# kubeflow/mpi-operator

Hardware: AMD Instinct MI355X
Metric: images/sec (higher is better)
Workload: dtype bf16; 1 GPU; model=resnet101, global_batch=64, image=224, parallelism=dp1, impl=hip, graph=True

## Files before the change

### mpi_operator_amd/ops/csrc/batchnorm.hip

```cpp
#include "common.h"

template <int WHAT>
__global__ void bn_partials_k(const ushort8 *__restrict__ x,
                              const ushort8 *__restrict__ dy,
                              const ushort8 *__restrict__ y,
                              const uint8_t *__restrict__ mask,
                              const float *__restrict__ mean,
                              const float *__restrict__ invstd,
                              float *__restrict__ partial,
                              long M, int C8, int relu) {
  int C = C8 * 8;
  int cb = threadIdx.x % C8;
  int row_lane = threadIdx.x / C8;
  int rows_per_block = blockDim.x / C8;
  float a0[8] = {0}, a1[8] = {0};
  float mn[8], is[8];
  if (WHAT == 1 && row_lane < rows_per_block) {
#pragma unroll
    for (int j = 0; j < 8; ++j) {
      mn[j] = mean[cb * 8 + j];
      is[j] = invstd[cb * 8 + j];
    }
  }
  if (row_lane < rows_per_block) {
    long stride = (long)gridDim.x * rows_per_block;
    for (long row = (long)blockIdx.x * rows_per_block + row_lane; row < M;
         row += 2 * stride) {
      long r2 = row + stride;
      bool has2 = r2 < M;
      long off = row * C8 + cb, off2 = r2 * C8 + cb;
      float fx[8], fx2[8];
      ushort8 vx = x[off];
      ushort8 vx2 = has2 ? x[off2] : ushort8{0, 0, 0, 0, 0, 0, 0, 0};
      bf8_to_f8(vx, fx);
      bf8_to_f8(vx2, fx2);
      if (WHAT == 0) {
#pragma unroll
        for (int j = 0; j < 8; ++j) {
          a0[j] += fx[j] + fx2[j];
          a1[j] += fx[j] * fx[j] + fx2[j] * fx2[j];
        }
      } else {
        ushort8 vdy = dy[off];
        ushort8 vdy2 = has2 ? dy[off2] : ushort8{0, 0, 0, 0, 0, 0, 0, 0};
        float fdy[8], fdy2[8];
        bf8_to_f8(vdy, fdy);
        bf8_to_f8(vdy2, fdy2);
        if (relu) {
          if (mask) {
            int m1 = mask[off], m2 = has2 ? mask[off2] : 0;
#pragma unroll
            for (int j = 0; j < 8; ++j) {
              if (!(m1 & (1 << j))) fdy[j] = 0.f;
              if (!(m2 & (1 << j))) fdy2[j] = 0.f;
            }
          } else {
            ushort8 vy = y[off];
            ushort8 vy2 = has2 ? y[off2] : ushort8{0, 0, 0, 0, 0, 0, 0, 0};
#pragma unroll
            for (int j = 0; j < 8; ++j) {
              if (!(bf2f(vy[j]) > 0.f)) fdy[j] = 0.f;
              if (!(bf2f(vy2[j]) > 0.f)) fdy2[j] = 0.f;
            }
          }
        }
#pragma unroll
        for (int j = 0; j < 8; ++j) {
          a0[j] += fdy[j] + fdy2[j];
          a1[j] += fdy[j] * ((fx[j] - mn[j]) * is[j]) +
                   fdy2[j] * ((fx2[j] - mn[j]) * is[j]);
        }
      }
    }
  }
  __shared__ float lds[2][256 * 8];
#pragma unroll
  for (int j = 0; j < 8; ++j) {
    lds[0][threadIdx.x * 8 + j] = a0[j];
    lds[1][threadIdx.x * 8 + j] = a1[j];
  }
  __syncthreads();
  if (row_lane == 0) {
    for (int rl = 1; rl < rows_per_block; ++rl) {
#pragma unroll
      for (int j = 0; j < 8; ++j) {
        a0[j] += lds[0][(rl * C8 + cb) * 8 + j];
        a1[j] += lds[1][(rl * C8 + cb) * 8 + j];
      }
    }
    float *p0 = partial + (long)blockIdx.x * 2 * C + cb * 8;
    float *p1 = p0 + C;
#pragma unroll
    for (int j = 0; j < 8; ++j) {
      p0[j] = a0[j];
      p1[j] = a1[j];
    }
  }
}

DEV_INLINE void lane8_sums(const float *__restrict__ partial, int grid, int C,
                           int c, int lane8, float &s0, float &s1) {
  s0 = 0.f;
  s1 = 0.f;
  for (int g = lane8; g < grid; g += 32) {
    s0 += partial[(long)g * 2 * C + c];
    s1 += partial[(long)g * 2 * C + C + c];
  }
#pragma unroll
  for (int off = 16; off > 0; off >>= 1) {
    s0 += __shfl_down(s0, off, 32);
    s1 += __shfl_down(s1, off, 32);
  }
}

__global__ void bn_finalize_fwd_k(const float *__restrict__ partial, int grid,
                                  int C, const float *__restrict__ gamma,
                                  const float *__restrict__ beta, float inv_m,
                                  float eps, float *__restrict__ mean,
                                  float *__restrict__ invstd,
                                  float *__restrict__ scale,
                                  float *__restrict__ shift,
                                  float *__restrict__ running_mean,
                                  float *__restrict__ running_var,
                                  float momentum, float unbias) {
  int t = blockIdx.x * blockDim.x + threadIdx.x;
  int c = t / 32, lane8 = t % 32;
  if (c >= C) return;
  float s, sq;
  lane8_sums(partial, grid, C, c, lane8, s, sq);
  if (lane8 != 0) return;
  float mu = s * inv_m;
  float var = fmaxf(sq * inv_m - mu * mu, 0.f);
  float is = rsqrtf(var + eps);
  mean[c] = mu;
  invstd[c] = is;
  float sc = gamma[c] * is;
  scale[c] = sc;
  shift[c] = beta[c] - mu * sc;
  if (running_mean) {
    running_mean[c] = running_mean[c] * (1.f - momentum) + mu * momentum;
    running_var[c] = running_var[c] * (1.f - momentum) + var * unbias * momentum;
  }
}

__global__ void bn_finalize_bwd_k(const float *__restrict__ partial, int grid,
                                  int C, const float *__restrict__ gamma,
                                  const float *__restrict__ invstd, float inv_m,
                                  float *__restrict__ dbeta,
                                  float *__restrict__ dgamma,
                                  float *__restrict__ k1,
                                  float *__restrict__ k2,
                                  float *__restrict__ k3) {
  int t = blockIdx.x * blockDim.x + threadIdx.x;
  int c = t / 32, lane8 = t % 32;
  if (c >= C) return;
  float s0, s1;
  lane8_sums(partial, grid, C, c, lane8, s0, s1);
  if (lane8 != 0) return;
  dbeta[c] = s0;
  dgamma[c] = s1;
  float g_is = gamma[c] * invstd[c];
  k1[c] = g_is;
  k2[c] = g_is * s0 * inv_m;
  k3[c] = g_is * s1 * inv_m;
}

__global__ void bn_finalize_fwd_bands_k(
    const float *__restrict__ partial, int grid, int C,
    const float *__restrict__ gamma, const float *__restrict__ beta,
    float inv_m, float eps, float *__restrict__ mean,
    float *__restrict__ invstd, float *__restrict__ scale,
    float *__restrict__ shift, float *__restrict__ running_mean,
    float *__restrict__ running_var, float momentum,
    float unbias);

__global__ void bn_finalize_bwd_bands_k(
    const float *__restrict__ partial, int grid, int C,
    const float *__restrict__ gamma, const float *__restrict__ invstd,
    float inv_m, float *__restrict__ dbeta, float *__restrict__ dgamma,
    float *__restrict__ k1, float *__restrict__ k2, float *__restrict__ k3) {
  int c = blockIdx.x;
  if (c >= C) return;
  float s0 = 0.f, s1 = 0.f;
  for (int g = threadIdx.x; g < grid; g += 256) {
    s0 += partial[(long)g * 2 * C + c];
    s1 += partial[(long)g * 2 * C + C + c];
  }
  __shared__ float red[2][256 / WAVE];
  s0 = wave_sum(s0);
  s1 = wave_sum(s1);
  if ((threadIdx.x & (WAVE - 1)) == 0) {
    red[0][threadIdx.x / WAVE] = s0;
    red[1][threadIdx.x / WAVE] = s1;
  }
  __syncthreads();
  if (threadIdx.x != 0) return;
  s0 = red[0][0] + red[0][1] + red[0][2] + red[0][3];
  s1 = red[1][0] + red[1][1] + red[1][2] + red[1][3];
  dbeta[c] = s0;
  dgamma[c] = s1;
  float g_is = gamma[c] * invstd[c];
  k1[c] = g_is;
  k2[c] = g_is * s0 * inv_m;
  k3[c] = g_is * s1 * inv_m;
}

__global__ void bn_apply_k(const ushort8 *__restrict__ x,
                           const ushort8 *__restrict__ res,
                           const float *__restrict__ scale,
                           const float *__restrict__ shift,
                           ushort8 *__restrict__ y,
                           uint8_t *__restrict__ mask,
                           long M, int C8, int relu) {
  int cb = threadIdx.x % C8;
  int row_lane = threadIdx.x / C8;
  int rows_per_block = blockDim.x / C8;
  if (row_lane >= rows_per_block) return;
  float sc[8], sh[8];
#pragma unroll
  for (int j = 0; j < 8; ++j) {
    sc[j] = scale[cb * 8 + j];
    sh[j] = shift[cb * 8 + j];
  }
  long stride = (long)gridDim.x * rows_per_block;
  for (long row = (long)blockIdx.x * rows_per_block + row_lane; row < M;
       row += 2 * stride) {
    long r2 = row + stride;
    long off = row * C8 + cb, off2 = r2 * C8 + cb;
    ushort8 v = x[off];
    ushort8 v2 = r2 < M ? x[off2] : ushort8{0, 0, 0, 0, 0, 0, 0, 0};
    float f[8], f2[8], g[8] = {0}, g2[8] = {0};
    bf8_to_f8(v, f);
    bf8_to_f8(v2, f2);
    if (res) {
      ushort8 w = res[off];
      ushort8 w2 = r2 < M ? res[off2] : ushort8{0, 0, 0, 0, 0, 0, 0, 0};
      bf8_to_f8(w, g);
      bf8_to_f8(w2, g2);
    }
    int m1 = 0, m2 = 0;
#pragma unroll
    for (int j = 0; j < 8; ++j) {
      f[j] = f[j] * sc[j] + sh[j] + g[j];
      f2[j] = f2[j] * sc[j] + sh[j] + g2[j];
      if (relu) {
        if (f[j] > 0.f) m1 |= 1 << j;
        if (f2[j] > 0.f) m2 |= 1 << j;
        f[j] = fmaxf(f[j], 0.f);
        f2[j] = fmaxf(f2[j], 0.f);
      }
    }
    y[off] = f8_to_bf8(f);
    if (r2 < M) y[off2] = f8_to_bf8(f2);
    if (relu && mask) {
      mask[off] = (uint8_t)m1;
      if (r2 < M) mask[off2] = (uint8_t)m2;
    }
  }
}

__global__ void bn_bwd_apply_k(const ushort8 *__restrict__ dy,
                               const ushort8 *__restrict__ x,
                               const ushort8 *__restrict__ y,
                               const uint8_t *__restrict__ mask,
                               const float *__restrict__ mean,
                               const float *__restrict__ invstd,
                               const float *__restrict__ k1,
                               const float *__restrict__ k2,
                               const float *__restrict__ k3,
                               ushort8 *__restrict__ dx, long M, int C8,
                               int relu) {
  int cb = threadIdx.x % C8;
  int row_lane = threadIdx.x / C8;
  int rows_per_block = blockDim.x / C8;
  if (row_lane >= rows_per_block) return;
  float mn[8], is[8], a[8], b[8], c3[8];
#pragma unroll
  for (int j = 0; j < 8; ++j) {
    int c = cb * 8 + j;
    mn[j] = mean[c];
    is[j] = invstd[c];
    a[j] = k1[c];
    b[j] = k2[c];
    c3[j] = k3[c];
  }
  long stride = (long)gridDim.x * rows_per_block;
  for (long row = (long)blockIdx.x * rows_per_block + row_lane; row < M;
       row += 2 * stride) {
    long r2 = row + stride;
    long off = row * C8 + cb, off2 = r2 * C8 + cb;
    ushort8 vdy = dy[off], vx = x[off];
    ushort8 vdy2 = r2 < M ? dy[off2] : ushort8{0, 0, 0, 0, 0, 0, 0, 0};
    ushort8 vx2 = r2 < M ? x[off2] : ushort8{0, 0, 0, 0, 0, 0, 0, 0};
    float fdy[8], fx[8], fdy2[8], fx2[8];
    bf8_to_f8(vdy, fdy);
    bf8_to_f8(vx, fx);
    bf8_to_f8(vdy2, fdy2);
    bf8_to_f8(vx2, fx2);
    if (relu) {
      if (mask) {
        int m1 = mask[off], m2 = r2 < M ? mask[off2] : 0;
#pragma unroll
        for (int j = 0; j < 8; ++j) {
          if (!(m1 & (1 << j))) fdy[j] = 0.f;
          if (!(m2 & (1 << j))) fdy2[j] = 0.f;
        }
      } else {
        ushort8 vy = y[off];
        ushort8 vy2 = r2 < M ? y[off2] : ushort8{0, 0, 0, 0, 0, 0, 0, 0};
#pragma unroll
        for (int j = 0; j < 8; ++j) {
          if (!(bf2f(vy[j]) > 0.f)) fdy[j] = 0.f;
          if (!(bf2f(vy2[j]) > 0.f)) fdy2[j] = 0.f;
        }
      }
    }
#pragma unroll
    for (int j = 0; j < 8; ++j) {
      fdy[j] = a[j] * fdy[j] - b[j] - c3[j] * ((fx[j] - mn[j]) * is[j]);
      fdy2[j] = a[j] * fdy2[j] - b[j] - c3[j] * ((fx2[j] - mn[j]) * is[j]);
    }
    dx[off] = f8_to_bf8(fdy);
    if (r2 < M) dx[off2] = f8_to_bf8(fdy2);
  }
}

extern "C" int bn_grid_cap(int C8) {
  static const long ovr = [] {
    const char *e = getenv("MPIAMD_BN_GRID");
    long v = e ? atol(e) : 0;
    return (v >= 1 && v <= 8192) ? v : 0;
  }();
  (void)C8;
  return ovr ? (int)ovr : 512;
}

static void bn_geom(long M, int C8, int &grid, int &rows_per_block) {
  rows_per_block = 256 / C8;
  long g = (M + rows_per_block - 1) / rows_per_block;
  long cap = bn_grid_cap(C8);
  grid = (int)(g > cap ? cap : (g < 1 ? 1 : g));
}

static int bn_apply_grid(long M, int C8) {
  static const long cap = [] {
    const char *e = getenv("MPIAMD_BN_APPLY_GRID");
    long v = e ? atol(e) : 0;
    return (v >= 64 && v <= 16384) ? v : 2048L;
  }();
  int rpb = 256 / C8;
  long g = (M + rpb - 1) / rpb;
  return (int)(g > cap ? cap : (g < 1 ? 1 : g));
}

extern "C" hipError_t bn_fwd_train_launch(
    const void *x, const void *res, const float *gamma, const float *beta,
    float eps, int relu, void *y, uint8_t *relu_mask, float *mean,
    float *invstd, float *scale, float *shift, float *partial,
    float *running_mean, float *running_var, float momentum, long M, int C,
    hipStream_t s) {
  int C8 = C / 8;
  if (C8 < 1 || C8 > 256) return hipErrorInvalidValue;
  int grid, rpb;
  bn_geom(M, C8, grid, rpb);
  bn_partials_k<0><<<grid, 256, 0, s>>>((const ushort8 *)x, nullptr, nullptr,
                                        nullptr, nullptr, nullptr, partial, M,
                                        C8, 0);
  HIP_KERNEL_CHECK();
  float unbias = M > 1 ? (float)M / (float)(M - 1) : 1.f;
  bn_finalize_fwd_bands_k<<<C, 256, 0, s>>>(
      partial, grid, C, gamma, beta, 1.f / (float)M, eps, mean, invstd, scale,
      shift, running_mean, running_var, momentum, unbias);
  HIP_KERNEL_CHECK();
  bn_apply_k<<<bn_apply_grid(M, C8), 256, 0, s>>>(
      (const ushort8 *)x, (const ushort8 *)res, scale, shift, (ushort8 *)y,
      relu_mask, M, C8, relu);
  HIP_KERNEL_CHECK();
  return hipSuccess;
}

__global__ void bn_finalize_fwd_bands_k(
    const float *__restrict__ partial, int grid, int C,
    const float *__restrict__ gamma, const float *__restrict__ beta,
    float inv_m, float eps, float *__restrict__ mean,
    float *__restrict__ invstd, float *__restrict__ scale,
    float *__restrict__ shift, float *__restrict__ running_mean,
    float *__restrict__ running_var, float momentum, float unbias) {
  int c = blockIdx.x;
  if (c >= C) return;
  float s = 0.f, sq = 0.f;
  for (int g = threadIdx.x; g < grid; g += 256) {
    s += partial[(long)g * 2 * C + c];
    sq += partial[(long)g * 2 * C + C + c];
  }
  __shared__ float red[2][256 / WAVE];
  s = wave_sum(s);
  sq = wave_sum(sq);
  if ((threadIdx.x & (WAVE - 1)) == 0) {
    red[0][threadIdx.x / WAVE] = s;
    red[1][threadIdx.x / WAVE] = sq;
  }
  __syncthreads();
  if (threadIdx.x != 0) return;
  s = red[0][0] + red[0][1] + red[0][2] + red[0][3];
  sq = red[1][0] + red[1][1] + red[1][2] + red[1][3];
  float mu = s * inv_m;
  float var = fmaxf(sq * inv_m - mu * mu, 0.f);
  float is = rsqrtf(var + eps);
  mean[c] = mu;
  invstd[c] = is;
  float sc = gamma[c] * is;
  scale[c] = sc;
  shift[c] = beta[c] - mu * sc;
  if (running_mean) {
    running_mean[c] = running_mean[c] * (1.f - momentum) + mu * momentum;
    running_var[c] = running_var[c] * (1.f - momentum) + var * unbias * momentum;
  }
}

extern "C" hipError_t bn_fwd_train_pre_launch(
    const float *pre_partial, int pre_grid, const void *x, const void *res,
    const float *gamma, const float *beta, float eps, int relu, void *y,
    uint8_t *relu_mask, float *mean, float *invstd, float *scale,
    float *shift, float *running_mean, float *running_var, float momentum,
    long M, int C, hipStream_t s) {
  int C8 = C / 8;
  if (C8 < 1 || C8 > 256) return hipErrorInvalidValue;
  float unbias = M > 1 ? (float)M / (float)(M - 1) : 1.f;
  bn_finalize_fwd_bands_k<<<C, 256, 0, s>>>(
      pre_partial, pre_grid, C, gamma, beta, 1.f / (float)M, eps, mean,
      invstd, scale, shift, running_mean, running_var, momentum, unbias);
  HIP_KERNEL_CHECK();
  bn_apply_k<<<bn_apply_grid(M, C8), 256, 0, s>>>(
      (const ushort8 *)x, (const ushort8 *)res, scale, shift, (ushort8 *)y,
      relu_mask, M, C8, relu);
  HIP_KERNEL_CHECK();
  return hipSuccess;
}

extern "C" hipError_t bn_fwd_eval_launch(const void *x, const float *scale,
                                         const float *shift, int relu, void *y,
                                         long M, int C, hipStream_t s) {
  int C8 = C / 8;
  if (C8 < 1 || C8 > 256) return hipErrorInvalidValue;
  int grid, rpb;
  bn_geom(M, C8, grid, rpb);
  bn_apply_k<<<bn_apply_grid(M, C8), 256, 0, s>>>(
      (const ushort8 *)x, nullptr, scale, shift, (ushort8 *)y, nullptr, M, C8,
      relu);
  HIP_KERNEL_CHECK();
  return hipSuccess;
}

extern "C" hipError_t bn_bwd_launch(const void *dy, const void *x,
                                    const void *y, const uint8_t *relu_mask,
                                    const float *gamma, const float *mean,
                                    const float *invstd, int relu, void *dx,
                                    float *dgamma, float *dbeta, float *k1,
                                    float *k2, float *k3, float *partial,
                                    long M, int C, hipStream_t s) {
  int C8 = C / 8;
  if (C8 < 1 || C8 > 256) return hipErrorInvalidValue;
  int grid, rpb;
  bn_geom(M, C8, grid, rpb);
  bn_partials_k<1><<<grid, 256, 0, s>>>((const ushort8 *)x, (const ushort8 *)dy,
                                        (const ushort8 *)y, relu_mask, mean,
                                        invstd, partial, M, C8, relu);
  HIP_KERNEL_CHECK();
  bn_finalize_bwd_bands_k<<<C, 256, 0, s>>>(
      partial, grid, C, gamma, invstd, 1.f / (float)M, dbeta, dgamma, k1, k2, k3);
  HIP_KERNEL_CHECK();
  bn_bwd_apply_k<<<bn_apply_grid(M, C8), 256, 0, s>>>(
      (const ushort8 *)dy, (const ushort8 *)x, (const ushort8 *)y, relu_mask,
      mean, invstd, k1, k2, k3, (ushort8 *)dx, M, C8, relu);
  HIP_KERNEL_CHECK();
  return hipSuccess;
}
```

### mpi_operator_amd/ops/csrc/bindings.cpp

```cpp
#include <torch/extension.h>

#include <ATen/hip/impl/HIPGuardImplMasqueradingAsCUDA.h>
#include <ATen/hip/impl/HIPStreamMasqueradingAsCUDA.h>
#include <hip/hip_runtime.h>

#include <vector>

namespace {

using at::Tensor;

int conv_splits(long M, int Ncols, int K) {
  static const int force = [] {
    const char *e = getenv("MPIAMD_CONV_SPLITS");
    return e ? atoi(e) : -1;
  }();
  if (force >= 1) return force;
  long tiles = ((M + 127) / 128) * ((Ncols + 127) / 128);
  int nk = (K + 63) / 64;
  if (tiles >= 256 || nk < 16) return 1;
  long s = 512 / tiles;
  if (s > nk / 8) s = nk / 8;
  if (s > 16) s = 16;
  return s < 1 ? 1 : (int)s;
}

#define CHK(call)                                                              \
  do {                                                                         \
    hipError_t e_ = (call);                                                    \
    TORCH_CHECK(e_ == hipSuccess, "HIP kernel failure: ", hipGetErrorString(e_)); \
  } while (0)

hipStream_t cur_stream() {
  return c10::hip::getCurrentHIPStreamMasqueradingAsCUDA().stream();
}
using HIPDeviceGuard = c10::hip::HIPGuardMasqueradingAsCUDA;

void check_cl_bf16(const Tensor &t, const char *name) {
  TORCH_CHECK(t.is_cuda(), name, " must be on GPU");
  TORCH_CHECK(t.scalar_type() == at::kBFloat16, name, " must be bf16");
  TORCH_CHECK(t.dim() == 4 && t.is_contiguous(at::MemoryFormat::ChannelsLast),
              name, " must be 4-D channels_last");
}

Tensor empty_cl_bf16(int64_t n, int64_t c, int64_t h, int64_t w, const Tensor &like) {
  return at::empty({n, c, h, w}, like.options().dtype(at::kBFloat16),
                   at::MemoryFormat::ChannelsLast);
}

}

extern "C" {
hipError_t add_relu_fwd(const void *, const void *, void *, long, hipStream_t);
hipError_t add_bf16(const void *, const void *, void *, long, hipStream_t);
hipError_t add_relu_bwd(const void *, const void *, void *, long, hipStream_t);
hipError_t add_relu_bwd_add(const void *, const void *, const void *, void *,
                            long, hipStream_t);
hipError_t add_relu_bwd_add_mask(const void *, const void *, const void *,
                                 void *, long, hipStream_t);
hipError_t gap_fwd(const void *, void *, int, int, int, hipStream_t);
hipError_t gap_bwd(const void *, void *, int, int, int, hipStream_t);
hipError_t bias_add(void *, const float *, long, int, hipStream_t);
hipError_t colsum_bf16(const void *, float *, float *, long, int, long, hipStream_t);
int colsum_chunks(long, int);
struct SgdDesc {
  const void *grad;
  float *master;
  float *mom;
  uint16_t *out;
  long numel;
};
hipError_t sgd_step_launch(const SgdDesc *, int, int, float, float, float, int,
                           hipStream_t);
int bn_grid_cap(int);
hipError_t bn_fwd_train_launch(const void *, const void *, const float *,
                               const float *, float, int, void *, uint8_t *,
                               float *, float *, float *, float *, float *,
                               float *, float *, float, long, int,
                               hipStream_t);
hipError_t bn_fwd_eval_launch(const void *, const float *, const float *, int,
                              void *, long, int, hipStream_t);
hipError_t bn_bwd_launch(const void *, const void *, const void *,
                         const uint8_t *, const float *, const float *,
                         const float *, int, void *, float *, float *,
                         float *, float *, float *, float *, long, int,
                         hipStream_t);
hipError_t maxpool_fwd_launch(const void *, void *, uint8_t *, int, int, int,
                              int, int, int, int, int, int, hipStream_t);
hipError_t maxpool_bwd_launch(const void *, const uint8_t *, void *, int, int,
                              int, int, int, int, int, int, int, hipStream_t);
hipError_t softmax_xent_fwd_launch(const void *, const long *, float *, float *,
                                   int, int, hipStream_t);
hipError_t masked_xent_fwd_launch(const void *, const long *, float *, float *,
                                  int, int, long, long, hipStream_t);
hipError_t masked_xent_bwd_launch(const void *, const long *, const float *,
                                  const float *, const float *, void *, int,
                                  int, long, long, hipStream_t);
hipError_t attn_fwd_launch(const void *, void *, void *, const float *, int,
                           int, int, float, hipStream_t);
hipError_t attn_bwd_launch(const void *, const void *, const void *, void *,
                           int, int, int, float, hipStream_t);
hipError_t softmax_xent_bwd_launch(const float *, const long *, void *, int,
                                   int, const float *, hipStream_t);
hipError_t gemm_nt(const void *, const void *, void *, int, int, int, long,
                   long, long, int, hipStream_t);
hipError_t gemm_nt_bias(const void *, const void *, const float *, void *,
                        int, int, int, long, long, long, hipStream_t);
hipError_t gemm_nt_bias_sk(const void *, const void *, const float *, float *,
                           void *, int, int, int, long, long, long, int,
                           hipStream_t);
int gemm_fwd_splits(int, int, int);
hipError_t gemm_nt_tn(const void *, const void *, void *, int, int, int, long,
                      long, long, int, hipStream_t);
hipError_t gemm_nt_tn_acc(const void *, const void *, void *, int, int, int,
                          long, long, long, hipStream_t);
hipError_t gemm_nt_gelu_bias(const void *, const void *, const float *,
                             void *, void *, int, int, int, long, long, long,
                             hipStream_t);
hipError_t gemm_nt_tn_gelubwd(const void *, const void *, const void *,
                              void *, int, int, int, long, long, long,
                              void *, hipStream_t);
int gemm_gelubwd_wants_wt(int, int, int);
hipError_t gemm_tn_tn(const void *, const void *, void *, int, int, int, long,
                      long, long, int, hipStream_t);
int gemm_tn_tn_splits(int, int, int);
hipError_t gemm_tn_tn_sk(const void *, const void *, float *, void *, int,
                         int, int, long, long, long, int, int, hipStream_t);
hipError_t gemm_nt_tn_sk(const void *, const void *, float *, void *, int,
                         int, int, long, long, long, int, hipStream_t);
int gemm_nt_tn_splits(int, int, int);
hipError_t conv_fwd(const void *, const void *, void *, int, int, int, int,
                    int, int, int, int, int, int, int, int, float *,
                    hipStream_t);
hipError_t conv_dgrad(const void *, const void *, void *, int, int, int, int,
                      int, int, int, int, int, int, int, int, float *,
                      hipStream_t);
hipError_t conv_fwd_bn(const void *, const void *, void *, int, int, int,
                       int, int, int, int, int, int, int, int, float *,
                       hipStream_t);
hipError_t bn_fwd_train_pre_launch(const float *, int, const void *,
                                   const void *, const float *, const float *,
                                   float, int, void *, uint8_t *, float *,
                                   float *, float *, float *, float *,
                                   float *, float, long, int, hipStream_t);
hipError_t conv_dgrad_1x1_acc(const void *, const void *, void *, long, int,
                              int, hipStream_t);
hipError_t conv_wgrad_implicit(const void *, const void *, float *, void *,
                               int, int, int, int, int, int, int, int, int,
                               int, int, int, int, hipStream_t);
hipError_t mfma_probe(const void *, const void *, float *, hipStream_t);
hipError_t ln_fwd(const void *, const float *, const float *, void *, float *,
                  float *, long, int, float, hipStream_t);
hipError_t ln_fwd_add(const void *, const void *, const float *,
                      const float *, void *, void *, float *, float *, long,
                      int, float, hipStream_t);
hipError_t ln_bwd(const void *, const void *, const float *, const float *,
                  const float *, void *, float *, float *, long, int, int *,
                  hipStream_t);
}

static Tensor conv2d_fwd(const Tensor &x, const Tensor &w, int64_t stride,
                         int64_t pad) {
  check_cl_bf16(x, "x");
  check_cl_bf16(w, "w");
  const HIPDeviceGuard guard(x.device());
  int N = x.size(0), C = x.size(1), H = x.size(2), W = x.size(3);
  int Kout = w.size(0), R = w.size(2), S = w.size(3);
  TORCH_CHECK(w.size(1) == C, "conv channel mismatch");
  TORCH_CHECK(C % 8 == 0, "conv requires C%8==0 (pad the stem input)");
  int HO = (H + 2 * (int)pad - R) / (int)stride + 1;
  int WO = (W + 2 * (int)pad - S) / (int)stride + 1;
  Tensor y = empty_cl_bf16(N, Kout, HO, WO, x);
  long M = (long)N * HO * WO;
  int splits = conv_splits(M, Kout, R * S * C);
  Tensor partial;
  float *pp = nullptr;
  if (splits > 1) {
    partial = at::empty({(long)splits, M, (long)Kout},
                        x.options().dtype(at::kFloat));
    pp = partial.data_ptr<float>();
  }
  CHK(conv_fwd(x.data_ptr(), w.data_ptr(), y.data_ptr(), N, H, W, C, Kout, R,
               S, (int)stride, (int)pad, HO, WO, splits, pp, cur_stream()));
  return y;
}

static Tensor conv2d_dgrad(const Tensor &dy, const Tensor &w, int64_t H,
                           int64_t W, int64_t stride, int64_t pad) {
  check_cl_bf16(dy, "dy");
  check_cl_bf16(w, "w");
  const HIPDeviceGuard guard(dy.device());
  int N = dy.size(0), Kout = dy.size(1), HO = dy.size(2), WO = dy.size(3);
  int C = w.size(1), R = w.size(2), S = w.size(3);
  TORCH_CHECK(Kout % 8 == 0, "dgrad requires out-channels %8==0");
  TORCH_CHECK(stride == 1 || stride == 2,
              "conv2d_dgrad supports stride 1 or 2 only, got ", stride);
  Tensor dx = empty_cl_bf16(N, C, H, W, dy);
  long M = (long)N * H * W;
  int splits = stride == 1 ? conv_splits(M, C, R * S * Kout) : 1;
  Tensor partial;
  float *pp = nullptr;
  if (splits > 1) {
    partial = at::empty({(long)splits, M, (long)C},
                        dy.options().dtype(at::kFloat));
    pp = partial.data_ptr<float>();
  }
  CHK(conv_dgrad(dy.data_ptr(), w.data_ptr(), dx.data_ptr(), N, (int)H,
                 (int)W, C, Kout, R, S, (int)stride, (int)pad, HO, WO, splits,
                 pp, cur_stream()));
  return dx;
}

static Tensor conv2d_wgrad(const Tensor &x, const Tensor &dy, int64_t R,
                           int64_t S, int64_t stride, int64_t pad) {
  check_cl_bf16(x, "x");
  check_cl_bf16(dy, "dy");
  const HIPDeviceGuard guard(x.device());
  int N = x.size(0), C = x.size(1), H = x.size(2), W = x.size(3);
  int Kout = dy.size(1), HO = dy.size(2), WO = dy.size(3);
  int RSC = (int)R * S * C;
  int tiles = ((Kout + 127) / 128) * ((RSC + 127) / 128);
  long M = (long)N * HO * WO;
  int nk = (int)((M + 63) / 64);
  static const int budget = [] {
    const char *e = getenv("MPIAMD_WGRAD_BUDGET");
    int v = e ? atoi(e) : 0;
    return (v >= 64 && v <= 2048) ? v : 512;
  }();
  int splits = std::max(budget / tiles, 1);
  splits = std::min(splits, std::max(nk / 8, 1));
  splits = std::min(splits, 256);
  if (splits >= 8) splits &= ~7;
  Tensor partial = at::empty({(long)splits, (long)Kout, (long)RSC},
                             x.options().dtype(at::kFloat));
  Tensor dw = at::empty({(int64_t)Kout, (int64_t)C, R, S},
                        x.options().dtype(at::kBFloat16),
                        at::MemoryFormat::ChannelsLast);
  CHK(conv_wgrad_implicit(dy.data_ptr(), x.data_ptr(),
                          partial.data_ptr<float>(), dw.data_ptr(), N, H, W, C,
                          Kout, (int)R, (int)S, (int)stride, (int)pad, HO, WO,
                          splits, 1, cur_stream()));
  return dw;
}

static Tensor add_bf16_b(const Tensor &a, const Tensor &b) {
  const HIPDeviceGuard guard(a.device());
  TORCH_CHECK(a.numel() == b.numel() && a.numel() % 8 == 0);
  Tensor c = at::empty_like(a);
  CHK(add_bf16(a.data_ptr(), b.data_ptr(), c.data_ptr(), a.numel(), cur_stream()));
  return c;
}

static void conv2d_dgrad_acc(const Tensor &dy, const Tensor &w, Tensor &dx_acc) {
  check_cl_bf16(dy, "dy");
  check_cl_bf16(w, "w");
  check_cl_bf16(dx_acc, "dx_acc");
  const HIPDeviceGuard guard(dy.device());
  TORCH_CHECK(w.size(2) == 1 && w.size(3) == 1, "acc dgrad is 1x1-only");
  long M = (long)dy.size(0) * dy.size(2) * dy.size(3);
  CHK(conv_dgrad_1x1_acc(dy.data_ptr(), w.data_ptr(), dx_acc.data_ptr(), M,
                         (int)w.size(1), (int)dy.size(1), cur_stream()));
}

static std::vector<Tensor> conv2d_fwd_bn(const Tensor &x, const Tensor &w,
                                         int64_t stride, int64_t pad) {
  check_cl_bf16(x, "x");
  check_cl_bf16(w, "w");
  const HIPDeviceGuard guard(x.device());
  int N = x.size(0), C = x.size(1), H = x.size(2), W = x.size(3);
  int Kout = w.size(0), R = w.size(2), S = w.size(3);
  int HO = (H + 2 * (int)pad - R) / (int)stride + 1;
  int WO = (W + 2 * (int)pad - S) / (int)stride + 1;
  long M = (long)N * HO * WO;
  int splits = conv_splits(M, Kout, R * S * C);
  auto f32 = x.options().dtype(at::kFloat);
  if (splits > 1 || Kout % 8 != 0) {
    Tensor y = conv2d_fwd(x, w, stride, pad);
    return {y, at::empty({0}, f32)};
  }
  Tensor y = empty_cl_bf16(N, Kout, HO, WO, x);
  long bands = (M + 63) / 64;
  Tensor slab = at::empty({bands, 2, (long)Kout}, f32);
  CHK(conv_fwd_bn(x.data_ptr(), w.data_ptr(), y.data_ptr(), N, H, W, C, Kout,
                  R, S, (int)stride, (int)pad, HO, WO,
                  slab.data_ptr<float>(), cur_stream()));
  return {y, slab};
}

static std::vector<Tensor> bn_fwd_train_pre(
    const Tensor &x, const Tensor &slab, const Tensor &gamma,
    const Tensor &beta, double eps, bool relu, const Tensor &running_mean,
    const Tensor &running_var, double momentum, const Tensor &res) {
  check_cl_bf16(x, "x");
  const HIPDeviceGuard guard(x.device());
  int N = x.size(0), C = x.size(1), H = x.size(2), W = x.size(3);
  long M = (long)N * H * W;
  TORCH_CHECK(slab.numel() == ((M + 63) / 64) * 2 * (long)C, "slab shape");
  auto f32 = x.options().dtype(at::kFloat);
  Tensor y = empty_cl_bf16(N, C, H, W, x);
  Tensor mean = at::empty({C}, f32), invstd = at::empty({C}, f32);
  Tensor scale = at::empty({C}, f32), shift = at::empty({C}, f32);
  float *rm = running_mean.defined() && running_mean.numel() == C
                  ? running_mean.data_ptr<float>() : nullptr;
  float *rv = rm ? running_var.data_ptr<float>() : nullptr;
  const void *resp = nullptr;
  if (res.defined() && res.numel() > 0) {
    check_cl_bf16(res, "res");
    resp = res.data_ptr();
  }
  Tensor mask;
  uint8_t *mp = nullptr;
  if (relu) {
    mask = at::empty({M, (long)C / 8}, x.options().dtype(at::kByte));
    mp = mask.data_ptr<uint8_t>();
  } else {
    mask = at::empty({0}, x.options().dtype(at::kByte));
  }
  CHK(bn_fwd_train_pre_launch(
      slab.data_ptr<float>(), (int)((M + 63) / 64), x.data_ptr(), resp,
      gamma.data_ptr<float>(), beta.data_ptr<float>(), (float)eps,
      relu ? 1 : 0, y.data_ptr(), mp, mean.data_ptr<float>(),
      invstd.data_ptr<float>(), scale.data_ptr<float>(),
      shift.data_ptr<float>(), rm, rv, (float)momentum, M, C, cur_stream()));
  return {y, mean, invstd, mask};
}

static std::vector<Tensor> bn_fwd_train(const Tensor &x, const Tensor &gamma,
                                        const Tensor &beta, double eps,
                                        bool relu, const Tensor &running_mean,
                                        const Tensor &running_var,
                                        double momentum, const Tensor &res) {
  check_cl_bf16(x, "x");
  const HIPDeviceGuard guard(x.device());
  int N = x.size(0), C = x.size(1), H = x.size(2), W = x.size(3);
  long M = (long)N * H * W;
  auto f32 = x.options().dtype(at::kFloat);
  Tensor y = empty_cl_bf16(N, C, H, W, x);
  Tensor mean = at::empty({C}, f32), invstd = at::empty({C}, f32);
  Tensor scale = at::empty({C}, f32), shift = at::empty({C}, f32);
  Tensor partial = at::empty({(long)bn_grid_cap(C / 8) * 2 * C}, f32);
  float *rm = running_mean.defined() && running_mean.numel() == C
                  ? running_mean.data_ptr<float>() : nullptr;
  float *rv = rm ? running_var.data_ptr<float>() : nullptr;
  const void *resp = nullptr;
  if (res.defined() && res.numel() > 0) {
    check_cl_bf16(res, "res");
    resp = res.data_ptr();
  }
  Tensor mask;
  uint8_t *mp = nullptr;
  if (relu) {
    mask = at::empty({M, (long)C / 8}, x.options().dtype(at::kByte));
    mp = mask.data_ptr<uint8_t>();
  } else {
    mask = at::empty({0}, x.options().dtype(at::kByte));
  }
  CHK(bn_fwd_train_launch(x.data_ptr(), resp, gamma.data_ptr<float>(),
                          beta.data_ptr<float>(), (float)eps, relu ? 1 : 0,
                          y.data_ptr(), mp, mean.data_ptr<float>(),
                          invstd.data_ptr<float>(), scale.data_ptr<float>(),
                          shift.data_ptr<float>(), partial.data_ptr<float>(),
                          rm, rv, (float)momentum, M, C, cur_stream()));
  return {y, mean, invstd, mask};
}

static Tensor bn_fwd_eval(const Tensor &x, const Tensor &scale,
                          const Tensor &shift, bool relu) {
  check_cl_bf16(x, "x");
  const HIPDeviceGuard guard(x.device());
  int N = x.size(0), C = x.size(1), H = x.size(2), W = x.size(3);
  Tensor y = empty_cl_bf16(N, C, H, W, x);
  CHK(bn_fwd_eval_launch(x.data_ptr(), scale.contiguous().data_ptr<float>(),
                         shift.contiguous().data_ptr<float>(), relu ? 1 : 0,
                         y.data_ptr(), (long)N * H * W, C, cur_stream()));
  return y;
}

static std::vector<Tensor> bn_bwd(const Tensor &dy, const Tensor &x,
                                  const Tensor &y, const Tensor &gamma,
                                  const Tensor &mean, const Tensor &invstd,
                                  bool relu, const Tensor &mask) {
  check_cl_bf16(dy, "dy");
  check_cl_bf16(x, "x");
  const HIPDeviceGuard guard(x.device());
  int N = x.size(0), C = x.size(1), H = x.size(2), W = x.size(3);
  long M = (long)N * H * W;
  auto f32 = x.options().dtype(at::kFloat);
  Tensor dx = empty_cl_bf16(N, C, H, W, x);
  Tensor dgamma = at::empty({C}, f32), dbeta = at::empty({C}, f32);
  Tensor k1 = at::empty({C}, f32), k2 = at::empty({C}, f32), k3 = at::empty({C}, f32);
  Tensor partial = at::empty({(long)bn_grid_cap(C / 8) * 2 * C}, f32);
  const uint8_t *mp =
      mask.defined() && mask.numel() > 0 ? mask.data_ptr<uint8_t>() : nullptr;
  CHK(bn_bwd_launch(dy.data_ptr(), x.data_ptr(), y.data_ptr(), mp,
                    gamma.data_ptr<float>(), mean.data_ptr<float>(),
                    invstd.data_ptr<float>(), relu ? 1 : 0, dx.data_ptr(),
                    dgamma.data_ptr<float>(), dbeta.data_ptr<float>(),
                    k1.data_ptr<float>(), k2.data_ptr<float>(),
                    k3.data_ptr<float>(), partial.data_ptr<float>(), M, C,
                    cur_stream()));
  return {dx, dgamma, dbeta};
}

static std::vector<Tensor> maxpool_fwd(const Tensor &x, int64_t K,
                                       int64_t stride, int64_t pad) {
  check_cl_bf16(x, "x");
  const HIPDeviceGuard guard(x.device());
  int N = x.size(0), C = x.size(1), H = x.size(2), W = x.size(3);
  int HO = (H + 2 * (int)pad - (int)K) / (int)stride + 1;
  int WO = (W + 2 * (int)pad - (int)K) / (int)stride + 1;
  Tensor y = empty_cl_bf16(N, C, HO, WO, x);
  Tensor idx = at::empty({N, HO, WO, C}, x.options().dtype(at::kByte));
  CHK(maxpool_fwd_launch(x.data_ptr(), y.data_ptr(), idx.data_ptr<uint8_t>(),
                         N, H, W, HO, WO, C, (int)K, (int)stride, (int)pad,
                         cur_stream()));
  return {y, idx};
}

static Tensor maxpool_bwd(const Tensor &dy, const Tensor &idx, int64_t H,
                          int64_t W, int64_t K, int64_t stride, int64_t pad) {
  check_cl_bf16(dy, "dy");
  const HIPDeviceGuard guard(dy.device());
  int N = dy.size(0), C = dy.size(1), HO = dy.size(2), WO = dy.size(3);
  Tensor dx = empty_cl_bf16(N, C, H, W, dy);
  CHK(maxpool_bwd_launch(dy.data_ptr(), idx.data_ptr<uint8_t>(), dx.data_ptr(),
                         N, (int)H, (int)W, HO, WO, C, (int)K, (int)stride,
                         (int)pad, cur_stream()));
  return dx;
}

static Tensor gap_fwd_b(const Tensor &x) {
  check_cl_bf16(x, "x");
  const HIPDeviceGuard guard(x.device());
  int N = x.size(0), C = x.size(1), HW = x.size(2) * x.size(3);
  Tensor y = at::empty({N, C}, x.options());
  CHK(gap_fwd(x.data_ptr(), y.data_ptr(), N, HW, C, cur_stream()));
  return y;
}

static Tensor gap_bwd_b(const Tensor &dy, int64_t H, int64_t W) {
  TORCH_CHECK(dy.is_cuda() && dy.scalar_type() == at::kBFloat16);
  const HIPDeviceGuard guard(dy.device());
  Tensor dyc = dy.contiguous();
  int N = dy.size(0), C = dy.size(1);
  Tensor dx = empty_cl_bf16(N, C, H, W, dy);
  CHK(gap_bwd(dyc.data_ptr(), dx.data_ptr(), N, (int)(H * W), C, cur_stream()));
  return dx;
}

static std::vector<Tensor> layernorm_fwd(const Tensor &x, const Tensor &gamma,
                                         const Tensor &beta, double eps) {
  TORCH_CHECK(x.is_cuda() && x.scalar_type() == at::kBFloat16);
  const HIPDeviceGuard guard(x.device());
  Tensor xc = x.contiguous();
  long M = xc.numel() / xc.size(-1);
  int N = xc.size(-1);
  auto f32 = x.options().dtype(at::kFloat);
  Tensor y = at::empty_like(xc);
  Tensor mean = at::empty({M}, f32), rstd = at::empty({M}, f32);
  CHK(ln_fwd(xc.data_ptr(), gamma.data_ptr<float>(), beta.data_ptr<float>(),
             y.data_ptr(), mean.data_ptr<float>(), rstd.data_ptr<float>(), M,
             N, (float)eps, cur_stream()));
  return {y, mean, rstd};
}

static std::vector<Tensor> layernorm_add_fwd(const Tensor &a, const Tensor &b,
                                             const Tensor &gamma,
                                             const Tensor &beta, double eps) {
  const HIPDeviceGuard guard(a.device());
  Tensor ac = a.contiguous(), bc = b.contiguous();
  TORCH_CHECK(ac.sizes() == bc.sizes());
  long M = ac.numel() / ac.size(-1);
  int N = ac.size(-1);
  auto f32 = a.options().dtype(at::kFloat);
  Tensor sum = at::empty_like(ac);
  Tensor y = at::empty_like(ac);
  Tensor mean = at::empty({M}, f32), rstd = at::empty({M}, f32);
  CHK(ln_fwd_add(ac.data_ptr(), bc.data_ptr(), gamma.data_ptr<float>(),
                 beta.data_ptr<float>(), sum.data_ptr(), y.data_ptr(),
                 mean.data_ptr<float>(), rstd.data_ptr<float>(), M, N,
                 (float)eps, cur_stream()));
  return {y, sum, mean, rstd};
}

static std::vector<Tensor> layernorm_bwd(const Tensor &dy, const Tensor &x,
                                         const Tensor &gamma,
                                         const Tensor &mean,
                                         const Tensor &rstd) {
  const HIPDeviceGuard guard(x.device());
  Tensor dyc = dy.contiguous(), xc = x.contiguous();
  long M = xc.numel() / xc.size(-1);
  int N = xc.size(-1);
  auto f32 = x.options().dtype(at::kFloat);
  Tensor partial = at::empty({512, 2L * N}, f32);
  Tensor dgb = at::empty({2L * N}, f32);
  Tensor dx = at::empty_like(xc);
  CHK(ln_bwd(dyc.data_ptr(), xc.data_ptr(), gamma.data_ptr<float>(),
             mean.data_ptr<float>(), rstd.data_ptr<float>(), dx.data_ptr(),
             partial.data_ptr<float>(), dgb.data_ptr<float>(), M, N, nullptr,
             cur_stream()));
  return {dx, dgb.narrow(0, 0, N), dgb.narrow(0, N, N)};
}

static Tensor linear_fwd(const Tensor &x, const Tensor &w, const Tensor &b) {
  TORCH_CHECK(x.is_cuda() && x.scalar_type() == at::kBFloat16);
  const HIPDeviceGuard guard(x.device());
  Tensor xc = x.contiguous(), wc = w.contiguous();
  int M = xc.size(0), K = xc.size(1), N = wc.size(0);
  TORCH_CHECK(K % 8 == 0, "linear requires in_features %8==0");
  Tensor y = at::empty({M, N}, xc.options());
  Tensor bf = b.scalar_type() == at::kFloat ? b.contiguous()
                                            : b.to(at::kFloat).contiguous();
  int fsp = gemm_fwd_splits(M, N, K);
  Tensor part;
  float *pp = nullptr;
  if (fsp > 1) {
    part = at::empty({fsp, (long)M * N}, x.options().dtype(at::kFloat));
    pp = part.data_ptr<float>();
  }
  CHK(gemm_nt_bias_sk(xc.data_ptr(), wc.data_ptr(), bf.data_ptr<float>(), pp,
                      y.data_ptr(), M, N, K, K, K, N, fsp, cur_stream()));
  return y;
}

static std::vector<Tensor> linear_bwd(const Tensor &dy, const Tensor &x,
                                      const Tensor &w) {
  const HIPDeviceGuard guard(x.device());
  Tensor dyc = dy.contiguous(), xc = x.contiguous(), wc = w.contiguous();
  int M = xc.size(0), K = xc.size(1), N = wc.size(0);
  auto f32 = x.options().dtype(at::kFloat);
  long Np = (N + 7) / 8 * 8;
  Tensor dyp = dyc;
  if (Np != N) {
    dyp = at::zeros({M, Np}, dyc.options());
    dyp.narrow(1, 0, N).copy_(dyc);
  }
  Tensor dx = at::empty({M, K}, xc.options());
  int dx_splits = gemm_nt_tn_splits(M, K, N);
  Tensor dxp = dx_splits > 1 ? at::empty({dx_splits, (long)M * K}, f32) : dx;
  CHK(gemm_nt_tn_sk(dyp.data_ptr(), wc.data_ptr(),
                    dx_splits > 1 ? dxp.data_ptr<float>() : nullptr,
                    dx.data_ptr(), M, K, N, Np, K, K, dx_splits,
                    cur_stream()));
  bool wbf = wc.scalar_type() == at::kBFloat16;
  Tensor dw = at::empty({N, K}, wbf ? wc.options() : f32);
  int dw_splits = gemm_tn_tn_splits(N, K, M);
  Tensor dwp = dw_splits > 1
                   ? at::empty({dw_splits, (long)N * K}, f32)
                   : dw;
  CHK(gemm_tn_tn_sk(dyp.data_ptr(),
                    xc.data_ptr(),
                    dw_splits > 1 ? dwp.data_ptr<float>() : nullptr,
                    dw.data_ptr(), N, K, M, Np, K, K, dw_splits, wbf ? 1 : 0,
                    cur_stream()));
  Tensor db = at::empty({N}, f32);
  int chunks = colsum_chunks(M, N);
  Tensor dbp = chunks > 0 ? at::empty({chunks, (long)N}, f32) : db;
  CHK(colsum_bf16(dyc.data_ptr(), dbp.data_ptr<float>(),
                  db.data_ptr<float>(), M, N, N, cur_stream()));
  return {dx, dw, db};
}

static Tensor linear_dgrad(const Tensor &dy, const Tensor &w) {
  const HIPDeviceGuard guard(dy.device());
  Tensor dyc = dy.contiguous(), wc = w.contiguous();
  int M = dyc.size(0), N = wc.size(0), K = wc.size(1);
  auto f32 = dy.options().dtype(at::kFloat);
  long Np = (N + 7) / 8 * 8;
  Tensor dyp = dyc;
  if (Np != N) {
    dyp = at::zeros({M, Np}, dyc.options());
    dyp.narrow(1, 0, N).copy_(dyc);
  }
  Tensor dx = at::empty({M, K}, dyc.options());
  int dx_splits = gemm_nt_tn_splits(M, K, N);
  Tensor dxp = dx_splits > 1 ? at::empty({dx_splits, (long)M * K}, f32) : dx;
  CHK(gemm_nt_tn_sk(dyp.data_ptr(), wc.data_ptr(),
                    dx_splits > 1 ? dxp.data_ptr<float>() : nullptr,
                    dx.data_ptr(), M, K, N, Np, K, K, dx_splits,
                    cur_stream()));
  return dx;
}

static Tensor linear_dgrad_acc(const Tensor &dy, const Tensor &w,
                               Tensor acc) {
  const HIPDeviceGuard guard(dy.device());
  Tensor dyc = dy.contiguous(), wc = w.contiguous();
  int M = dyc.size(0), N = wc.size(0), K = wc.size(1);
  TORCH_CHECK(N % 8 == 0, "linear_dgrad_acc requires out_features %8");
  TORCH_CHECK(acc.is_contiguous() && acc.size(0) == M && acc.size(1) == K);
  CHK(gemm_nt_tn_acc(dyc.data_ptr(), wc.data_ptr(), acc.data_ptr(), M, K, N,
                     N, K, K, cur_stream()));
  return acc;
}

static std::vector<Tensor> linear_wgrad_only(const Tensor &dy,
                                             const Tensor &x) {
  const HIPDeviceGuard guard(x.device());
  Tensor dyc = dy.contiguous(), xc = x.contiguous();
  int M = xc.size(0), K = xc.size(1), N = dyc.size(1);
  auto f32 = x.options().dtype(at::kFloat);
  bool wbf = xc.scalar_type() == at::kBFloat16;
  Tensor dw = at::empty({N, K}, wbf ? xc.options() : f32);
  int dw_splits = gemm_tn_tn_splits(N, K, M);
  Tensor dwp =
      dw_splits > 1 ? at::empty({dw_splits, (long)N * K}, f32) : dw;
  CHK(gemm_tn_tn_sk(dyc.data_ptr(), xc.data_ptr(),
                    dw_splits > 1 ? dwp.data_ptr<float>() : nullptr,
                    dw.data_ptr(), N, K, M, N, K, K, dw_splits, wbf ? 1 : 0,
                    cur_stream()));
  Tensor db = at::empty({N}, f32);
  int chunks = colsum_chunks(M, N);
  Tensor dbp = chunks > 0 ? at::empty({chunks, (long)N}, f32) : db;
  CHK(colsum_bf16(dyc.data_ptr(), dbp.data_ptr<float>(),
                  db.data_ptr<float>(), M, N, N, cur_stream()));
  return {dw, db};
}

static std::vector<Tensor> attn_fwd(const Tensor &qkv, int64_t heads,
                                    double scale,
                                    const c10::optional<Tensor> &mask,
                                    bool want_probs) {
  TORCH_CHECK(qkv.is_cuda() && qkv.scalar_type() == at::kBFloat16);
  TORCH_CHECK(qkv.dim() == 5 && qkv.size(2) == 3 && qkv.size(4) == 64,
              "qkv must be [B,S,3,H,64]");
  TORCH_CHECK(qkv.is_contiguous());
  const HIPDeviceGuard guard(qkv.device());
  int B = qkv.size(0), S = qkv.size(1), H = qkv.size(3);
  TORCH_CHECK(H == heads);
  TORCH_CHECK(S <= 256, "fused attention supports seq <= 256");
  Tensor ctx = at::empty({B, S, (long)H * 64}, qkv.options());
  Tensor probs;
  const float *mp = nullptr;
  Tensor maskc;
  if (mask.has_value()) {
    maskc = mask->to(at::kFloat).contiguous();
    TORCH_CHECK(maskc.numel() == (long)B * S, "mask must be [B,S] additive");
    mp = maskc.data_ptr<float>();
  }
  void *pp = nullptr;
  if (want_probs) {
    probs = at::empty({B, (long)H, S, S}, qkv.options());
    pp = probs.data_ptr();
  }
  CHK(attn_fwd_launch(qkv.data_ptr(), ctx.data_ptr(), pp, mp, B, S, H,
                      (float)scale, cur_stream()));
  if (!want_probs) probs = at::empty({0}, qkv.options());
  return {ctx, probs};
}

static Tensor attn_bwd(const Tensor &qkv, const Tensor &dctx,
                       const Tensor &probs, double scale) {
  TORCH_CHECK(qkv.is_cuda() && qkv.scalar_type() == at::kBFloat16);
  const HIPDeviceGuard guard(qkv.device());
  int B = qkv.size(0), S = qkv.size(1), H = qkv.size(3);
  TORCH_CHECK(S == 128 && qkv.size(4) == 64, "fused attn bwd: S=128, D=64");
  TORCH_CHECK(qkv.is_contiguous() && probs.is_contiguous());
  Tensor dc = dctx.contiguous();
  Tensor dqkv = at::empty_like(qkv);
  CHK(attn_bwd_launch(qkv.data_ptr(), dc.data_ptr(), probs.data_ptr(),
                      dqkv.data_ptr(), B, S, H, (float)scale, cur_stream()));
  return dqkv;
}

static std::vector<Tensor> linear_gelu_fwd(const Tensor &x, const Tensor &w,
                                           const Tensor &b) {
  TORCH_CHECK(x.is_cuda() && x.scalar_type() == at::kBFloat16 && x.dim() == 2);
  TORCH_CHECK(x.is_contiguous() && w.is_contiguous());
  const HIPDeviceGuard guard(x.device());
  int M = x.size(0), K = x.size(1), N = w.size(0);
  TORCH_CHECK(w.size(1) == K);
  Tensor bias = b.to(at::kFloat).contiguous();
  Tensor g = at::empty({M, N}, x.options());
  Tensor deriv = at::empty({M, N}, x.options());
  CHK(gemm_nt_gelu_bias(x.data_ptr(), w.data_ptr(), bias.data_ptr<float>(),
                        deriv.data_ptr(), g.data_ptr(), M, N, K, K, K, N,
                        cur_stream()));
  return {g, deriv};
}

static Tensor linear_gelu_dgrad(const Tensor &dy, const Tensor &w,
                                const Tensor &pre) {
  TORCH_CHECK(dy.is_cuda() && dy.scalar_type() == at::kBFloat16);
  TORCH_CHECK(dy.is_contiguous() && w.is_contiguous() && pre.is_contiguous());
  const HIPDeviceGuard guard(dy.device());
  int M = dy.size(0), K = dy.size(1), N = w.size(1);
  TORCH_CHECK(pre.size(0) == M && pre.size(1) == N);
  Tensor dh = at::empty({M, N}, dy.options());
  Tensor wt;
  void *wtp = nullptr;
  if (gemm_gelubwd_wants_wt(M, N, K)) {
    wt = at::empty({N, K}, dy.options());
    wtp = wt.data_ptr();
  }
  CHK(gemm_nt_tn_gelubwd(dy.data_ptr(), w.data_ptr(), pre.data_ptr(),
                         dh.data_ptr(), M, N, K, K, N, N, wtp, cur_stream()));
  return dh;
}

static std::vector<Tensor> softmax_xent_fwd(const Tensor &logits,
                                            const Tensor &target) {
  TORCH_CHECK(logits.is_cuda() && logits.scalar_type() == at::kBFloat16);
  const HIPDeviceGuard guard(logits.device());
  int B = logits.size(0), V = logits.size(1);
  auto f32 = logits.options().dtype(at::kFloat);
  Tensor probs = at::empty({B, V}, f32);
  Tensor loss = at::empty({}, f32);
  CHK(softmax_xent_fwd_launch(logits.data_ptr(), target.data_ptr<long>(),
                              probs.data_ptr<float>(), loss.data_ptr<float>(),
                              B, V, cur_stream()));
  return {loss, probs};
}

static Tensor softmax_xent_bwd(const Tensor &probs, const Tensor &target,
                               const Tensor &dloss) {
  const HIPDeviceGuard guard(probs.device());
  int B = probs.size(0), V = probs.size(1);
  TORCH_CHECK(dloss.is_cuda() && dloss.scalar_type() == at::kFloat &&
              dloss.numel() == 1, "dloss must be a device fp32 scalar");
  Tensor d = at::empty({B, V}, probs.options().dtype(at::kBFloat16));
  CHK(softmax_xent_bwd_launch(probs.data_ptr<float>(), target.data_ptr<long>(),
                              d.data_ptr(), B, V, dloss.data_ptr<float>(),
                              cur_stream()));
  return d;
}

static std::vector<Tensor> masked_xent_fwd(const Tensor &logits,
                                           const Tensor &target,
                                           int64_t ignore_index) {
  TORCH_CHECK(logits.is_cuda() && logits.scalar_type() == at::kBFloat16);
  TORCH_CHECK(logits.is_contiguous());
  const HIPDeviceGuard guard(logits.device());
  int B = logits.size(0), V = logits.size(1);
  auto f32 = logits.options().dtype(at::kFloat);
  Tensor stats = at::empty({B, 2}, f32);
  Tensor out = at::empty({2}, f32);
  CHK(masked_xent_fwd_launch(logits.data_ptr(), target.data_ptr<long>(),
                             stats.data_ptr<float>(), out.data_ptr<float>(),
                             B, V, V, ignore_index, cur_stream()));
  return {out, stats};
}

static Tensor masked_xent_bwd(const Tensor &logits, const Tensor &target,
                              const Tensor &stats, const Tensor &out,
                              const Tensor &dloss, int64_t ignore_index) {
  const HIPDeviceGuard guard(logits.device());
  int B = logits.size(0), V = logits.size(1);
  TORCH_CHECK(dloss.is_cuda() && dloss.scalar_type() == at::kFloat &&
              dloss.numel() == 1, "dloss must be a device fp32 scalar");
  Tensor d = at::empty({B, V}, logits.options());
  CHK(masked_xent_bwd_launch(logits.data_ptr(), target.data_ptr<long>(),
                             stats.data_ptr<float>(), out.data_ptr<float>(),
                             dloss.data_ptr<float>(), d.data_ptr(), B, V, V,
                             ignore_index, cur_stream()));
  return d;
}

static std::vector<Tensor> mlm_head_fwd(const Tensor &h, const Tensor &w,
                                        const Tensor &b, const Tensor &target,
                                        int64_t ignore_index) {
  TORCH_CHECK(h.is_cuda() && h.scalar_type() == at::kBFloat16 && h.dim() == 2);
  TORCH_CHECK(h.is_contiguous() && w.is_contiguous());
  TORCH_CHECK(b.scalar_type() == at::kFloat, "mlm bias must be fp32");
  const HIPDeviceGuard guard(h.device());
  int M = h.size(0), K = h.size(1), V = w.size(0);
  TORCH_CHECK(w.size(1) == K && target.numel() == M);
  long Vp = ((long)V + 7) / 8 * 8;
  auto f32 = h.options().dtype(at::kFloat);
  Tensor logits = at::empty({M, Vp}, h.options());
  Tensor bc = b.contiguous();
  CHK(gemm_nt_bias(h.data_ptr(), w.data_ptr(), bc.data_ptr<float>(),
                   logits.data_ptr(), M, V, K, K, K, Vp, cur_stream()));
  Tensor stats = at::empty({M, 2}, f32);
  Tensor out = at::empty({2}, f32);
  CHK(masked_xent_fwd_launch(logits.data_ptr(), target.data_ptr<long>(),
                             stats.data_ptr<float>(), out.data_ptr<float>(),
                             M, V, Vp, ignore_index, cur_stream()));
  return {out, logits, stats};
}

static std::vector<Tensor> mlm_head_bwd(const Tensor &logits, int64_t V64,
                                        const Tensor &target,
                                        const Tensor &stats, const Tensor &out,
                                        const Tensor &dloss, const Tensor &h,
                                        const Tensor &w, int64_t ignore_index) {
  const HIPDeviceGuard guard(h.device());
  int M = logits.size(0), V = (int)V64, K = h.size(1);
  long Vp = logits.size(1);
  TORCH_CHECK(dloss.is_cuda() && dloss.scalar_type() == at::kFloat &&
              dloss.numel() == 1, "dloss must be a device fp32 scalar");
  auto f32 = h.options().dtype(at::kFloat);
  Tensor dlog = at::empty_like(logits);
  CHK(masked_xent_bwd_launch(logits.data_ptr(), target.data_ptr<long>(),
                             stats.data_ptr<float>(), out.data_ptr<float>(),
                             dloss.data_ptr<float>(), dlog.data_ptr(), M, V,
                             Vp, ignore_index, cur_stream()));
  Tensor dh = at::empty({M, K}, h.options());
  int dx_splits = gemm_nt_tn_splits(M, K, V);
  Tensor dhp = dx_splits > 1 ? at::empty({dx_splits, (long)M * K}, f32) : dh;
  CHK(gemm_nt_tn_sk(dlog.data_ptr(), w.data_ptr(),
                    dx_splits > 1 ? dhp.data_ptr<float>() : nullptr,
                    dh.data_ptr(), M, K, V, Vp, K, K, dx_splits,
                    cur_stream()));
  bool wbf = w.scalar_type() == at::kBFloat16;
  Tensor dw = at::empty({(long)V, K}, wbf ? w.options() : f32);
  int dw_splits = gemm_tn_tn_splits(V, K, M);
  Tensor dwp = dw_splits > 1 ? at::empty({dw_splits, (long)V * K}, f32) : dw;
  CHK(gemm_tn_tn_sk(dlog.data_ptr(), h.data_ptr(),
                    dw_splits > 1 ? dwp.data_ptr<float>() : nullptr,
                    dw.data_ptr(), V, K, M, Vp, K, K, dw_splits, wbf ? 1 : 0,
                    cur_stream()));
  Tensor db_pad = at::empty({Vp}, f32);
  int chunks = colsum_chunks(M, (int)Vp);
  Tensor dbp = chunks > 0 ? at::empty({chunks, Vp}, f32) : db_pad;
  CHK(colsum_bf16(dlog.data_ptr(), dbp.data_ptr<float>(),
                  db_pad.data_ptr<float>(), M, (int)Vp, Vp, cur_stream()));
  return {dh, dw, db_pad.narrow(0, 0, V)};
}

static Tensor add_relu_fwd_b(const Tensor &a, const Tensor &b) {
  check_cl_bf16(a, "a");
  const HIPDeviceGuard guard(a.device());
  Tensor y = at::empty_like(a);
  CHK(add_relu_fwd(a.data_ptr(), b.data_ptr(), y.data_ptr(), a.numel(), cur_stream()));
  return y;
}

static Tensor add_relu_bwd_b(const Tensor &dy, const Tensor &y) {
  const HIPDeviceGuard guard(dy.device());
  Tensor dx = at::empty_like(dy);
  CHK(add_relu_bwd(dy.data_ptr(), y.data_ptr(), dx.data_ptr(), dy.numel(), cur_stream()));
  return dx;
}

static Tensor add_relu_bwd_add_b(const Tensor &dy, const Tensor &y,
                                 const Tensor &dx0) {
  const HIPDeviceGuard guard(dy.device());
  TORCH_CHECK(dy.numel() == y.numel() && dy.numel() == dx0.numel() &&
              dy.numel() % 8 == 0);
  Tensor out = at::empty_like(dx0);
  CHK(add_relu_bwd_add(dy.data_ptr(), y.data_ptr(), dx0.data_ptr(),
                       out.data_ptr(), dy.numel(), cur_stream()));
  return out;
}

static Tensor add_relu_bwd_add_mask_b(const Tensor &dy, const Tensor &mask,
                                      const Tensor &dx0) {
  const HIPDeviceGuard guard(dy.device());
  TORCH_CHECK(dy.numel() == dx0.numel() && dy.numel() % 8 == 0 &&
              mask.numel() == dy.numel() / 8 &&
              mask.scalar_type() == at::kByte);
  Tensor out = at::empty_like(dx0);
  CHK(add_relu_bwd_add_mask(dy.data_ptr(), mask.data_ptr(), dx0.data_ptr(),
                            out.data_ptr(), dy.numel(), cur_stream()));
  return out;
}

static void sgd_step(std::vector<Tensor> masters, std::vector<Tensor> grads,
                     std::vector<Tensor> momenta, std::vector<Tensor> outs,
                     double lr, double mu, double wd, bool nesterov) {
  TORCH_CHECK(!masters.empty());
  const HIPDeviceGuard guard(masters[0].device());
  std::vector<SgdDesc> by_dtype[2];
  for (size_t i = 0; i < masters.size(); ++i) {
    SgdDesc d;
    d.grad = grads[i].data_ptr();
    d.master = masters[i].data_ptr<float>();
    d.mom = momenta[i].data_ptr<float>();
    d.out = outs[i].numel() > 0 ? (uint16_t *)outs[i].data_ptr() : nullptr;
    d.numel = masters[i].numel();
    by_dtype[grads[i].scalar_type() == at::kBFloat16 ? 1 : 0].push_back(d);
  }
  for (int t = 0; t < 2; ++t)
    if (!by_dtype[t].empty())
      CHK(sgd_step_launch(by_dtype[t].data(), (int)by_dtype[t].size(), t,
                          (float)lr, (float)mu, (float)wd, nesterov ? 1 : 0,
                          cur_stream()));
}

static Tensor gemm_nt_b(const Tensor &a, const Tensor &b, bool c_f32) {
  const HIPDeviceGuard guard(a.device());
  Tensor ac = a.contiguous(), bc = b.contiguous();
  int M = ac.size(0), K = ac.size(1), N = bc.size(0);
  TORCH_CHECK(bc.size(1) == K);
  TORCH_CHECK(K % 8 == 0, "gemm_nt requires K%8==0");
  Tensor c = at::empty({M, N}, ac.options().dtype(c_f32 ? at::kFloat : at::kBFloat16));
  CHK(gemm_nt(ac.data_ptr(), bc.data_ptr(), c.data_ptr(), M, N, K, K, K, N,
              c_f32 ? 1 : 0, cur_stream()));
  return c;
}

PYBIND11_MODULE(TORCH_EXTENSION_NAME, m) {
  m.def("conv2d_fwd", &conv2d_fwd);
  m.def("conv2d_dgrad", &conv2d_dgrad);
  m.def("conv2d_fwd_bn", &conv2d_fwd_bn);
  m.def("bn_fwd_train_pre", &bn_fwd_train_pre);
  m.def("conv2d_wgrad", &conv2d_wgrad);
  m.def("conv2d_dgrad_acc", &conv2d_dgrad_acc);
  m.def("add_bf16", &add_bf16_b);
  m.def("bn_fwd_train", &bn_fwd_train);
  m.def("bn_fwd_eval", &bn_fwd_eval);
  m.def("bn_bwd", &bn_bwd);
  m.def("maxpool_fwd", &maxpool_fwd);
  m.def("maxpool_bwd", &maxpool_bwd);
  m.def("gap_fwd", &gap_fwd_b);
  m.def("gap_bwd", &gap_bwd_b);
  m.def("layernorm_fwd", &layernorm_fwd);
  m.def("layernorm_bwd", &layernorm_bwd);
  m.def("layernorm_add_fwd", &layernorm_add_fwd);
  m.def("linear_fwd", &linear_fwd);
  m.def("linear_bwd", &linear_bwd);
  m.def("linear_dgrad", &linear_dgrad);
  m.def("linear_dgrad_acc", &linear_dgrad_acc);
  m.def("softmax_xent_fwd", &softmax_xent_fwd);
  m.def("masked_xent_fwd", &masked_xent_fwd);
  m.def("mlm_head_fwd", &mlm_head_fwd);
  m.def("mlm_head_bwd", &mlm_head_bwd);
  m.def("linear_gelu_fwd", &linear_gelu_fwd);
  m.def("attn_fwd", &attn_fwd);
  m.def("attn_bwd", &attn_bwd);
  m.def("linear_wgrad_only", &linear_wgrad_only);
  m.def("linear_gelu_dgrad", &linear_gelu_dgrad);
  m.def("masked_xent_bwd", &masked_xent_bwd);
  m.def("softmax_xent_bwd", &softmax_xent_bwd);
  m.def("add_relu_fwd", &add_relu_fwd_b);
  m.def("add_relu_bwd", &add_relu_bwd_b);
  m.def("add_relu_bwd_add", &add_relu_bwd_add_b);
  m.def("add_relu_bwd_add_mask", &add_relu_bwd_add_mask_b);
  m.def("sgd_step", &sgd_step);
  m.def("gemm_nt", &gemm_nt_b);
  m.def("mfma_probe", [](const Tensor &a, const Tensor &b) {
    const HIPDeviceGuard guard(a.device());
    Tensor d = at::empty({16, 16}, a.options().dtype(at::kFloat));
    CHK(mfma_probe(a.contiguous().data_ptr(), b.contiguous().data_ptr(),
                   d.data_ptr<float>(), cur_stream()));
    return d;
  });
}
```

### mpi_operator_amd/ops/csrc/common.h

```cpp
#pragma once
#include <hip/hip_runtime.h>
#include <hip/hip_bf16.h>
#include <stdint.h>

#define DEV_INLINE __device__ __forceinline__

constexpr int WAVE = 64;

using bf16 = __hip_bfloat16;
typedef __attribute__((ext_vector_type(8))) uint16_t ushort8;
typedef __attribute__((ext_vector_type(4))) uint16_t ushort4v;
typedef __attribute__((ext_vector_type(4))) float float4v;
typedef __attribute__((ext_vector_type(8))) float float8v;
typedef __attribute__((ext_vector_type(2))) float float2v;

DEV_INLINE float bf2f(uint16_t u) {
  union { uint32_t i; float f; } v;
  v.i = uint32_t(u) << 16;
  return v.f;
}

DEV_INLINE uint16_t f2bf(float f) {
  union { float f; uint32_t i; } v;
  v.f = f;
  uint32_t lsb = (v.i >> 16) & 1u;
  v.i += 0x7fffu + lsb;
  return uint16_t(v.i >> 16);
}

DEV_INLINE void bf8_to_f8(const ushort8 &u, float *f) {
#pragma unroll
  for (int i = 0; i < 8; ++i) f[i] = bf2f(u[i]);
}

DEV_INLINE ushort8 f8_to_bf8(const float *f) {
  ushort8 u;
#pragma unroll
  for (int i = 0; i < 8; ++i) u[i] = f2bf(f[i]);
  return u;
}

DEV_INLINE float wave_sum(float v) {
#pragma unroll
  for (int off = 32; off > 0; off >>= 1) v += __shfl_xor(v, off, WAVE);
  return v;
}

DEV_INLINE float wave_max(float v) {
#pragma unroll
  for (int off = 32; off > 0; off >>= 1) v = fmaxf(v, __shfl_xor(v, off, WAVE));
  return v;
}

#define HIP_KERNEL_CHECK()                                                    \
  do {                                                                        \
    hipError_t e = hipGetLastError();                                         \
    if (e != hipSuccess) return e;                                            \
  } while (0)

DEV_INLINE constexpr int cdiv(int a, int b) { return (a + b - 1) / b; }
static inline int cdiv_h(long a, long b) { return (int)((a + b - 1) / b); }
```

### mpi_operator_amd/ops/csrc/conv.hip

```cpp
#include "mfma_tile.h"
#include "mix_gemm.h"

extern "C" hipError_t splitk_reduce(const float *, int, long, void *, int,
                                    hipStream_t);

struct ConvFwdStage {
  static constexpr int PITCH = MXP;
  static constexpr bool GLDS = false;
  static DEV_INLINE int rslot(int slot, int) { return slot; }
  const uint16_t *x;
  int H, W, C, HO, WO, S, stride, pad, K;
  long M;
  ushort8 r[4];
  long nbase_[4];
  int hb_[4], wb_[4];
  bool ok_[4];
  DEV_INLINE void init(int tid, int base) {
    int s_row = tid >> 3;
#pragma unroll
    for (int i = 0; i < 4; ++i) {
      long m = base + s_row + 32 * i;
      ok_[i] = m < M;
      int wo = (int)(m % WO);
      long t = m / WO;
      int ho = (int)(t % HO);
      int n = (int)(t / HO);
      nbase_[i] = (long)n * H * W;
      hb_[i] = ho * stride - pad;
      wb_[i] = wo * stride - pad;
    }
  }
  DEV_INLINE void load(int tid, int, int kb, ushort8 *) {
    int k = kb + (tid & 7) * 8;
    int c = k % C, rs = k / C;
    int s_ = rs % S, rr = rs / S;
    bool kok = k < K;
#pragma unroll
    for (int i = 0; i < 4; ++i) {
      int h = hb_[i] + rr, w = wb_[i] + s_;
      if (kok && ok_[i] && (unsigned)h < (unsigned)H && (unsigned)w < (unsigned)W)
        r[i] = *(const ushort8 *)(x + (nbase_[i] + (long)h * W + w) * C + c);
      else
        r[i] = ushort8{0, 0, 0, 0, 0, 0, 0, 0};
    }
  }
  DEV_INLINE void write(int tid, ushort8 *img) const {
    int s_row = tid >> 3, s_slot = tid & 7;
#pragma unroll
    for (int i = 0; i < 4; ++i) img[(s_row + 32 * i) * MXP + s_slot] = r[i];
  }
};

template <int STRIDE> struct ConvDgradStage {
  static constexpr int PITCH = MXP;
  static constexpr bool GLDS = false;
  static DEV_INLINE int rslot(int slot, int) { return slot; }
  const uint16_t *dy;
  int H, W, Q , HO, WO, S, pad, K;
  long M;
  ushort8 r[4];
  long nbase_[4];
  int hb_[4], wb_[4];
  bool ok_[4];
  DEV_INLINE void init(int tid, int base) {
    int s_row = tid >> 3;
#pragma unroll
    for (int i = 0; i < 4; ++i) {
      long m = base + s_row + 32 * i;
      ok_[i] = m < M;
      int w_ = (int)(m % W);
      long t = m / W;
      int h_ = (int)(t % H);
      int n = (int)(t / H);
      nbase_[i] = (long)n * HO * WO;
      hb_[i] = h_ + pad;
      wb_[i] = w_ + pad;
    }
  }
  DEV_INLINE void load(int tid, int, int kb, ushort8 *) {
    int k = kb + (tid & 7) * 8;
    int q = k % Q, rs = k / Q;
    int s_ = rs % S, rr = rs / S;
    bool kok = k < K;
#pragma unroll
    for (int i = 0; i < 4; ++i) {
      int hn = hb_[i] - rr, wn = wb_[i] - s_;
      int ho = hn / STRIDE, wo = wn / STRIDE;
      bool ok = kok && ok_[i] && hn >= 0 && wn >= 0 &&
                (STRIDE == 1 || (hn % STRIDE == 0 && wn % STRIDE == 0)) &&
                ho < HO && wo < WO;
      r[i] = ok ? *(const ushort8 *)(dy + (nbase_[i] + (long)ho * WO + wo) * Q + q)
                : ushort8{0, 0, 0, 0, 0, 0, 0, 0};
    }
  }
  DEV_INLINE void write(int tid, ushort8 *img) const {
    int s_row = tid >> 3, s_slot = tid & 7;
#pragma unroll
    for (int i = 0; i < 4; ++i) img[(s_row + 32 * i) * MXP + s_slot] = r[i];
  }
};

struct XcolStage {
  static constexpr int PITCH = MXP;
  static constexpr bool GLDS = false;
  static DEV_INLINE int rslot(int slot, int row) {
    return slot ^ ((row >> 3) & 7);
  }
  const uint16_t *x;
  int H, W, C, HO, WO, S, stride, pad, RSC;
  long M;
  ushort8 r[4];
  int k0_[2], coff_[2], rr_[2], ss_[2];
  bool cok_[2];
  DEV_INLINE void init(int tid, int base) {
#pragma unroll
    for (int it = 0; it < 2; ++it) {
      int p = tid + it * 256;
      k0_[it] = (p >> 4) * 2;
      int rsc0 = base + (p & 15) * 8;
      cok_[it] = rsc0 < RSC;
      int c = rsc0 % C, rs = rsc0 / C;
      ss_[it] = rs % S;
      rr_[it] = rs / S;
      coff_[it] = c;
    }
  }
  DEV_INLINE ushort8 gather(int it, int n, int ho, int wo, bool mok) const {
    int h = ho * stride + rr_[it] - pad, w = wo * stride + ss_[it] - pad;
    if (mok && cok_[it] && (unsigned)h < (unsigned)H && (unsigned)w < (unsigned)W)
      return *(const ushort8 *)(x + ((long)(n * H + h) * W + w) * C + coff_[it]);
    return ushort8{0, 0, 0, 0, 0, 0, 0, 0};
  }
  DEV_INLINE void load(int tid, int, int kb, ushort8 *) {
#pragma unroll
    for (int it = 0; it < 2; ++it) {
      long m = kb + k0_[it];
      int wo = (int)(m % WO);
      long t = m / WO;
      int ho = (int)(t % HO);
      int n = (int)(t / HO);
      r[it * 2] = gather(it, n, ho, wo, m < M);
      int wo2 = wo + 1, ho2 = ho, n2 = n;
      if (wo2 == WO) {
        wo2 = 0;
        if (++ho2 == HO) {
          ho2 = 0;
          ++n2;
        }
      }
      r[it * 2 + 1] = gather(it, n2, ho2, wo2, m + 1 < M);
    }
  }
  DEV_INLINE void write(int tid, ushort8 *img) const {
    uint32_t *img32 = (uint32_t *)img;
#pragma unroll
    for (int it = 0; it < 2; ++it) {
      int p = tid + it * 256;
      int k0 = (p >> 4) * 2;
      int col0 = (p & 15) * 8;
      int slot = k0 >> 3, within = (k0 & 7) >> 1;
      const ushort8 &va = r[it * 2], &vb = r[it * 2 + 1];
#pragma unroll
      for (int j = 0; j < 8; ++j) {
        int row = col0 + j;
        img32[row * (MXP * 4) + rslot(slot, row) * 4 + within] =
            (uint32_t)va[j] | ((uint32_t)vb[j] << 16);
      }
    }
  }
};

extern "C" hipError_t conv_fwd(const void *x, const void *w, void *y, int N,
                               int H, int W, int C, int Kout, int R, int S,
                               int stride, int pad, int HO, int WO, int splits,
                               float *partial, hipStream_t strm) {
  long M = (long)N * HO * WO;
  int K = R * S * C;
  int nk = (K + BK - 1) / BK;
  if (splits > nk) splits = nk > 0 ? nk : 1;
  void *out = splits > 1 ? (void *)partial : y;
  bool f32 = splits > 1;
  hipError_t e;
  if (R == 1 && S == 1 && stride == 1 && pad == 0) {
    GemmLoader la{(const uint16_t *)x, (int)M, (long)C, C};
    GemmLoader lb{(const uint16_t *)w, Kout, (long)C, C};
    e = launch_nt_gemm(la, lb, out, (int)M, Kout, C, Kout, f32, strm, splits);
  } else if (use_pipegather()) {
    NtPipe<ConvFwdSrc> sa{
        {(const uint16_t *)x, H, W, C, HO, WO, S, stride, pad, K, M}};
    NtPipe<PlainNtSrc> sb{{(const uint16_t *)w, (long)K, Kout, K}};
    e = launch_pipe_mix_wr(sa, sb, out, (int)M, Kout, K,
                           LinearWriter{(long)Kout}, Kout, f32, strm, splits);
  } else {
    ConvFwdStage sa{(const uint16_t *)x, H, W, C, HO, WO, S, stride, pad, K, M};
    GemmLoader lb{(const uint16_t *)w, Kout, (long)K, K};
    e = launch_mix_gemm(sa, NtStage<GemmLoader>{lb}, out, (int)M, Kout, K,
                        Kout, f32, strm, splits);
  }
  if (e != hipSuccess || splits <= 1) return e;
  return splitk_reduce(partial, splits, M * Kout, y, 1, strm);
}

extern "C" hipError_t conv_fwd_bn(const void *x, const void *w, void *y,
                                  int N, int H, int W, int C, int Kout, int R,
                                  int S, int stride, int pad, int HO, int WO,
                                  float *bn_slab, hipStream_t strm) {
  long M = (long)N * HO * WO;
  int K = R * S * C;
  BnStatsWriter wrt{(long)Kout, bn_slab, Kout};
  if (R == 1 && S == 1 && stride == 1 && pad == 0) {
    GemmLoader la{(const uint16_t *)x, (int)M, (long)C, C};
    GemmLoader lb{(const uint16_t *)w, Kout, (long)C, C};
    if (M % 256 == 0 && Kout % 256 == 0 && C % 64 == 0 &&
        (long)(M / 256) * (Kout / 256) >= 128)
      return launch_pipe256_wr(la, lb, y, (int)M, Kout, C, Kout, false, wrt,
                               strm);
    if (use_pipemix()) {
      NtPipe<PlainNtSrc> sa{{(const uint16_t *)x, (long)C, (int)M, C}};
      NtPipe<PlainNtSrc> sb{{(const uint16_t *)w, (long)C, Kout, C}};
      return launch_pipe_mix_wr(sa, sb, y, (int)M, Kout, C, wrt, Kout, false,
                                strm);
    }
    GldsNt ga{la.p, la.rows, la.ld, la.kdim};
    GldsNt gb{lb.p, lb.rows, lb.ld, lb.kdim};
    return launch_mix_gemm_wr(ga, gb, y, (int)M, Kout, C, wrt, Kout, false,
                              strm);
  }
  if (use_pipegather()) {
    NtPipe<ConvFwdSrc> sa{
        {(const uint16_t *)x, H, W, C, HO, WO, S, stride, pad, K, M}};
    NtPipe<PlainNtSrc> sb{{(const uint16_t *)w, (long)K, Kout, K}};
    return launch_pipe_mix_wr(sa, sb, y, (int)M, Kout, K, wrt, Kout, false,
                              strm);
  }
  ConvFwdStage sa{(const uint16_t *)x, H, W, C, HO, WO, S, stride, pad, K, M};
  GemmLoader lb{(const uint16_t *)w, Kout, (long)K, K};
  return launch_mix_gemm_wr(sa, NtStage<GemmLoader>{lb}, y, (int)M, Kout, K,
                            wrt, Kout, false, strm);
}

extern "C" hipError_t conv_dgrad_1x1_acc(const void *dy, const void *w,
                                         void *dx_acc, long M, int C, int Kout,
                                         hipStream_t strm) {
  if (use_pipemix()) {
    NtPipe<PlainNtSrc> sa{{(const uint16_t *)dy, (long)Kout, (int)M, Kout}};
    TnPipe<PlainTnSrc> sb{{(const uint16_t *)w, (long)C, Kout, C}};
    return launch_pipe_mix_wr(sa, sb, dx_acc, (int)M, C, Kout,
                              LinearAccWriter{(long)C}, C, false, strm);
  }
  GemmLoader la{(const uint16_t *)dy, (int)M, (long)Kout, Kout};
  TnRowMajor lb{(const uint16_t *)w, (long)C, Kout, C};
  return launch_mix_gemm_wr(NtStage<GemmLoader>{la}, TnStage<TnRowMajor>{lb},
                            dx_acc, (int)M, C, Kout, LinearAccWriter{(long)C},
                            C, false, strm);
}

struct DgradWTn {
  const uint16_t *w;
  int C, Q, K, RSC;
  DEV_INLINE ushort8 load(int k, int c0) const {
    if (k >= K || c0 >= C) return ushort8{0, 0, 0, 0, 0, 0, 0, 0};
    int q = k % Q, rs = k / Q;
    return *(const ushort8 *)(w + (long)q * RSC + rs * C + c0);
  }
};


struct DgradS2Stage {
  static constexpr int PITCH = MXP;
  static constexpr bool GLDS = false;
  static DEV_INLINE int rslot(int slot, int) { return slot; }
  const uint16_t *dy;
  int HO, WO, Q, W2, H2, K;
  long M;
  int dh0, dw0, nth, ntw;
  ushort8 r[4];
  long nbase_[4];
  int hb_[4], wb_[4];
  bool ok_[4];
  DEV_INLINE void init(int tid, int base) {
    int s_row = tid >> 3;
#pragma unroll
    for (int i = 0; i < 4; ++i) {
      long m = base + s_row + 32 * i;
      ok_[i] = m < M;
      int w_ = (int)(m % W2);
      long t = m / W2;
      int h_ = (int)(t % H2);
      int n = (int)(t / H2);
      nbase_[i] = (long)n * HO * WO;
      hb_[i] = h_;
      wb_[i] = w_;
    }
  }
  DEV_INLINE void load(int tid, int, int kb, ushort8 *) {
    int k = kb + (tid & 7) * 8;
    int q = k % Q, ti = k / Q;
    int ih = ti / ntw, iw = ti - ih * ntw;
    int dho = dh0 - ih, dwo = dw0 - iw;
    bool kok = k < K;
#pragma unroll
    for (int i = 0; i < 4; ++i) {
      int ho = hb_[i] + dho, wo = wb_[i] + dwo;
      bool ok = kok && ok_[i] && (unsigned)ho < (unsigned)HO &&
                (unsigned)wo < (unsigned)WO;
      r[i] = ok ? *(const ushort8 *)(dy + (nbase_[i] + (long)ho * WO + wo) * Q + q)
                : ushort8{0, 0, 0, 0, 0, 0, 0, 0};
    }
  }
  DEV_INLINE void write(int tid, ushort8 *img) const {
    int s_row = tid >> 3, s_slot = tid & 7;
#pragma unroll
    for (int i = 0; i < 4; ++i) img[(s_row + 32 * i) * MXP + s_slot] = r[i];
  }
};

struct DgradWS2Tn {
  const uint16_t *w;
  int C, Q, K, RSC, S;
  int r0, s0, nth, ntw;
  DEV_INLINE ushort8 load(int k, int c0) const {
    if (k >= K || c0 >= C) return ushort8{0, 0, 0, 0, 0, 0, 0, 0};
    int q = k % Q, ti = k / Q;
    int ih = ti / ntw, iw = ti - ih * ntw;
    return *(const ushort8 *)(w + (long)q * RSC +
                              ((r0 + 2 * ih) * S + s0 + 2 * iw) * C + c0);
  }
};

static hipError_t conv_dgrad_s2(const void *dy, const void *w, void *dx,
                                int N, int H, int W, int C, int Kout, int R,
                                int S, int pad, int HO, int WO,
                                hipStream_t strm) {
  int n_live = 0;
  for (int ph = 0; ph < 2; ++ph)
    for (int pw = 0; pw < 2; ++pw) {
      int nth = 0, ntw = 0;
      for (int r = (ph + pad) & 1; r < R; r += 2) nth++;
      for (int s = (pw + pad) & 1; s < S; s += 2) ntw++;
      if (nth > 0 && ntw > 0) n_live++;
    }
  if (n_live != 1 && n_live != 4)
    (void)hipMemsetAsync(dx, 0, (long)N * H * W * C * 2, strm);

  for (int ph = 0; ph < 2; ++ph) {
    int H2 = (H - ph + 1) / 2;
    for (int pw = 0; pw < 2; ++pw) {
      int W2 = (W - pw + 1) / 2;
      DgradS2Stage sa{};
      DgradWS2Tn lb{};
      int r_first = (ph + pad) & 1, s_first = (pw + pad) & 1;
      sa.nth = (R - r_first + 1) / 2;
      sa.ntw = (S - s_first + 1) / 2;
      sa.dh0 = (ph + pad - r_first) / 2;
      sa.dw0 = (pw + pad - s_first) / 2;
      lb.r0 = r_first;
      lb.s0 = s_first;
      if (sa.nth == 0 || sa.ntw == 0 || H2 == 0 || W2 == 0) continue;
      long M = (long)N * H2 * W2;
      int K = sa.nth * sa.ntw * Kout;
      sa.dy = (const uint16_t *)dy;
      sa.HO = HO; sa.WO = WO; sa.Q = Kout; sa.W2 = W2; sa.H2 = H2;
      sa.K = K; sa.M = M;
      lb.w = (const uint16_t *)w;
      lb.C = C; lb.Q = Kout; lb.K = K; lb.RSC = R * S * C; lb.S = S;
      lb.nth = sa.nth; lb.ntw = sa.ntw;
      static const bool pipes2 = [] {
        const char *env = getenv("MPIAMD_PIPES2");
        return !(env && env[0] == '0');
      }();
      hipError_t e;
      if (use_pipegather() && pipes2) {
        NtPipe<DgradS2Src> sa2{{(const uint16_t *)dy, HO, WO, Kout, W2, H2,
                                K, M, sa.dh0, sa.dw0, sa.nth, sa.ntw}};
        TnPipe<DgradWS2TnSrc> sb2{{(const uint16_t *)w, C, Kout, K,
                                   R * S * C, S, r_first, s_first, sa.nth,
                                   sa.ntw}};
        if (n_live == 1) {
          Stride2ZeroWriter wrt{W2, H2, ph, pw, W, H, C};
          e = launch_pipe_mix_wr(sa2, sb2, dx, (int)M, C, K, wrt, C, false,
                                 strm);
        } else {
          Stride2Writer wrt{W2, H2, ph, pw, W, H, C};
          e = launch_pipe_mix_wr(sa2, sb2, dx, (int)M, C, K, wrt, C, false,
                                 strm);
        }
      } else if (n_live == 1) {
        Stride2ZeroWriter wrt{W2, H2, ph, pw, W, H, C};
        e = launch_mix_gemm_wr(sa, TnStage<DgradWS2Tn>{lb}, dx, (int)M, C, K,
                               wrt, C, false, strm);
      } else {
        Stride2Writer wrt{W2, H2, ph, pw, W, H, C};
        e = launch_mix_gemm_wr(sa, TnStage<DgradWS2Tn>{lb}, dx, (int)M, C, K,
                               wrt, C, false, strm);
      }
      if (e != hipSuccess) return e;
    }
  }
  return hipSuccess;
}

extern "C" hipError_t conv_dgrad(const void *dy, const void *w, void *dx,
                                 int N, int H, int W, int C, int Kout, int R,
                                 int S, int stride, int pad, int HO, int WO,
                                 int splits, float *partial,
                                 hipStream_t strm) {
  long M = (long)N * H * W;
  int K = R * S * Kout;
  if (stride != 1)
    return conv_dgrad_s2(dy, w, dx, N, H, W, C, Kout, R, S, pad, HO, WO, strm);
  int nk = (K + BK - 1) / BK;
  if (splits > nk) splits = nk > 0 ? nk : 1;
  void *out = splits > 1 ? (void *)partial : dx;
  bool f32 = splits > 1;
  hipError_t e;
  if (R == 1 && S == 1 && pad == 0) {
    if (use_pipemix()) {
      NtPipe<PlainNtSrc> sa{{(const uint16_t *)dy, (long)Kout, (int)M, Kout}};
      TnPipe<PlainTnSrc> sb{{(const uint16_t *)w, (long)C, Kout, C}};
      e = launch_pipe_mix_wr(sa, sb, out, (int)M, C, Kout, LinearWriter{(long)C},
                             C, f32, strm, splits);
    } else {
      GemmLoader la{(const uint16_t *)dy, (int)M, (long)Kout, Kout};
      TnRowMajor lb{(const uint16_t *)w, (long)C, Kout, C};
      e = launch_mix_gemm(NtStage<GemmLoader>{la}, TnStage<TnRowMajor>{lb}, out,
                          (int)M, C, Kout, C, f32, strm, splits);
    }
  } else if (use_pipegather()) {
    NtPipe<ConvDgradSrc<1>> sa{
        {(const uint16_t *)dy, H, W, Kout, HO, WO, S, pad, K, M}};
    TnPipe<DgradWTnSrc> sb{{(const uint16_t *)w, C, Kout, K, R * S * C}};
    e = launch_pipe_mix_wr(sa, sb, out, (int)M, C, K, LinearWriter{(long)C},
                           C, f32, strm, splits);
  } else {
    DgradWTn lb{(const uint16_t *)w, C, Kout, K, R * S * C};
    ConvDgradStage<1> sa{(const uint16_t *)dy, H, W, Kout, HO, WO, S, pad, K, M};
    e = launch_mix_gemm(sa, TnStage<DgradWTn>{lb}, out, (int)M, C, K, C, f32,
                        strm, splits);
  }
  if (e != hipSuccess || splits <= 1) return e;
  return splitk_reduce(partial, splits, M * C, dx, 1, strm);
}

template <bool OUT_BF16, int SPLITS = 0>
__global__ void splitk_reduce_k(const float4v *__restrict__ partial,
                                int splits_rt, long len4,
                                void *__restrict__ out) {
  const int splits = SPLITS ? SPLITS : splits_rt;
  for (long i = blockIdx.x * blockDim.x + threadIdx.x; i < len4;
       i += (long)gridDim.x * blockDim.x) {
    float4v a = partial[i];
    float4v b = {0.f, 0.f, 0.f, 0.f};
    int s = 1;
    if (SPLITS == 0) {
      for (; s + 8 <= splits; s += 8) {
        float4v c0 = {0.f, 0.f, 0.f, 0.f};
        float4v c1 = {0.f, 0.f, 0.f, 0.f};
#pragma unroll
        for (int j = 0; j < 8; j += 2) {
          c0 += partial[(long)(s + j) * len4 + i];
          c1 += partial[(long)(s + j + 1) * len4 + i];
        }
        a += c0;
        b += c1;
      }
    }
#pragma unroll
    for (; s + 1 < splits; s += 2) {
      a += partial[(long)s * len4 + i];
      b += partial[(long)(s + 1) * len4 + i];
    }
    if (s < splits) b += partial[(long)s * len4 + i];
    a += b;
    if (OUT_BF16) {
      uint16_t *o = (uint16_t *)out + i * 4;
#pragma unroll
      for (int j = 0; j < 4; ++j) o[j] = f2bf(a[j]);
    } else {
      ((float4v *)out)[i] = a;
    }
  }
}

template <int SPLITS>
__global__ void splitk_bias_reduce_k(const float4v *__restrict__ partial,
                                     int splits_rt, long len4, int N4,
                                     const float4v *__restrict__ bias,
                                     uint16_t *__restrict__ out) {
  const int splits = SPLITS ? SPLITS : splits_rt;
  for (long i = blockIdx.x * blockDim.x + threadIdx.x; i < len4;
       i += (long)gridDim.x * blockDim.x) {
    float4v a = partial[i];
    float4v b = {0.f, 0.f, 0.f, 0.f};
    int s = 1;
#pragma unroll
    for (; s + 1 < splits; s += 2) {
      a += partial[(long)s * len4 + i];
      b += partial[(long)(s + 1) * len4 + i];
    }
    if (s < splits) b += partial[(long)s * len4 + i];
    a += b + bias[(int)(i % N4)];
    uint16_t *o = out + i * 4;
#pragma unroll
    for (int j = 0; j < 4; ++j) o[j] = f2bf(a[j]);
  }
}

extern "C" hipError_t splitk_bias_reduce(const float *partial, int splits,
                                         long len, int N, const float *bias,
                                         void *out, hipStream_t s) {
  long len4 = len / 4;
  int grid = (int)((len4 + 255) / 256);
  if (grid > 4096) grid = 4096;
  switch (splits) {
  case 2:
    splitk_bias_reduce_k<2><<<grid, 256, 0, s>>>(
        (const float4v *)partial, splits, len4, N / 4, (const float4v *)bias,
        (uint16_t *)out);
    break;
  case 4:
    splitk_bias_reduce_k<4><<<grid, 256, 0, s>>>(
        (const float4v *)partial, splits, len4, N / 4, (const float4v *)bias,
        (uint16_t *)out);
    break;
  default:
    splitk_bias_reduce_k<0><<<grid, 256, 0, s>>>(
        (const float4v *)partial, splits, len4, N / 4, (const float4v *)bias,
        (uint16_t *)out);
  }
  HIP_KERNEL_CHECK();
  return hipSuccess;
}

__global__ void slab_colreduce_k(const float *__restrict__ partial,
                                 float *__restrict__ out, int chunks,
                                 long N) {
  long c = blockIdx.x;
  if (c >= N) return;
  float a = 0.f;
  for (int g = threadIdx.x; g < chunks; g += 256)
    a += partial[(long)g * N + c];
  __shared__ float red[256 / WAVE];
  a = wave_sum(a);
  if ((threadIdx.x & (WAVE - 1)) == 0) red[threadIdx.x / WAVE] = a;
  __syncthreads();
  if (threadIdx.x == 0) out[c] = red[0] + red[1] + red[2] + red[3];
}

extern "C" hipError_t slab_colreduce(const float *partial, float *out,
                                     int chunks, long N, hipStream_t s) {
  slab_colreduce_k<<<(int)N, 256, 0, s>>>(partial, out, chunks, N);
  HIP_KERNEL_CHECK();
  return hipSuccess;
}

extern "C" hipError_t splitk_reduce(const float *partial, int splits, long len,
                                    void *out, int out_bf16, hipStream_t s) {
  long len4 = len / 4;
  long blocks = (len4 + 255) / 256;
  if (blocks > 2048) blocks = 2048;
  const float4v *p4 = (const float4v *)partial;
  int nb = (int)blocks;
#define SKR_DISPATCH(BF)                                                        do {                                                                            switch (splits) {                                                             case 2: splitk_reduce_k<BF, 2><<<nb, 256, 0, s>>>(p4, splits, len4, out); break;     case 3: splitk_reduce_k<BF, 3><<<nb, 256, 0, s>>>(p4, splits, len4, out); break;     case 4: splitk_reduce_k<BF, 4><<<nb, 256, 0, s>>>(p4, splits, len4, out); break;     case 5: splitk_reduce_k<BF, 5><<<nb, 256, 0, s>>>(p4, splits, len4, out); break;     case 6: splitk_reduce_k<BF, 6><<<nb, 256, 0, s>>>(p4, splits, len4, out); break;     case 8: splitk_reduce_k<BF, 8><<<nb, 256, 0, s>>>(p4, splits, len4, out); break;     case 16: splitk_reduce_k<BF, 16><<<nb, 256, 0, s>>>(p4, splits, len4, out); break;     default: splitk_reduce_k<BF, 0><<<nb, 256, 0, s>>>(p4, splits, len4, out); break;     }                                                                           } while (0)
  if (out_bf16)
    SKR_DISPATCH(true);
  else
    SKR_DISPATCH(false);
#undef SKR_DISPATCH
  return hipGetLastError();
}

extern "C" hipError_t conv_wgrad_implicit(const void *dy, const void *x,
                                          float *partial, void *dw, int N,
                                          int H, int W, int C, int Kout, int R,
                                          int S, int stride, int pad, int HO,
                                          int WO, int splits, int dw_bf16,
                                          hipStream_t strm) {
  long M = (long)N * HO * WO;
  int RSC = R * S * C;
  int nk = (int)((M + BK - 1) / BK);
  if (splits > nk) splits = nk > 0 ? nk : 1;
  TnRowMajor la{(const uint16_t *)dy, Kout, (int)M, Kout};
  hipError_t e;
  if (R == 1 && S == 1 && stride == 1 && pad == 0) {
    if (use_pipemix()) {
      TnPipe<PlainTnSrc> sa{{(const uint16_t *)dy, (long)Kout, (int)M, Kout}};
      TnPipe<PlainTnSrc> sb{{(const uint16_t *)x, (long)C, (int)M, C}};
      e = launch_pipe_mix_wr(sa, sb, partial, Kout, RSC, (int)M,
                             LinearWriter{(long)RSC}, RSC, true, strm, splits);
    } else {
      TnRowMajor lb{(const uint16_t *)x, (long)C, (int)M, C};
      e = launch_mix_gemm(TnStage<TnRowMajor>{la}, TnStage<TnRowMajor>{lb},
                          partial, Kout, RSC, (int)M, RSC, true, strm, splits);
    }
  } else if (use_pipegather_wgrad()) {
    TnPipe<PlainTnSrc> sa{{(const uint16_t *)dy, (long)Kout, (int)M, Kout}};
    TnPipe<XcolSrc> sb{
        {(const uint16_t *)x, H, W, C, HO, WO, S, stride, pad, RSC, M}};
    e = launch_pipe_mix_wr(sa, sb, partial, Kout, RSC, (int)M,
                           LinearWriter{(long)RSC}, RSC, true, strm, splits);
  } else {
    XcolStage sb{(const uint16_t *)x, H, W, C, HO, WO, S, stride, pad, RSC, M};
    e = launch_mix_gemm(TnStage<TnRowMajor>{la}, sb, partial, Kout, RSC,
                        (int)M, RSC, true, strm, splits);
  }
  if (e != hipSuccess) return e;
  return splitk_reduce(partial, splits, (long)Kout * RSC, dw, dw_bf16, strm);
}
```

### mpi_operator_amd/ops/csrc/mix_gemm.h

```cpp
#pragma once
#include "mfma_tile.h"

constexpr int MXP = 9;


template <class L> struct NtStage {
  static constexpr int PITCH = MXP;
  static constexpr bool GLDS = false;
  static DEV_INLINE int rslot(int slot, int) { return slot; }
  L l;
  ushort8 r[4];
  DEV_INLINE void init(int, int) {}
  DEV_INLINE void load(int tid, int base, int kb, ushort8 *) {
    int s_row = tid >> 3, s_slot = tid & 7;
#pragma unroll
    for (int i = 0; i < 4; ++i)
      r[i] = l.load(base + s_row + 32 * i, kb + s_slot * 8);
  }
  DEV_INLINE void write(int tid, ushort8 *img) const {
    int s_row = tid >> 3, s_slot = tid & 7;
#pragma unroll
    for (int i = 0; i < 4; ++i) img[(s_row + 32 * i) * MXP + s_slot] = r[i];
  }
};

template <class L> struct TnStage {
  static constexpr int PITCH = MXP;
  static constexpr bool GLDS = false;
  static DEV_INLINE int rslot(int slot, int row) {
    return slot ^ ((row >> 3) & 7);
  }
  L l;
  ushort8 r[4];
  DEV_INLINE void init(int, int) {}
  DEV_INLINE void load(int tid, int base, int kb, ushort8 *) {
#pragma unroll
    for (int it = 0; it < 2; ++it) {
      int p = tid + it * 256;
      int k0 = (p >> 4) * 2;
      int col0 = (p & 15) * 8;
      r[it * 2] = l.load(kb + k0, base + col0);
      r[it * 2 + 1] = l.load(kb + k0 + 1, base + col0);
    }
  }
  DEV_INLINE void write(int tid, ushort8 *img) const {
    uint32_t *img32 = (uint32_t *)img;
#pragma unroll
    for (int it = 0; it < 2; ++it) {
      int p = tid + it * 256;
      int k0 = (p >> 4) * 2;
      int col0 = (p & 15) * 8;
      int slot = k0 >> 3, within = (k0 & 7) >> 1;
      const ushort8 &va = r[it * 2], &vb = r[it * 2 + 1];
#pragma unroll
      for (int j = 0; j < 8; ++j) {
        int row = col0 + j;
        img32[row * (MXP * 4) + rslot(slot, row) * 4 + within] =
            (uint32_t)va[j] | ((uint32_t)vb[j] << 16);
      }
    }
  }
};

struct GldsNt {
  static constexpr int PITCH = 8;
  static constexpr bool GLDS = true;
  static DEV_INLINE int rslot(int slot, int row) { return slot ^ (row & 7); }
  const uint16_t *p;
  int rows;
  long ld;
  int kdim;
  DEV_INLINE void init(int, int) {}
  DEV_INLINE void load(int tid, int base, int kb, ushort8 *img) {
    int s_row = tid >> 3, s_slot = tid & 7;
#pragma unroll
    for (int i = 0; i < 4; ++i) {
      int row = base + s_row + 32 * i;
      int k = kb + (s_slot ^ (row & 7)) * 8;
      if (row < rows && k < kdim) {
        auto *dst = (__attribute__((address_space(3))) ushort8 *)(img + i * 256 + tid);
        __builtin_amdgcn_global_load_lds(
            (const __attribute__((address_space(1))) void *)(p + (long)row * ld + k),
            (__attribute__((address_space(3))) void *)dst, 16, 0, 0);
      } else {
        img[i * 256 + tid] = ushort8{0, 0, 0, 0, 0, 0, 0, 0};
      }
    }
  }
  DEV_INLINE void write(int, ushort8 *) const {}
};

typedef __attribute__((ext_vector_type(16))) float float16v;

struct LinearWriter {
  static constexpr bool ACC = false;
  static constexpr bool STATS = false;
  long ldc;
  typedef long RowCtx;
  DEV_INLINE RowCtx row_ctx(int row) const { return (long)row * ldc; }
  DEV_INLINE void store_f32(float *p, RowCtx b, int col, float v) const {
    p[b + col] = v;
  }
  DEV_INLINE void store_bf16(uint16_t *p, RowCtx b, int col, float v) const {
    p[b + col] = f2bf(v);
  }
};

struct BiasWriter {
  static constexpr bool ACC = false;
  static constexpr bool STATS = false;
  long ldc;
  const float *bias;
  typedef long RowCtx;
  DEV_INLINE RowCtx row_ctx(int row) const { return (long)row * ldc; }
  DEV_INLINE void store_f32(float *p, RowCtx b, int col, float v) const {
    p[b + col] = v + bias[col];
  }
  DEV_INLINE void store_bf16(uint16_t *p, RowCtx b, int col, float v) const {
    p[b + col] = f2bf(v + bias[col]);
  }
};

DEV_INLINE float tanh_fast(float u) {
  float a = __expf(-2.f * fabsf(u));
  float t = (1.f - a) / (1.f + a);
  return u < 0.f ? -t : t;
}
DEV_INLINE float gelu_f(float x) {
  float u = 0.7978845608028654f * (x + 0.044715f * x * x * x);
  return 0.5f * x * (1.f + tanh_fast(u));
}
DEV_INLINE float dgelu_f(float x) {
  float u = 0.7978845608028654f * (x + 0.044715f * x * x * x);
  float t = tanh_fast(u);
  return 0.5f * (1.f + t) +
         0.5f * x * (1.f - t * t) * 0.7978845608028654f *
             (1.f + 3.f * 0.044715f * x * x);
}
DEV_INLINE float gelu_pair_f(float x, float &dg) {
  float u = 0.7978845608028654f * (x + 0.044715f * x * x * x);
  float t = tanh_fast(u);
  dg = 0.5f * (1.f + t) +
       0.5f * x * (1.f - t * t) * 0.7978845608028654f *
           (1.f + 3.f * 0.044715f * x * x);
  return 0.5f * x * (1.f + t);
}

struct GeluBiasWriter {
  static constexpr bool ACC = false;
  static constexpr bool STATS = false;
  long ldc;
  const float *bias;
  uint16_t *deriv;
  typedef long RowCtx;
  DEV_INLINE RowCtx row_ctx(int row) const { return (long)row * ldc; }
  DEV_INLINE void store_f32(float *p, RowCtx b, int col, float v) const {
    float h = v + bias[col], dg;
    p[b + col] = gelu_pair_f(h, dg);
    deriv[b + col] = f2bf(dg);
  }
  DEV_INLINE void store_bf16(uint16_t *p, RowCtx b, int col, float v) const {
    float h = v + bias[col], dg;
    p[b + col] = f2bf(gelu_pair_f(h, dg));
    deriv[b + col] = f2bf(dg);
  }
};

struct GeluBwdWriter {
  static constexpr bool ACC = false;
  static constexpr bool STATS = false;
  long ldc;
  const uint16_t *deriv;
  typedef long RowCtx;
  DEV_INLINE RowCtx row_ctx(int row) const { return (long)row * ldc; }
  DEV_INLINE void store_f32(float *p, RowCtx b, int col, float v) const {
    p[b + col] = v * bf2f(deriv[b + col]);
  }
  DEV_INLINE void store_bf16(uint16_t *p, RowCtx b, int col, float v) const {
    p[b + col] = f2bf(v * bf2f(deriv[b + col]));
  }
};

struct GeluBiasPreWriter {
  static constexpr bool ACC = false;
  static constexpr bool STATS = false;
  long ldc;
  const float *bias;
  uint16_t *pre;
  typedef long RowCtx;
  DEV_INLINE RowCtx row_ctx(int row) const { return (long)row * ldc; }
  DEV_INLINE void store_f32(float *p, RowCtx b, int col, float v) const {
    float h = v + bias[col];
    pre[b + col] = f2bf(h);
    p[b + col] = gelu_f(h);
  }
  DEV_INLINE void store_bf16(uint16_t *p, RowCtx b, int col, float v) const {
    float h = v + bias[col];
    pre[b + col] = f2bf(h);
    p[b + col] = f2bf(gelu_f(h));
  }
};

struct GeluBwdPreWriter {
  static constexpr bool ACC = false;
  static constexpr bool STATS = false;
  long ldc;
  const uint16_t *pre;
  typedef long RowCtx;
  DEV_INLINE RowCtx row_ctx(int row) const { return (long)row * ldc; }
  DEV_INLINE void store_f32(float *p, RowCtx b, int col, float v) const {
    p[b + col] = v * dgelu_f(bf2f(pre[b + col]));
  }
  DEV_INLINE void store_bf16(uint16_t *p, RowCtx b, int col, float v) const {
    p[b + col] = f2bf(v * dgelu_f(bf2f(pre[b + col])));
  }
};

struct BnStatsWriter {
  static constexpr bool ACC = false;
  static constexpr bool STATS = true;
  long ldc;
  float *slab;
  int C;
  mutable float s0[2][2], s1[2][2];
  mutable int tm[2], colc[2];
  mutable int half_;
  typedef long RowCtx;
  DEV_INLINE void reset() const {
    s0[0][0] = s0[0][1] = s0[1][0] = s0[1][1] = 0.f;
    s1[0][0] = s1[0][1] = s1[1][0] = s1[1][1] = 0.f;
    tm[0] = tm[1] = -1;
    colc[0] = colc[1] = -1;
    half_ = 0;
  }
  DEV_INLINE RowCtx row_ctx(int row) const {
    half_ = (row >> 6) & 1;
    tm[half_] = row >> 6;
    return (long)row * ldc;
  }
  DEV_INLINE void store_f32(float *p, RowCtx b, int col, float v) const {
    p[b + col] = v;
  }
  DEV_INLINE void store_bf16(uint16_t *p, RowCtx b, int col, float v) const {
    uint16_t r = f2bf(v);
    p[b + col] = r;
    float vr = bf2f(r);
    int ci = (col >> 5) & 1;
    colc[ci] = col;
    s0[half_][ci] += vr;
    s1[half_][ci] += vr * vr;
  }
  DEV_INLINE void flush(int lane) const {
#pragma unroll
    for (int h = 0; h < 2; ++h) {
#pragma unroll
      for (int ci = 0; ci < 2; ++ci) {
        float a = s0[h][ci] + __shfl_xor(s0[h][ci], 32, 64);
        float b = s1[h][ci] + __shfl_xor(s1[h][ci], 32, 64);
        if (lane < 32 && tm[h] >= 0 && colc[ci] >= 0) {
          float *e = slab + (long)tm[h] * 2 * C;
          e[colc[ci]] = a;
          e[C + colc[ci]] = b;
        }
      }
    }
  }
};

struct LinearAccWriter {
  static constexpr bool ACC = true;
  static constexpr bool STATS = false;
  long ldc;
  typedef long RowCtx;
  DEV_INLINE RowCtx row_ctx(int row) const { return (long)row * ldc; }
  DEV_INLINE void store_f32(float *p, RowCtx b, int col, float v) const {
    p[b + col] += v;
  }
  DEV_INLINE void store_bf16(uint16_t *p, RowCtx b, int col, float v) const {
    p[b + col] = f2bf(v + bf2f(p[b + col]));
  }
};

struct Stride2Writer {
  static constexpr bool ACC = false;
  static constexpr bool STATS = false;
  int W2, H2, ph, pw, W, H, C;
  typedef long RowCtx;
  DEV_INLINE RowCtx row_ctx(int row) const {
    int w_ = row % W2;
    long t = row / W2;
    int h_ = (int)(t % H2);
    int n = (int)(t / H2);
    return (((long)n * H + 2 * h_ + ph) * W + 2 * w_ + pw) * (long)C;
  }
  DEV_INLINE void store_f32(float *p, RowCtx b, int col, float v) const {
    p[b + col] = v;
  }
  DEV_INLINE void store_bf16(uint16_t *p, RowCtx b, int col, float v) const {
    p[b + col] = f2bf(v);
  }
};

struct Stride2ZeroWriter {
  static constexpr bool ACC = false;
  static constexpr bool STATS = false;
  int W2, H2, ph, pw, W, H, C;
  struct RowCtx {
    long base;
    int sib;
  };
  DEV_INLINE RowCtx row_ctx(int row) const {
    int w_ = row % W2;
    long t = row / W2;
    int h_ = (int)(t % H2);
    int n = (int)(t / H2);
    int hh = 2 * h_ + ph, ww = 2 * w_ + pw;
    RowCtx c;
    c.base = (((long)n * H + hh) * W + ww) * (long)C;
    c.sib = (ww + 1 < W ? 1 : 0) | (hh + 1 < H ? 2 : 0);
    return c;
  }
  DEV_INLINE void store_f32(float *p, RowCtx c, int col, float v) const {
    p[c.base + col] = v;
  }
  DEV_INLINE void store_bf16(uint16_t *p, RowCtx c, int col, float v) const {
    p[c.base + col] = f2bf(v);
    if (c.sib & 1) p[c.base + C + col] = 0;
    if (c.sib & 2) {
      p[c.base + (long)W * C + col] = 0;
      if (c.sib & 1) p[c.base + (long)W * C + C + col] = 0;
    }
  }
};

template <class SA, class SB, bool C_F32, class WR = LinearWriter,
          bool ONEBUF = false>
__global__ __launch_bounds__(NT_THREADS) void mix_gemm_k(
    SA sa, SB sb, void *__restrict__ cptr, int M, int N, int K, WR wrt,
    int tiles_n, int kt_per_split, long split_stride, int xcd_cpx, int swap) {
  int tile = swap ? blockIdx.y : blockIdx.x;
  int split = swap ? blockIdx.x : blockIdx.y;
  if (xcd_cpx)
    tile = (tile & 7) * xcd_cpx + (tile >> 3);
  int tm = tile / tiles_n, tn = tile % tiles_n;
  int row0 = tm * BM, col0 = tn * BN;
  int tid = threadIdx.x;
  int lane = tid & 63, wave = tid >> 6;
  int wr = wave >> 1, wc = wave & 1;

  constexpr int ASZ = BM * SA::PITCH, BSZ = BM * SB::PITCH;
  constexpr int NBUF = ONEBUF ? 1 : 2;
  __shared__ ushort8 lds[NBUF * (ASZ + BSZ)];
#define MXG_A(b) (lds + ((b) % NBUF) * (ASZ + BSZ))
#define MXG_B(b) (lds + ((b) % NBUF) * (ASZ + BSZ) + ASZ)

  float16v acc[2][2] = {};

  int nk_total = (K + BK - 1) / BK;
  int t0 = split * kt_per_split;
  int nk = min(kt_per_split, nk_total - t0);
  if (nk < 0) nk = 0;

  sa.init(tid, row0);
  sb.init(tid, col0);
  if (nk > 0) {
    sa.load(tid, row0, t0 * BK, MXG_A(0));
    sb.load(tid, col0, t0 * BK, MXG_B(0));
    sa.write(tid, MXG_A(0));
    sb.write(tid, MXG_B(0));
  }
  __syncthreads();

  for (int t = 0; t < nk; ++t) {
    int buf = ONEBUF ? 0 : (t & 1);
    if (t + 1 < nk) {
      sa.load(tid, row0, (t0 + t + 1) * BK, MXG_A(buf ^ 1));
      sb.load(tid, col0, (t0 + t + 1) * BK, MXG_B(buf ^ 1));
    }
#pragma unroll
    for (int kk = 0; kk < BK / 16; ++kk) {
      bf16x8 af[2], bf_[2];
      int slot = kk * 2 + (lane >> 5);
#pragma unroll
      for (int mi = 0; mi < 2; ++mi) {
        int arow = wr * 64 + mi * 32 + (lane & 31);
        af[mi] = us8_to_bf8v(MXG_A(buf)[arow * SA::PITCH + SA::rslot(slot, arow)]);
      }
#pragma unroll
      for (int ni = 0; ni < 2; ++ni) {
        int brow = wc * 64 + ni * 32 + (lane & 31);
        bf_[ni] = us8_to_bf8v(MXG_B(buf)[brow * SB::PITCH + SB::rslot(slot, brow)]);
      }
#pragma unroll
      for (int mi = 0; mi < 2; ++mi)
#pragma unroll
        for (int ni = 0; ni < 2; ++ni)
          acc[mi][ni] = __builtin_amdgcn_mfma_f32_32x32x16_bf16(
              af[mi], bf_[ni], acc[mi][ni], 0, 0, 0);
    }
    if (ONEBUF) {
      if (t + 1 < nk) {
        __syncthreads();
        sa.write(tid, MXG_A(0));
        sb.write(tid, MXG_B(0));
      }
    } else if (t + 1 < nk) {
      sa.write(tid, MXG_A(buf ^ 1));
      sb.write(tid, MXG_B(buf ^ 1));
    }
    __syncthreads();
  }

  if constexpr (WR::STATS) wrt.reset();
  cptr = (void *)((char *)cptr + split * split_stride * (C_F32 ? 4 : 2));
#pragma unroll
  for (int mi = 0; mi < 2; ++mi) {
#pragma unroll
    for (int r = 0; r < 16; ++r) {
      int row = row0 + wr * 64 + mi * 32 + (r & 3) + 8 * (r >> 2) + 4 * (lane >> 5);
      if (row >= M) continue;
      typename WR::RowCtx rc = wrt.row_ctx(row);
#pragma unroll
      for (int ni = 0; ni < 2; ++ni) {
        int col = col0 + wc * 64 + ni * 32 + (lane & 31);
        if (col >= N) continue;
        if (C_F32)
          wrt.store_f32((float *)cptr, rc, col, acc[mi][ni][r]);
        else
          wrt.store_bf16((uint16_t *)cptr, rc, col, acc[mi][ni][r]);
      }
    }
  }
  if constexpr (WR::STATS) wrt.flush(lane);
}

#undef MXG_A
#undef MXG_B

template <class SA, class SB, class WR>
static hipError_t launch_mix_gemm_wr(const SA &sa, const SB &sb, void *c,
                                     int M, int N, int K, const WR &wrt,
                                     long ldc, bool c_f32, hipStream_t s,
                                     int splits = 1) {
  int tiles_m = (M + BM - 1) / BM, tiles_n = (N + BN - 1) / BN;
  int nk = (K + BK - 1) / BK;
  if (splits > nk) splits = nk > 0 ? nk : 1;
  int kts = (nk + splits - 1) / splits;
  long split_stride = (long)M * ldc;
  int nwg = tiles_m * tiles_n;
  static const int swap_env = [] {
    const char *e = getenv("MPIAMD_SPLITMAJOR");
    return e && e[0] == '1' ? 1 : 0;
  }();
  int swap = (splits > 1 && splits % 8 == 0) ? swap_env : 0;
  int cpx = (nwg % 8 == 0 && nwg >= 32 && (splits == 1 || swap)) ? nwg / 8 : 0;
  dim3 grid = swap ? dim3(splits, nwg) : dim3(nwg, splits);
  static const bool onebuf_env = [] {
    const char *e = getenv("MPIAMD_GEMM_ONEBUF");
    return e && e[0] == '1';
  }();
  const bool onebuf = onebuf_env && !SA::GLDS && !SB::GLDS;
  if (onebuf) {
    if (c_f32)
      mix_gemm_k<SA, SB, true, WR, true><<<grid, NT_THREADS, 0, s>>>(
          sa, sb, c, M, N, K, wrt, tiles_n, kts, split_stride, cpx, swap);
    else
      mix_gemm_k<SA, SB, false, WR, true><<<grid, NT_THREADS, 0, s>>>(
          sa, sb, c, M, N, K, wrt, tiles_n, kts, split_stride, cpx, swap);
    return hipGetLastError();
  }
  if (c_f32)
    mix_gemm_k<SA, SB, true, WR><<<grid, NT_THREADS, 0, s>>>(
        sa, sb, c, M, N, K, wrt, tiles_n, kts, split_stride, cpx, swap);
  else
    mix_gemm_k<SA, SB, false, WR><<<grid, NT_THREADS, 0, s>>>(
        sa, sb, c, M, N, K, wrt, tiles_n, kts, split_stride, cpx, swap);
  return hipGetLastError();
}

template <class SA, class SB>
static hipError_t launch_mix_gemm(const SA &sa, const SB &sb, void *c, int M,
                                  int N, int K, long ldc, bool c_f32,
                                  hipStream_t s, int splits = 1) {
  return launch_mix_gemm_wr(sa, sb, c, M, N, K, LinearWriter{ldc}, ldc, c_f32,
                            s, splits);
}

#include "gemm256.h"
#include "pipe256.h"
#include "pipe_mix.h"

template <class LA, class LB>
static hipError_t launch_nt_gemm(const LA &la, const LB &lb, void *c, int M,
                                 int N, int K, long ldc, bool c_f32,
                                 hipStream_t s, int splits = 1,
                                 const float *bias = nullptr) {
  static const bool use_256 = [] {
    const char *e = getenv("MPIAMD_GEMM256");
    return !(e && e[0] == '0');
  }();
  static const bool use_pipe = [] {
    const char *e = getenv("MPIAMD_PIPE");
    return !(e && e[0] == '0');
  }();
  if (use_256 && splits <= 1 && M % 256 == 0 && N % 256 == 0 && K % 32 == 0 &&
      K > 0 && la.kdim == K && lb.kdim == K && ldc == N &&
      (long)(M / 256) * (N / 256) >= 128) {
    if (use_pipe && K % 64 == 0)
      return launch_pipe256(la, lb, c, M, N, K, ldc, c_f32, s, bias);
    return launch_nt256(la, lb, c, M, N, K, ldc, c_f32, s, bias);
  }
  static const bool use_pipent = [] {
    const char *e = getenv("MPIAMD_PIPENT");
    return !(e && e[0] == '0');
  }();
  if (use_pipemix() && use_pipent) {
    NtPipe<PlainNtSrc> ga{{la.p, la.ld, la.rows, la.kdim}};
    NtPipe<PlainNtSrc> gb{{lb.p, lb.ld, lb.rows, lb.kdim}};
    if (bias)
      return launch_pipe_mix_wr(ga, gb, c, M, N, K, BiasWriter{ldc, bias},
                                ldc, c_f32, s, splits);
    return launch_pipe_mix_wr(ga, gb, c, M, N, K, LinearWriter{ldc}, ldc,
                              c_f32, s, splits);
  }
  static const bool use_glds = [] {
    const char *e = getenv("MPIAMD_GLDS");
    return !(e && e[0] == '0');
  }();
  if (use_glds) {
    GldsNt ga{la.p, la.rows, la.ld, la.kdim};
    GldsNt gb{lb.p, lb.rows, lb.ld, lb.kdim};
    if (bias)
      return launch_mix_gemm_wr(ga, gb, c, M, N, K, BiasWriter{ldc, bias},
                                ldc, c_f32, s, splits);
    return launch_mix_gemm(ga, gb, c, M, N, K, ldc, c_f32, s, splits);
  }
  if (bias)
    return launch_mix_gemm_wr(NtStage<LA>{la}, NtStage<LB>{lb}, c, M, N, K,
                              BiasWriter{ldc, bias}, ldc, c_f32, s, splits);
  return launch_mix_gemm(NtStage<LA>{la}, NtStage<LB>{lb}, c, M, N, K, ldc,
                         c_f32, s, splits);
}


struct TnRowMajor {
  const uint16_t *p;
  long ld;
  int kdim;
  int cols;
  DEV_INLINE ushort8 load(int k, int c0) const {
    if (k >= kdim || c0 >= cols) return ushort8{0, 0, 0, 0, 0, 0, 0, 0};
    if (c0 + 8 <= cols) return *(const ushort8 *)(p + (long)k * ld + c0);
    ushort8 v{0, 0, 0, 0, 0, 0, 0, 0};
#pragma unroll
    for (int j = 0; j < 8; ++j)
      if (c0 + j < cols) v[j] = p[(long)k * ld + c0 + j];
    return v;
  }
};
```

### mpi_operator_amd/ops/csrc/pipe256.h

```cpp
#pragma once


template <int SWZ> DEV_INLINE int p256_swz(int q, int row) {
  if (SWZ == 1) return q ^ ((row >> 2) & 3);
  if (SWZ == 2) return q ^ (row & 3);
  return q;
}

template <bool C_F32, bool BIAS, int SWZ = 1, int NPB = 2, int SP = 0,
          class WR = LinearWriter, bool USE_WR = false>
__global__ __launch_bounds__(512) void pipe256_gemm_k(
    const uint16_t *__restrict__ a, long lda, const uint16_t *__restrict__ b,
    long ldb, void *__restrict__ cptr, int M, int N, int K, long ldc,
    int tiles_n, int xcd_cpx, const float *__restrict__ bias,
    WR wrt = WR{}) {
  int tile = blockIdx.x;
  if (xcd_cpx) tile = (tile & 7) * xcd_cpx + (tile >> 3);
  int tm = tile / tiles_n, tn = tile % tiles_n;
  int row0 = tm * 256, col0 = tn * 256;
  int tid = threadIdx.x;
  int lane = tid & 63, wave = tid >> 6;
  int wr = wave >> 2, wc = wave & 3;

  constexpr int HSZ = 256 * 4;
  __shared__ ushort8 lds[8 * HSZ];
#define P256_IMG(buf, op, kh) (lds + (((buf) * 2 + (op)) * 2 + (kh)) * HSZ)

  if (USE_WR) {
    if constexpr (WR::STATS) wrt.reset();
  }
  float16v acc[4][2] = {};
  int nk = K / 64;

  const uint16_t *ap = a + (long)row0 * lda;
  const uint16_t *bp = b + (long)col0 * ldb;
  auto stage = [&](int t, int op, int kh) {
    const uint16_t *p = op ? bp : ap;
    long ld = op ? ldb : lda;
    ushort8 *img = P256_IMG(t & 1, op, kh);
    int kb = t * 64 + kh * 32;
#pragma unroll
    for (int i = 0; i < 2; ++i) {
      int idx = i * 512 + tid;
      int r = idx >> 2;
      int k = kb + p256_swz<SWZ>(idx & 3, r) * 8;
      __builtin_amdgcn_global_load_lds(
          (const __attribute__((address_space(1))) void *)(p + (long)r * ld + k),
          (__attribute__((address_space(3))) void *)(img + idx), 16, 0, 0);
    }
  };

  auto read_a = [&](bf16x8 af[2][2], int kh, int mh, int buf) {
#pragma unroll
    for (int mi = 0; mi < 2; ++mi)
#pragma unroll
      for (int kk = 0; kk < 2; ++kk) {
        int r = wr * 128 + (mh * 2 + mi) * 32 + (lane & 31);
        int q = kk * 2 + (lane >> 5);
        af[mi][kk] =
            us8_to_bf8v(P256_IMG(buf, 0, kh)[r * 4 + p256_swz<SWZ>(q, r)]);
      }
  };
  auto read_b = [&](bf16x8 bf_[2][2], int kh, int buf) {
#pragma unroll
    for (int ni = 0; ni < 2; ++ni)
#pragma unroll
      for (int kk = 0; kk < 2; ++kk) {
        int r = wc * 64 + ni * 32 + (lane & 31);
        int q = kk * 2 + (lane >> 5);
        bf_[ni][kk] =
            us8_to_bf8v(P256_IMG(buf, 1, kh)[r * 4 + p256_swz<SWZ>(q, r)]);
      }
  };

  if (nk > 0) {
    stage(0, 0, 0);
    stage(0, 1, 0);
    stage(0, 0, 1);
    stage(0, 1, 1);
    asm volatile("s_waitcnt vmcnt(4)" ::: "memory");
    __builtin_amdgcn_s_barrier();
  }

  if (SP == 1 && __builtin_amdgcn_readfirstlane(threadIdx.x) >= 256)
    __builtin_amdgcn_s_setprio(1);

  bf16x8 af[2][2], bf_[2][2];
  for (int t = 0; t < nk; ++t) {
    int buf = t & 1;
    bool pre = t + 1 < nk;
#pragma unroll
    for (int ph = 0; ph < 4; ++ph) {
      int kh = ph >> 1, mh = ph & 1;
      if (ph == 1 || ph == 3) {
        if (pre)
          asm volatile("s_waitcnt vmcnt(2)" ::: "memory");
        else
          asm volatile("s_waitcnt vmcnt(0)" ::: "memory");
      }
      if (mh == 0) read_b(bf_, kh, buf);
      read_a(af, kh, mh, buf);
      if (pre) stage(t + 1, ph & 1, ph >> 1);
      __builtin_amdgcn_s_barrier();
      asm volatile("s_waitcnt lgkmcnt(0)" ::: "memory");
      if (SP == 0) __builtin_amdgcn_s_setprio(1);
#pragma unroll
      for (int kk = 0; kk < 2; ++kk)
#pragma unroll
        for (int mi = 0; mi < 2; ++mi)
#pragma unroll
          for (int ni = 0; ni < 2; ++ni)
            acc[mh * 2 + mi][ni] = __builtin_amdgcn_mfma_f32_32x32x16_bf16(
                af[mi][kk], bf_[ni][kk], acc[mh * 2 + mi][ni], 0, 0, 0);
      if (SP == 0) __builtin_amdgcn_s_setprio(0);
      if (NPB == 2) __builtin_amdgcn_s_barrier();
    }
  }
  if (SP == 1) __builtin_amdgcn_s_setprio(0);
  asm volatile("s_waitcnt vmcnt(0)" ::: "memory");

#pragma unroll
  for (int mi = 0; mi < 4; ++mi) {
#pragma unroll
    for (int r = 0; r < 16; ++r) {
      long row = row0 + wr * 128 + mi * 32 + (r & 3) + 8 * (r >> 2) +
                 4 * (lane >> 5);
      if (USE_WR) {
        typename WR::RowCtx rc = wrt.row_ctx((int)row);
#pragma unroll
        for (int ni = 0; ni < 2; ++ni) {
          int col = col0 + wc * 64 + ni * 32 + (lane & 31);
          if (C_F32)
            wrt.store_f32((float *)cptr, rc, col, acc[mi][ni][r]);
          else
            wrt.store_bf16((uint16_t *)cptr, rc, col, acc[mi][ni][r]);
        }
        continue;
      }
      long base = row * ldc;
#pragma unroll
      for (int ni = 0; ni < 2; ++ni) {
        int col = col0 + wc * 64 + ni * 32 + (lane & 31);
        float v = BIAS ? acc[mi][ni][r] + bias[col] : acc[mi][ni][r];
        if (C_F32)
          ((float *)cptr)[base + col] = v;
        else
          ((uint16_t *)cptr)[base + col] = f2bf(v);
      }
    }
  }
  if (USE_WR) {
    if constexpr (WR::STATS) wrt.flush(lane);
  }
}
#undef P256_IMG

template <bool C_F32, bool BIAS, int SWZ = 1, int SP = 1,
          class WR = LinearWriter, bool USE_WR = false>
__global__ __launch_bounds__(1024) void pipe256x16_gemm_k(
    const uint16_t *__restrict__ a, long lda, const uint16_t *__restrict__ b,
    long ldb, void *__restrict__ cptr, int M, int N, int K, long ldc,
    int tiles_n, int xcd_cpx, const float *__restrict__ bias,
    WR wrt = WR{}) {
  int tile = blockIdx.x;
  if (xcd_cpx) tile = (tile & 7) * xcd_cpx + (tile >> 3);
  int tm = tile / tiles_n, tn = tile % tiles_n;
  int row0 = tm * 256, col0 = tn * 256;
  int tid = threadIdx.x;
  int lane = tid & 63, wave = tid >> 6;
  int wr = wave >> 2, wc = wave & 3;

  constexpr int HSZ = 256 * 4;
  __shared__ ushort8 lds[8 * HSZ];
#define P256X_IMG(buf, op, kh) (lds + (((buf) * 2 + (op)) * 2 + (kh)) * HSZ)

  if (USE_WR) {
    if constexpr (WR::STATS) wrt.reset();
  }
  float16v acc[2][2] = {};
  int nk = K / 64;

  const uint16_t *ap = a + (long)row0 * lda;
  const uint16_t *bp = b + (long)col0 * ldb;
  auto stage = [&](int t, int op, int kh) {
    const uint16_t *p = op ? bp : ap;
    long ld = op ? ldb : lda;
    ushort8 *img = P256X_IMG(t & 1, op, kh);
    int kb = t * 64 + kh * 32;
    int r = tid >> 2;
    int k = kb + p256_swz<SWZ>(tid & 3, r) * 8;
    __builtin_amdgcn_global_load_lds(
        (const __attribute__((address_space(1))) void *)(p + (long)r * ld + k),
        (__attribute__((address_space(3))) void *)(img + tid), 16, 0, 0);
  };

  auto read_a = [&](bf16x8 af[2], int kh, int mh, int buf) {
#pragma unroll
    for (int kk = 0; kk < 2; ++kk) {
      int r = wr * 64 + mh * 32 + (lane & 31);
      int q = kk * 2 + (lane >> 5);
      af[kk] = us8_to_bf8v(P256X_IMG(buf, 0, kh)[r * 4 + p256_swz<SWZ>(q, r)]);
    }
  };
  auto read_b = [&](bf16x8 bf_[2][2], int kh, int buf) {
#pragma unroll
    for (int ni = 0; ni < 2; ++ni)
#pragma unroll
      for (int kk = 0; kk < 2; ++kk) {
        int r = wc * 64 + ni * 32 + (lane & 31);
        int q = kk * 2 + (lane >> 5);
        bf_[ni][kk] =
            us8_to_bf8v(P256X_IMG(buf, 1, kh)[r * 4 + p256_swz<SWZ>(q, r)]);
      }
  };

  if (nk > 0) {
    stage(0, 0, 0);
    stage(0, 1, 0);
    stage(0, 0, 1);
    stage(0, 1, 1);
    asm volatile("s_waitcnt vmcnt(2)" ::: "memory");
    __builtin_amdgcn_s_barrier();
  }

  if (SP == 1 && __builtin_amdgcn_readfirstlane(threadIdx.x) >= 512)
    __builtin_amdgcn_s_setprio(1);

  bf16x8 af[2], bf_[2][2];
  for (int t = 0; t < nk; ++t) {
    int buf = t & 1;
    bool pre = t + 1 < nk;
#pragma unroll
    for (int ph = 0; ph < 4; ++ph) {
      int kh = ph >> 1, mh = ph & 1;
      if (ph == 1 || ph == 3) {
        if (pre)
          asm volatile("s_waitcnt vmcnt(1)" ::: "memory");
        else
          asm volatile("s_waitcnt vmcnt(0)" ::: "memory");
      }
      if (mh == 0) read_b(bf_, kh, buf);
      read_a(af, kh, mh, buf);
      if (pre) stage(t + 1, ph & 1, ph >> 1);
      __builtin_amdgcn_s_barrier();
      asm volatile("s_waitcnt lgkmcnt(0)" ::: "memory");
#pragma unroll
      for (int kk = 0; kk < 2; ++kk)
#pragma unroll
        for (int ni = 0; ni < 2; ++ni)
          acc[mh][ni] = __builtin_amdgcn_mfma_f32_32x32x16_bf16(
              af[kk], bf_[ni][kk], acc[mh][ni], 0, 0, 0);
    }
  }
  if (SP == 1) __builtin_amdgcn_s_setprio(0);
  asm volatile("s_waitcnt vmcnt(0)" ::: "memory");

#pragma unroll
  for (int mh = 0; mh < 2; ++mh) {
#pragma unroll
    for (int r = 0; r < 16; ++r) {
      long row = row0 + wr * 64 + mh * 32 + (r & 3) + 8 * (r >> 2) +
                 4 * (lane >> 5);
      if (USE_WR) {
        typename WR::RowCtx rc = wrt.row_ctx((int)row);
#pragma unroll
        for (int ni = 0; ni < 2; ++ni) {
          int col = col0 + wc * 64 + ni * 32 + (lane & 31);
          if (C_F32)
            wrt.store_f32((float *)cptr, rc, col, acc[mh][ni][r]);
          else
            wrt.store_bf16((uint16_t *)cptr, rc, col, acc[mh][ni][r]);
        }
        continue;
      }
      long base = row * ldc;
#pragma unroll
      for (int ni = 0; ni < 2; ++ni) {
        int col = col0 + wc * 64 + ni * 32 + (lane & 31);
        float v = BIAS ? acc[mh][ni][r] + bias[col] : acc[mh][ni][r];
        if (C_F32)
          ((float *)cptr)[base + col] = v;
        else
          ((uint16_t *)cptr)[base + col] = f2bf(v);
      }
    }
  }
  if (USE_WR) {
    if constexpr (WR::STATS) wrt.flush(lane);
  }
}
#undef P256X_IMG

static inline bool use_p256x16() {
  static const bool on = [] {
    const char *e = getenv("MPIAMD_P256X16");
    return !(e && e[0] == '0');
  }();
  return on;
}

template <class WR, class LA, class LB>
static hipError_t launch_pipe256_wr(const LA &la, const LB &lb, void *c,
                                    int M, int N, int K, long ldc, bool c_f32,
                                    const WR &wrt, hipStream_t s) {
  int tiles_m = M / 256, tiles_n = N / 256;
  int nwg = tiles_m * tiles_n;
  int cpx = (nwg % 8 == 0 && nwg >= 32) ? nwg / 8 : 0;
  constexpr int SWZ = 1, NPB = 1, SP = 1;
  if (use_p256x16()) {
    if (c_f32)
      pipe256x16_gemm_k<true, false, SWZ, SP, WR, true><<<nwg, 1024, 0, s>>>(
          la.p, la.ld, lb.p, lb.ld, c, M, N, K, ldc, tiles_n, cpx, nullptr,
          wrt);
    else
      pipe256x16_gemm_k<false, false, SWZ, SP, WR, true><<<nwg, 1024, 0, s>>>(
          la.p, la.ld, lb.p, lb.ld, c, M, N, K, ldc, tiles_n, cpx, nullptr,
          wrt);
    return hipGetLastError();
  }
  if (c_f32)
    pipe256_gemm_k<true, false, SWZ, NPB, SP, WR, true><<<nwg, 512, 0, s>>>(
        la.p, la.ld, lb.p, lb.ld, c, M, N, K, ldc, tiles_n, cpx, nullptr, wrt);
  else
    pipe256_gemm_k<false, false, SWZ, NPB, SP, WR, true><<<nwg, 512, 0, s>>>(
        la.p, la.ld, lb.p, lb.ld, c, M, N, K, ldc, tiles_n, cpx, nullptr, wrt);
  return hipGetLastError();
}

template <class LA, class LB>
static hipError_t launch_pipe256(const LA &la, const LB &lb, void *c, int M,
                                 int N, int K, long ldc, bool c_f32,
                                 hipStream_t s, const float *bias = nullptr) {
  int tiles_m = M / 256, tiles_n = N / 256;
  int nwg = tiles_m * tiles_n;
  int cpx = (nwg % 8 == 0 && nwg >= 32) ? nwg / 8 : 0;
  constexpr int SWZ = 1, NPB = 1, SP = 1;
  if (use_p256x16()) {
    if (c_f32) {
      if (bias)
        pipe256x16_gemm_k<true, true, SWZ, SP><<<nwg, 1024, 0, s>>>(
            la.p, la.ld, lb.p, lb.ld, c, M, N, K, ldc, tiles_n, cpx, bias);
      else
        pipe256x16_gemm_k<true, false, SWZ, SP><<<nwg, 1024, 0, s>>>(
            la.p, la.ld, lb.p, lb.ld, c, M, N, K, ldc, tiles_n, cpx, bias);
    } else {
      if (bias)
        pipe256x16_gemm_k<false, true, SWZ, SP><<<nwg, 1024, 0, s>>>(
            la.p, la.ld, lb.p, lb.ld, c, M, N, K, ldc, tiles_n, cpx, bias);
      else
        pipe256x16_gemm_k<false, false, SWZ, SP><<<nwg, 1024, 0, s>>>(
            la.p, la.ld, lb.p, lb.ld, c, M, N, K, ldc, tiles_n, cpx, bias);
    }
    return hipGetLastError();
  }
  if (c_f32) {
    if (bias)
      pipe256_gemm_k<true, true, SWZ, NPB, SP><<<nwg, 512, 0, s>>>(
          la.p, la.ld, lb.p, lb.ld, c, M, N, K, ldc, tiles_n, cpx, bias);
    else
      pipe256_gemm_k<true, false, SWZ, NPB, SP><<<nwg, 512, 0, s>>>(
          la.p, la.ld, lb.p, lb.ld, c, M, N, K, ldc, tiles_n, cpx, bias);
  } else {
    if (bias)
      pipe256_gemm_k<false, true, SWZ, NPB, SP><<<nwg, 512, 0, s>>>(
          la.p, la.ld, lb.p, lb.ld, c, M, N, K, ldc, tiles_n, cpx, bias);
    else
      pipe256_gemm_k<false, false, SWZ, NPB, SP><<<nwg, 512, 0, s>>>(
          la.p, la.ld, lb.p, lb.ld, c, M, N, K, ldc, tiles_n, cpx, bias);
  }
  return hipGetLastError();
}
```

### mpi_operator_amd/ops/csrc/pipe_mix.h

```cpp
#pragma once

#include <mutex>


typedef __attribute__((ext_vector_type(2))) unsigned int uint2v_pm;

static inline bool use_pipemix() {
  static const bool on = [] {
    const char *e = getenv("MPIAMD_PIPEMIX");
    return !(e && e[0] == '0');
  }();
  return on;
}

static inline bool use_pipegather() {
  static const bool on = [] {
    const char *e = getenv("MPIAMD_PIPEGATHER");
    return !(e && e[0] == '0');
  }();
  return use_pipemix() && on;
}

static inline bool use_pipegather_wgrad() {
  static const bool on = [] {
    const char *e = getenv("MPIAMD_PIPEGATHER_WGRAD");
    return !(e && e[0] == '0');
  }();
  return (use_pipemix() && on) || use_pipegather();
}


struct PlainNtSrc {
  const uint16_t *p;
  long ld;
  int rows, kdim;
  const uint16_t *base_[2];
  int koff_[2];
  DEV_INLINE void init(int i, int rc, int koff) {
    base_[i] = rc < rows ? p + (long)rc * ld + koff : nullptr;
    koff_[i] = koff;
  }
  DEV_INLINE const uint16_t *ptr16(int i, int kb) const {
    return (base_[i] && kb + koff_[i] < kdim) ? base_[i] + kb : nullptr;
  }
};

struct PlainTnSrc {
  const uint16_t *p;
  long ld;
  int kdim, cols;
  const uint16_t *base_[2];
  int koff_[2];
  DEV_INLINE void init(int i, int rc, int koff) {
    base_[i] = rc < cols ? p + (long)koff * ld + rc : nullptr;
    koff_[i] = koff;
  }
  DEV_INLINE const uint16_t *ptr16(int i, int kb) const {
    return (base_[i] && kb + koff_[i] < kdim) ? base_[i] + (long)kb * ld
                                              : nullptr;
  }
};

DEV_INLINE int ilog2_if_pow2(int v) {
  return (v & (v - 1)) == 0 ? (31 - __builtin_clz(v)) : -1;
}
DEV_INLINE int div_small(int num, int recip16) {
  return (num * recip16) >> 16;
}

struct ConvFwdSrc {
  const uint16_t *x;
  int H, W, C, HO, WO, S, stride, pad, K;
  long M;
  long nbase_[2];
  int hb_[2], wb_[2], koff_[2];
  int csh_, srecip_;
  bool ok_[2];
  DEV_INLINE void init(int i, int rc, int koff) {
    long m = rc;
    ok_[i] = m < M;
    int wo = (int)(m % WO);
    long t = m / WO;
    int ho = (int)(t % HO);
    int n = (int)(t / HO);
    nbase_[i] = (long)n * H * W;
    hb_[i] = ho * stride - pad;
    wb_[i] = wo * stride - pad;
    koff_[i] = koff;
    csh_ = ilog2_if_pow2(C);
    srecip_ = (1 << 16) / S + 1;
  }
  DEV_INLINE const uint16_t *ptr16(int i, int kb) const {
    int k = kb + koff_[i];
    int c, rs;
    if (csh_ >= 0) {
      c = k & (C - 1);
      rs = k >> csh_;
    } else {
      c = k % C;
      rs = k / C;
    }
    int rr = div_small(rs, srecip_);
    int s_ = rs - rr * S;
    int h = hb_[i] + rr, w = wb_[i] + s_;
    if (k < K && ok_[i] && (unsigned)h < (unsigned)H && (unsigned)w < (unsigned)W)
      return x + (nbase_[i] + (long)h * W + w) * C + c;
    return nullptr;
  }
};

template <int STRIDE> struct ConvDgradSrc {
  const uint16_t *dy;
  int H, W, Q, HO, WO, S, pad, K;
  long M;
  long nbase_[2];
  int hb_[2], wb_[2], koff_[2];
  int qsh_, srecip_;
  bool ok_[2];
  DEV_INLINE void init(int i, int rc, int koff) {
    long m = rc;
    ok_[i] = m < M;
    int w_ = (int)(m % W);
    long t = m / W;
    int h_ = (int)(t % H);
    int n = (int)(t / H);
    nbase_[i] = (long)n * HO * WO;
    hb_[i] = h_ + pad;
    wb_[i] = w_ + pad;
    koff_[i] = koff;
    qsh_ = ilog2_if_pow2(Q);
    srecip_ = (1 << 16) / S + 1;
  }
  DEV_INLINE const uint16_t *ptr16(int i, int kb) const {
    int k = kb + koff_[i];
    int q, rs;
    if (qsh_ >= 0) {
      q = k & (Q - 1);
      rs = k >> qsh_;
    } else {
      q = k % Q;
      rs = k / Q;
    }
    int rr = div_small(rs, srecip_);
    int s_ = rs - rr * S;
    int hn = hb_[i] - rr, wn = wb_[i] - s_;
    int ho = hn / STRIDE, wo = wn / STRIDE;
    if (k < K && ok_[i] && hn >= 0 && wn >= 0 &&
        (STRIDE == 1 || (hn % STRIDE == 0 && wn % STRIDE == 0)) && ho < HO &&
        wo < WO)
      return dy + (nbase_[i] + (long)ho * WO + wo) * Q + q;
    return nullptr;
  }
};

struct DgradWTnSrc {
  const uint16_t *w;
  int C, Q, K, RSC;
  int col_[2], koff_[2];
  DEV_INLINE void init(int i, int rc, int koff) {
    col_[i] = rc;
    koff_[i] = koff;
  }
  DEV_INLINE const uint16_t *ptr16(int i, int kb) const {
    int k = kb + koff_[i];
    if (k >= K || col_[i] >= C) return nullptr;
    int q = k % Q, rs = k / Q;
    return w + (long)q * RSC + rs * C + col_[i];
  }
};

struct DgradS2Src {
  const uint16_t *dy;
  int HO, WO, Q, W2, H2, K;
  long M;
  int dh0, dw0, nth, ntw;
  long nbase_[2];
  int hb_[2], wb_[2], koff_[2];
  bool ok_[2];
  int qsh_, ntwrecip_;
  DEV_INLINE void init(int i, int rc, int koff) {
    long m = rc;
    ok_[i] = m < M;
    int w_ = (int)(m % W2);
    long t = m / W2;
    int h_ = (int)(t % H2);
    int n = (int)(t / H2);
    nbase_[i] = (long)n * HO * WO;
    hb_[i] = h_;
    wb_[i] = w_;
    koff_[i] = koff;
    qsh_ = ilog2_if_pow2(Q);
    ntwrecip_ = (1 << 16) / ntw + 1;
  }
  DEV_INLINE const uint16_t *ptr16(int i, int kb) const {
    int k = kb + koff_[i];
    int q, ti;
    if (qsh_ >= 0) {
      q = k & (Q - 1);
      ti = k >> qsh_;
    } else {
      q = k % Q;
      ti = k / Q;
    }
    int ih = div_small(ti, ntwrecip_);
    int iw = ti - ih * ntw;
    int ho = hb_[i] + dh0 - ih, wo = wb_[i] + dw0 - iw;
    if (k < K && ok_[i] && (unsigned)ho < (unsigned)HO &&
        (unsigned)wo < (unsigned)WO)
      return dy + (nbase_[i] + (long)ho * WO + wo) * Q + q;
    return nullptr;
  }
};

struct DgradWS2TnSrc {
  const uint16_t *w;
  int C, Q, K, RSC, S, r0, s0, nth, ntw;
  int col_[2], koff_[2];
  int qsh_, ntwrecip_;
  DEV_INLINE void init(int i, int rc, int koff) {
    col_[i] = rc;
    koff_[i] = koff;
    qsh_ = ilog2_if_pow2(Q);
    ntwrecip_ = (1 << 16) / ntw + 1;
  }
  DEV_INLINE const uint16_t *ptr16(int i, int kb) const {
    int k = kb + koff_[i];
    if (k >= K || col_[i] >= C) return nullptr;
    int q, ti;
    if (qsh_ >= 0) {
      q = k & (Q - 1);
      ti = k >> qsh_;
    } else {
      q = k % Q;
      ti = k / Q;
    }
    int ih = div_small(ti, ntwrecip_);
    int iw = ti - ih * ntw;
    return w + (long)q * RSC + ((r0 + 2 * ih) * S + s0 + 2 * iw) * C + col_[i];
  }
};

struct XcolSrc {
  const uint16_t *x;
  int H, W, C, HO, WO, S, stride, pad, RSC;
  long M;
  int rr_[2], ss_[2], coff_[2], koff_[2];
  mutable long mcur_[2];
  mutable int n_[2], ho_[2], wo_[2];
  int dho_, dwo_;
  bool cok_[2];
  DEV_INLINE void init(int i, int rc, int koff) {
    cok_[i] = rc < RSC;
    int c = rc % C, rs = rc / C;
    ss_[i] = rs % S;
    rr_[i] = rs / S;
    coff_[i] = c;
    koff_[i] = koff;
    mcur_[i] = -1;
    dho_ = 32 / WO;
    dwo_ = 32 % WO;
  }
  DEV_INLINE const uint16_t *ptr16(int i, int kb) const {
    long m = kb + koff_[i];
    if (mcur_[i] != m) {
      wo_[i] = (int)(m % WO);
      long t = m / WO;
      ho_[i] = (int)(t % HO);
      n_[i] = (int)(t / HO);
    }
    const uint16_t *out = nullptr;
    if (m < M && cok_[i]) {
      int h = ho_[i] * stride + rr_[i] - pad, w = wo_[i] * stride + ss_[i] - pad;
      if ((unsigned)h < (unsigned)H && (unsigned)w < (unsigned)W)
        out = x + ((long)(n_[i] * H + h) * W + w) * C + coff_[i];
    }
    int wo = wo_[i] + dwo_, ho = ho_[i] + dho_;
    if (wo >= WO) {
      wo -= WO;
      ++ho;
    }
    while (ho >= HO) {
      ho -= HO;
      ++n_[i];
    }
    wo_[i] = wo;
    ho_[i] = ho;
    mcur_[i] = m + 32;
    return out;
  }
};

constexpr int PM_BM = 128, PM_BK = 64;
constexpr int PM_THREADS = 256;
constexpr int PM_HSZ = 512;

DEV_INLINE int pm_swz(int q, int row) { return q ^ ((row >> 2) & 3); }

template <class SRC> struct NtPipe {
  static constexpr bool TR = false;
  SRC s;
  DEV_INLINE void init(int tid, int base) {
#pragma unroll
    for (int i = 0; i < 2; ++i) {
      int idx = i * PM_THREADS + tid;
      int row = idx >> 2;
      s.init(i, base + row, pm_swz(idx & 3, row) * 8);
    }
  }
  DEV_INLINE void stage(int tid, int kb, ushort8 *img,
                        const uint16_t *zeros) const {
#pragma unroll
    for (int i = 0; i < 2; ++i) {
      int idx = i * PM_THREADS + tid;
      const uint16_t *src = s.ptr16(i, kb);
      __builtin_amdgcn_global_load_lds(
          (const __attribute__((address_space(1))) void *)(src ? src : zeros),
          (__attribute__((address_space(3))) void *)(img + idx), 16, 0, 0);
    }
  }
  DEV_INLINE bf16x8 read(const ushort8 *img, int lane, int frag0, int ks) const {
    int row = frag0 + (lane & 31);
    int q = ks * 2 + (lane >> 5);
    return us8_to_bf8v(img[row * 4 + pm_swz(q, row)]);
  }
};

template <class SRC> struct TnPipe {
  static constexpr bool TR = true;
  SRC s;
  DEV_INLINE void init(int tid, int base) {
#pragma unroll
    for (int i = 0; i < 2; ++i) {
      int idx = i * PM_THREADS + tid;
      int st = idx >> 3;
      int kq = st >> 3, cq = st & 7;
      int kl = (idx & 7) >> 1, ch = idx & 1;
      s.init(i, base + cq * 16 + ch * 8, kq * 4 + kl);
    }
  }
  DEV_INLINE void stage(int tid, int kb, ushort8 *img,
                        const uint16_t *zeros) const {
#pragma unroll
    for (int i = 0; i < 2; ++i) {
      int idx = i * PM_THREADS + tid;
      const uint16_t *src = s.ptr16(i, kb);
      __builtin_amdgcn_global_load_lds(
          (const __attribute__((address_space(1))) void *)(src ? src : zeros),
          (__attribute__((address_space(3))) void *)(img + idx), 16, 0, 0);
    }
  }
  DEV_INLINE bf16x8 read(const ushort8 *img, int lane, int frag0, int ks) const {
    unsigned base = (unsigned)(unsigned long)(
        __attribute__((address_space(3))) const void *)img;
    int kq0 = ks * 4 + ((lane >> 5) & 1) * 2;
    int cq = (frag0 >> 4) + ((lane >> 4) & 1);
    unsigned a0 = base + (unsigned)((kq0 * 8 + cq) * 128 + (lane & 15) * 8);
    uint2v_pm lo, hi;
    asm volatile("ds_read_b64_tr_b16 %0, %2\n\t"
                 "ds_read_b64_tr_b16 %1, %2 offset:1024\n\t"
                 "s_waitcnt lgkmcnt(0)"
                 : "=&v"(lo), "=&v"(hi)
                 : "v"(a0)
                 : "memory");
    union { unsigned u[4]; bf16x8 v; } r;
    r.u[0] = lo.x; r.u[1] = lo.y; r.u[2] = hi.x; r.u[3] = hi.y;
    return r.v;
  }
};

template <class SA, class SB, bool C_F32, class WR, int NPB = 1>
__global__ __launch_bounds__(PM_THREADS) void pipe_mix_k(
    SA sa, SB sb, void *__restrict__ cptr, int M, int N, int K, WR wrt,
    int tiles_n, int kt_per_split, long split_stride, int xcd_cpx, int swap,
    const uint16_t *__restrict__ zeros) {
  int tile = swap ? blockIdx.y : blockIdx.x;
  int split = swap ? blockIdx.x : blockIdx.y;
  if (xcd_cpx) tile = (tile & 7) * xcd_cpx + (tile >> 3);
  int tm = tile / tiles_n, tn = tile % tiles_n;
  int row0 = tm * PM_BM, col0 = tn * PM_BM;
  int tid = threadIdx.x;
  int lane = tid & 63, wave = tid >> 6;
  int wr = wave >> 1, wc = wave & 1;

  __shared__ __align__(128) ushort8 lds[8 * PM_HSZ];
  if constexpr (WR::STATS) wrt.reset();
#define PM_IMG(buf, op, kh) (lds + (((buf) * 2 + (op)) * 2 + (kh)) * PM_HSZ)

  float16v acc[2][2] = {};

  int nk_total = (K + PM_BK - 1) / PM_BK;
  int t0 = split * kt_per_split;
  int nk = min(kt_per_split, nk_total - t0);
  if (nk < 0) nk = 0;

  sa.init(tid, row0);
  sb.init(tid, col0);
  auto stage_half = [&](int t, int kh) {
    int kb = (t0 + t) * PM_BK + kh * 32;
    sa.stage(tid, kb, PM_IMG(t & 1, 0, kh), zeros);
    sb.stage(tid, kb, PM_IMG(t & 1, 1, kh), zeros);
  };

  if (nk > 0) {
    stage_half(0, 0);
    stage_half(0, 1);
    if (nk > 1) {
      stage_half(1, 0);
      stage_half(1, 1);
      asm volatile("s_waitcnt vmcnt(8)" ::: "memory");
    } else {
      asm volatile("s_waitcnt vmcnt(0)" ::: "memory");
    }
    __builtin_amdgcn_s_barrier();
  }

  for (int t = 0; t < nk; ++t) {
    int buf = t & 1;
#pragma unroll
    for (int kh = 0; kh < 2; ++kh) {
      if (t > 0 || kh > 0) {
        bool steady = (kh == 0) ? (t + 1 < nk) : (t + 2 < nk);
        if (steady)
          asm volatile("s_waitcnt vmcnt(4)" ::: "memory");
        else
          asm volatile("s_waitcnt vmcnt(0)" ::: "memory");
      }
      bf16x8 af[2][2], bf_[2][2];
#pragma unroll
      for (int ks = 0; ks < 2; ++ks) {
#pragma unroll
        for (int mi = 0; mi < 2; ++mi)
          af[mi][ks] = sa.read(PM_IMG(buf, 0, kh), lane, wr * 64 + mi * 32, ks);
#pragma unroll
        for (int ni = 0; ni < 2; ++ni)
          bf_[ni][ks] = sb.read(PM_IMG(buf, 1, kh), lane, wc * 64 + ni * 32, ks);
      }
      if (kh == 0) {
        if (t > 0 && t + 1 < nk) stage_half(t + 1, 1);
      } else {
        if (t + 2 < nk) stage_half(t + 2, 0);
      }
      __builtin_amdgcn_s_barrier();
      asm volatile("s_waitcnt lgkmcnt(0)" ::: "memory");
      __builtin_amdgcn_s_setprio(1);
#pragma unroll
      for (int ks = 0; ks < 2; ++ks)
#pragma unroll
        for (int mi = 0; mi < 2; ++mi)
#pragma unroll
          for (int ni = 0; ni < 2; ++ni)
            acc[mi][ni] = __builtin_amdgcn_mfma_f32_32x32x16_bf16(
                af[mi][ks], bf_[ni][ks], acc[mi][ni], 0, 0, 0);
      __builtin_amdgcn_s_setprio(0);
      if (NPB == 2) __builtin_amdgcn_s_barrier();
    }
  }
  asm volatile("s_waitcnt vmcnt(0)" ::: "memory");

  cptr = (void *)((char *)cptr + split * split_stride * (C_F32 ? 4 : 2));
#pragma unroll
  for (int mi = 0; mi < 2; ++mi) {
#pragma unroll
    for (int r = 0; r < 16; ++r) {
      int row = row0 + wr * 64 + mi * 32 + (r & 3) + 8 * (r >> 2) + 4 * (lane >> 5);
      if (row >= M) continue;
      typename WR::RowCtx rc = wrt.row_ctx(row);
#pragma unroll
      for (int ni = 0; ni < 2; ++ni) {
        int col = col0 + wc * 64 + ni * 32 + (lane & 31);
        if (col >= N) continue;
        if (C_F32)
          wrt.store_f32((float *)cptr, rc, col, acc[mi][ni][r]);
        else
          wrt.store_bf16((uint16_t *)cptr, rc, col, acc[mi][ni][r]);
      }
    }
  }
  if constexpr (WR::STATS) wrt.flush(lane);
}
#undef PM_IMG

inline const uint16_t *pm_zeros_page() {
  static std::mutex mu;
  static uint16_t *pages[64] = {};
  int dev = 0;
  hipGetDevice(&dev);
  if (!pages[dev]) {
    std::lock_guard<std::mutex> lk(mu);
    if (!pages[dev]) {
      void *p = nullptr;
      if (hipMalloc(&p, 256) != hipSuccess) return nullptr;
      hipMemset(p, 0, 256);
      pages[dev] = (uint16_t *)p;
    }
  }
  return pages[dev];
}

template <class SRC> struct Nt8Pipe;
template <class SRC> struct Tn8Pipe;
template <class P> struct Pipe8Of;
template <class S> struct Pipe8Of<NtPipe<S>> { using type = Nt8Pipe<S>; };
template <class S> struct Pipe8Of<TnPipe<S>> { using type = Tn8Pipe<S>; };
static inline bool use_pipe8();
template <class SA8, class SB8, class WR>
static hipError_t launch_pipe_mix8_wr(const SA8 &sa, const SB8 &sb, void *c,
                                      int M, int N, int K, const WR &wrt,
                                      long ldc, bool c_f32, hipStream_t s,
                                      int splits);

template <class SA, class SB, class WR>
static hipError_t launch_pipe_mix_wr(const SA &sa, const SB &sb, void *c,
                                     int M, int N, int K, const WR &wrt,
                                     long ldc, bool c_f32, hipStream_t s,
                                     int splits = 1) {
  if constexpr (!WR::STATS) {
    if (use_pipe8())
      return launch_pipe_mix8_wr(typename Pipe8Of<SA>::type{sa.s},
                                 typename Pipe8Of<SB>::type{sb.s}, c, M, N,
                                 K, wrt, ldc, c_f32, s, splits);
  }
  const uint16_t *zeros = pm_zeros_page();
  if (!zeros) return hipErrorOutOfMemory;
  int tiles_m = (M + PM_BM - 1) / PM_BM, tiles_n = (N + PM_BM - 1) / PM_BM;
  int nk = (K + PM_BK - 1) / PM_BK;
  if (splits > nk) splits = nk > 0 ? nk : 1;
  int kts = (nk + splits - 1) / splits;
  long split_stride = (long)M * ldc;
  int nwg = tiles_m * tiles_n;
  static const bool sk_cpx = [] {
    const char *e = getenv("MPIAMD_SK_CPX");
    return !(e && e[0] == '0');
  }();
  int cpx = (nwg % 8 == 0 && nwg >= 32 && (splits == 1 || sk_cpx))
                ? nwg / 8 : 0;
  dim3 grid(nwg, splits);
  if (c_f32)
    pipe_mix_k<SA, SB, true, WR><<<grid, PM_THREADS, 0, s>>>(
        sa, sb, c, M, N, K, wrt, tiles_n, kts, split_stride, cpx, 0, zeros);
  else
    pipe_mix_k<SA, SB, false, WR><<<grid, PM_THREADS, 0, s>>>(
        sa, sb, c, M, N, K, wrt, tiles_n, kts, split_stride, cpx, 0, zeros);
  return hipGetLastError();
}


template <class SRC> struct Nt8Pipe {
  static constexpr bool TR = false;
  SRC s;
  DEV_INLINE void init(int tid, int base) {
    int row = tid >> 2;
    s.init(0, base + row, pm_swz(tid & 3, row) * 8);
  }
  DEV_INLINE void stage(int tid, int kb, ushort8 *img,
                        const uint16_t *zeros) const {
    const uint16_t *src = s.ptr16(0, kb);
    __builtin_amdgcn_global_load_lds(
        (const __attribute__((address_space(1))) void *)(src ? src : zeros),
        (__attribute__((address_space(3))) void *)(img + tid), 16, 0, 0);
  }
  DEV_INLINE bf16x8 read(const ushort8 *img, int lane, int frag0, int ks) const {
    int row = frag0 + (lane & 31);
    int q = ks * 2 + (lane >> 5);
    return us8_to_bf8v(img[row * 4 + pm_swz(q, row)]);
  }
};

template <class SRC> struct Tn8Pipe {
  static constexpr bool TR = true;
  SRC s;
  DEV_INLINE void init(int tid, int base) {
    int st = tid >> 3;
    int kq = st >> 3, cq = st & 7;
    int kl = (tid & 7) >> 1, ch = tid & 1;
    s.init(0, base + cq * 16 + ch * 8, kq * 4 + kl);
  }
  DEV_INLINE void stage(int tid, int kb, ushort8 *img,
                        const uint16_t *zeros) const {
    const uint16_t *src = s.ptr16(0, kb);
    __builtin_amdgcn_global_load_lds(
        (const __attribute__((address_space(1))) void *)(src ? src : zeros),
        (__attribute__((address_space(3))) void *)(img + tid), 16, 0, 0);
  }
  DEV_INLINE bf16x8 read(const ushort8 *img, int lane, int frag0, int ks) const {
    unsigned base = (unsigned)(unsigned long)(
        __attribute__((address_space(3))) const void *)img;
    int kq0 = ks * 4 + ((lane >> 5) & 1) * 2;
    int cq = (frag0 >> 4) + ((lane >> 4) & 1);
    unsigned a0 = base + (unsigned)((kq0 * 8 + cq) * 128 + (lane & 15) * 8);
    uint2v_pm lo, hi;
    asm volatile("ds_read_b64_tr_b16 %0, %2\n\t"
                 "ds_read_b64_tr_b16 %1, %2 offset:1024\n\t"
                 "s_waitcnt lgkmcnt(0)"
                 : "=&v"(lo), "=&v"(hi)
                 : "v"(a0)
                 : "memory");
    union { unsigned u[4]; bf16x8 v; } r;
    r.u[0] = lo.x; r.u[1] = lo.y; r.u[2] = hi.x; r.u[3] = hi.y;
    return r.v;
  }
};

template <class SA, class SB, bool C_F32, class WR>
__global__ __launch_bounds__(512) void pipe_mix8_k(
    SA sa, SB sb, void *__restrict__ cptr, int M, int N, int K, WR wrt,
    int tiles_n, int kt_per_split, long split_stride, int xcd_cpx, int swap,
    const uint16_t *__restrict__ zeros) {
  int tile = swap ? blockIdx.y : blockIdx.x;
  int split = swap ? blockIdx.x : blockIdx.y;
  if (xcd_cpx) tile = (tile & 7) * xcd_cpx + (tile >> 3);
  int tm = tile / tiles_n, tn = tile % tiles_n;
  int row0 = tm * PM_BM, col0 = tn * PM_BM;
  int tid = threadIdx.x;
  int lane = tid & 63, wave = tid >> 6;
  int wr = wave >> 2, wc = wave & 3;

  __shared__ __align__(128) ushort8 lds[8 * PM_HSZ];
  if constexpr (WR::STATS) wrt.reset();
#define PM8_IMG(buf, op, kh) (lds + (((buf) * 2 + (op)) * 2 + (kh)) * PM_HSZ)

  float16v acc[2] = {};

  int nk_total = (K + PM_BK - 1) / PM_BK;
  int t0 = split * kt_per_split;
  int nk = min(kt_per_split, nk_total - t0);
  if (nk < 0) nk = 0;

  sa.init(tid, row0);
  sb.init(tid, col0);
  auto stage_half = [&](int t, int kh) {
    int kb = (t0 + t) * PM_BK + kh * 32;
    sa.stage(tid, kb, PM8_IMG(t & 1, 0, kh), zeros);
    sb.stage(tid, kb, PM8_IMG(t & 1, 1, kh), zeros);
  };

  if (nk > 0) {
    stage_half(0, 0);
    stage_half(0, 1);
    if (nk > 1) {
      stage_half(1, 0);
      stage_half(1, 1);
      asm volatile("s_waitcnt vmcnt(4)" ::: "memory");
    } else {
      asm volatile("s_waitcnt vmcnt(0)" ::: "memory");
    }
    __builtin_amdgcn_s_barrier();
  }

  for (int t = 0; t < nk; ++t) {
    int buf = t & 1;
#pragma unroll
    for (int kh = 0; kh < 2; ++kh) {
      if (t > 0 || kh > 0) {
        bool steady = (kh == 0) ? (t + 1 < nk) : (t + 2 < nk);
        if (steady)
          asm volatile("s_waitcnt vmcnt(2)" ::: "memory");
        else
          asm volatile("s_waitcnt vmcnt(0)" ::: "memory");
      }
      bf16x8 af[2][2], bf_[2];
#pragma unroll
      for (int ks = 0; ks < 2; ++ks) {
#pragma unroll
        for (int mi = 0; mi < 2; ++mi)
          af[mi][ks] = sa.read(PM8_IMG(buf, 0, kh), lane, wr * 64 + mi * 32, ks);
        bf_[ks] = sb.read(PM8_IMG(buf, 1, kh), lane, wc * 32, ks);
      }
      if (kh == 0) {
        if (t > 0 && t + 1 < nk) stage_half(t + 1, 1);
      } else {
        if (t + 2 < nk) stage_half(t + 2, 0);
      }
      __builtin_amdgcn_s_barrier();
      asm volatile("s_waitcnt lgkmcnt(0)" ::: "memory");
      __builtin_amdgcn_s_setprio(1);
#pragma unroll
      for (int ks = 0; ks < 2; ++ks)
#pragma unroll
        for (int mi = 0; mi < 2; ++mi)
          acc[mi] = __builtin_amdgcn_mfma_f32_32x32x16_bf16(
              af[mi][ks], bf_[ks], acc[mi], 0, 0, 0);
      __builtin_amdgcn_s_setprio(0);
    }
  }
  asm volatile("s_waitcnt vmcnt(0)" ::: "memory");

  cptr = (void *)((char *)cptr + split * split_stride * (C_F32 ? 4 : 2));
#pragma unroll
  for (int mi = 0; mi < 2; ++mi) {
#pragma unroll
    for (int r = 0; r < 16; ++r) {
      int row = row0 + wr * 64 + mi * 32 + (r & 3) + 8 * (r >> 2) + 4 * (lane >> 5);
      if (row >= M) continue;
      typename WR::RowCtx rc = wrt.row_ctx(row);
      int col = col0 + wc * 32 + (lane & 31);
      if (col >= N) continue;
      if (C_F32)
        wrt.store_f32((float *)cptr, rc, col, acc[mi][r]);
      else
        wrt.store_bf16((uint16_t *)cptr, rc, col, acc[mi][r]);
    }
  }
}
#undef PM8_IMG

static inline bool use_pipe8() {
  static const bool on = [] {
    const char *e = getenv("MPIAMD_PIPE8");
    return !(e && e[0] == '0');
  }();
  return on;
}

template <class SA8, class SB8, class WR>
static hipError_t launch_pipe_mix8_wr(const SA8 &sa, const SB8 &sb, void *c,
                                      int M, int N, int K, const WR &wrt,
                                      long ldc, bool c_f32, hipStream_t s,
                                      int splits) {
  const uint16_t *zeros = pm_zeros_page();
  if (!zeros) return hipErrorOutOfMemory;
  int tiles_m = (M + PM_BM - 1) / PM_BM, tiles_n = (N + PM_BM - 1) / PM_BM;
  int nk = (K + PM_BK - 1) / PM_BK;
  if (splits > nk) splits = nk > 0 ? nk : 1;
  int kts = (nk + splits - 1) / splits;
  long split_stride = (long)M * ldc;
  int nwg = tiles_m * tiles_n;
  int cpx = (nwg % 8 == 0 && nwg >= 32) ? nwg / 8 : 0;
  dim3 grid(nwg, splits);
  if (c_f32)
    pipe_mix8_k<SA8, SB8, true, WR><<<grid, 512, 0, s>>>(
        sa, sb, c, M, N, K, wrt, tiles_n, kts, split_stride, cpx, 0, zeros);
  else
    pipe_mix8_k<SA8, SB8, false, WR><<<grid, 512, 0, s>>>(
        sa, sb, c, M, N, K, wrt, tiles_n, kts, split_stride, cpx, 0, zeros);
  return hipGetLastError();
}
```

### mpi_operator_amd/ops/fused_block.py

```python
from __future__ import annotations

import torch

from ._backend import hip_ext

import os as _os

_FUSEBN = _os.environ.get("MPIAMD_FUSEBN", "0") == "1"

_EMPTY = None


def _empty():
    global _EMPTY
    if _EMPTY is None:
        _EMPTY = torch.empty(0)
    return _EMPTY


class BottleneckFn(torch.autograd.Function):
    @staticmethod
    def forward(ctx, x, stride, eps, momentum,
                w1, g1, b1, rm1, rv1,
                w2, g2, b2, rm2, rv2,
                w3, g3, b3, rm3, rv3,
                wd, gd, bd, rmd, rvd):
        ext = hip_ext()
        e = _empty()

        def conv_bn(xin, w, st, pad, g, b, eps_, relu, rm, rv, mom, res):
            if not _FUSEBN:
                a = ext.conv2d_fwd(xin, w, st, pad)
                y, m, v, mk = ext.bn_fwd_train(a, g, b, eps_, relu, rm, rv,
                                               mom, res)
                return a, y, m, v, mk
            a, slab = ext.conv2d_fwd_bn(xin, w, st, pad)
            if slab.numel() > 0:
                y, m, v, mk = ext.bn_fwd_train_pre(a, slab, g, b, eps_, relu,
                                                   rm, rv, mom, res)
            else:
                y, m, v, mk = ext.bn_fwd_train(a, g, b, eps_, relu, rm, rv,
                                               mom, res)
            return a, y, m, v, mk

        a1, y1, m1, v1, mk1 = conv_bn(x, w1, 1, 0, g1, b1, eps, True, rm1,
                                      rv1, momentum, e)
        a2, y2, m2, v2, mk2 = conv_bn(y1, w2, stride, 1, g2, b2, eps, True,
                                      rm2, rv2, momentum, e)
        has_ds = wd is not None
        if has_ds:
            ad, res, md, vd, _ = conv_bn(x, wd, stride, 0, gd, bd, eps,
                                         False, rmd, rvd, momentum, e)
        else:
            ad = res = md = vd = None
        a3, out, m3, v3, mk3 = conv_bn(y2, w3, 1, 0, g3, b3, eps, True, rm3,
                                       rv3, momentum, res if has_ds else x)
        saved = [x, a1, y1, a2, y2, a3, out, m1, v1, m2, v2, m3, v3,
                 w1, g1, w2, g2, w3, g3, mk1, mk2, mk3]
        if has_ds:
            saved += [ad, md, vd, wd, gd]
        ctx.save_for_backward(*saved)
        ctx.stride = stride
        ctx.has_ds = has_ds
        return out

    @staticmethod
    def backward(ctx, dout):
        ext = hip_ext()
        st = ctx.stride
        (x, a1, y1, a2, y2, a3, out, m1, v1, m2, v2, m3, v3,
         w1, g1, w2, g2, w3, g3, mk1, mk2, mk3) = ctx.saved_tensors[:22]
        if ctx.has_ds:
            ad, md, vd, wd, gd = ctx.saved_tensors[22:]

        dout = dout.contiguous(memory_format=torch.channels_last)
        dx3, dg3, db3 = ext.bn_bwd(dout, a3, out, g3, m3, v3, True, mk3)
        dw3 = ext.conv2d_wgrad(y2, dx3, 1, 1, 1, 0)
        dy2 = ext.conv2d_dgrad(dx3, w3, y2.shape[2], y2.shape[3], 1, 0)
        dx2, dg2, db2 = ext.bn_bwd(dy2, a2, y2, g2, m2, v2, True, mk2)
        dw2 = ext.conv2d_wgrad(y1, dx2, 3, 3, st, 1)
        dy1 = ext.conv2d_dgrad(dx2, w2, y1.shape[2], y1.shape[3], st, 1)
        dx1, dg1, db1 = ext.bn_bwd(dy1, a1, y1, g1, m1, v1, True, mk1)
        dw1 = ext.conv2d_wgrad(x, dx1, 1, 1, 1, 0)

        dx0 = ext.conv2d_dgrad(dx1, w1, x.shape[2], x.shape[3], 1, 0)
        if ctx.has_ds:
            dad, dgd, dbd = ext.bn_bwd(dout, ad, out, gd, md, vd, True, mk3)
            dwd = ext.conv2d_wgrad(x, dad, 1, 1, st, 0)
            skip = ext.conv2d_dgrad(dad, wd, x.shape[2], x.shape[3], st, 0)
            dxt = ext.add_bf16(skip, dx0)
        else:
            dwd = dgd = dbd = None
            dxt = ext.add_relu_bwd_add_mask(dout, mk3, dx0)

        f32 = torch.float32
        return (dxt, None, None, None,
                dw1, dg1.to(f32), db1.to(f32), None, None,
                dw2, dg2.to(f32), db2.to(f32), None, None,
                dw3, dg3.to(f32), db3.to(f32), None, None,
                dwd, dgd.to(f32) if dgd is not None else None,
                dbd.to(f32) if dbd is not None else None, None, None)


def fused_bottleneck(x, block):
    ds = block.downsample
    if ds is not None:
        wd, bnd = ds[0].weight, ds[1]
        args = (wd, bnd.weight, bnd.bias, bnd.running_mean, bnd.running_var)
    else:
        args = (None, None, None, None, None)
    return BottleneckFn.apply(
        x, block.conv2.stride, block.bn1.eps, block.bn1.momentum,
        block.conv1.weight, block.bn1.weight, block.bn1.bias,
        block.bn1.running_mean, block.bn1.running_var,
        block.conv2.weight, block.bn2.weight, block.bn2.bias,
        block.bn2.running_mean, block.bn2.running_var,
        block.conv3.weight, block.bn3.weight, block.bn3.bias,
        block.bn3.running_mean, block.bn3.running_var,
        *args)
```

Measured before the change: 3859 images/sec.

## Fuse BN statistics into split-K conv reduction and dgrad epilogues

Fused conv+BN-stats is now on by default. The split-K reduction kernel also accumulates per-channel BN partial sums (forward mean/var, backward dbeta/dgamma terms) while it writes the bf16 output, so the separate BN partials pass that re-reads the activation is skipped. Conv dgrad gets a matching fused path that feeds bn_bwd_pre, and the GEMM writers gain stats slots so the pipe8 path can be used with stats. This adds code paths and numeric differences from summing after bf16 rounding, and it risks slower kernels where the fused reduction lowers occupancy.

```diff
diff --git a/mpi_operator_amd/ops/csrc/batchnorm.hip b/mpi_operator_amd/ops/csrc/batchnorm.hip
--- a/mpi_operator_amd/ops/csrc/batchnorm.hip
+++ b/mpi_operator_amd/ops/csrc/batchnorm.hip
@@ -96,6 +96,148 @@
       p1[j] = a1[j];
     }
   }
+}
+
+DEV_INLINE void bn_acc_fwd(float *a0, float *a1, const float *fx,
+                           const float *fx2) {
+#pragma unroll
+  for (int j = 0; j < 8; ++j) {
+    a0[j] += fx[j] + fx2[j];
+    a1[j] += fx[j] * fx[j] + fx2[j] * fx2[j];
+  }
+}
+
+DEV_INLINE void bn_acc_bwd(float *a0, float *a1, const float *fx,
+                           const float *fx2, float *fdy, float *fdy2,
+                           const ushort8 *__restrict__ y,
+                           const uint8_t *__restrict__ mask, long off,
+                           long off2, bool has2, int relu, const float *mn,
+                           const float *is) {
+  if (relu) {
+    if (mask) {
+      int m1 = mask[off], m2 = has2 ? mask[off2] : 0;
+#pragma unroll
+      for (int j = 0; j < 8; ++j) {
+        if (!(m1 & (1 << j))) fdy[j] = 0.f;
+        if (!(m2 & (1 << j))) fdy2[j] = 0.f;
+      }
+    } else {
+      ushort8 vy = y[off];
+      ushort8 vy2 = has2 ? y[off2] : ushort8{0, 0, 0, 0, 0, 0, 0, 0};
+#pragma unroll
+      for (int j = 0; j < 8; ++j) {
+        if (!(bf2f(vy[j]) > 0.f)) fdy[j] = 0.f;
+        if (!(bf2f(vy2[j]) > 0.f)) fdy2[j] = 0.f;
+      }
+    }
+  }
+#pragma unroll
+  for (int j = 0; j < 8; ++j) {
+    a0[j] += fdy[j] + fdy2[j];
+    float xh = __fmul_rn(__fsub_rn(fx[j], mn[j]), is[j]);
+    float xh2 = __fmul_rn(__fsub_rn(fx2[j], mn[j]), is[j]);
+    a1[j] = __fadd_rn(a1[j], __fmaf_rn(fdy[j], xh, __fmul_rn(fdy2[j], xh2)));
+  }
+}
+
+DEV_INLINE void bn_block_store(float *a0, float *a1,
+                               float *__restrict__ partial, int C8, int cb,
+                               int row_lane, int rows_per_block) {
+  int C = C8 * 8;
+  __shared__ float lds[2][256 * 8];
+#pragma unroll
+  for (int j = 0; j < 8; ++j) {
+    lds[0][threadIdx.x * 8 + j] = a0[j];
+    lds[1][threadIdx.x * 8 + j] = a1[j];
+  }
+  __syncthreads();
+  if (row_lane == 0) {
+    for (int rl = 1; rl < rows_per_block; ++rl) {
+#pragma unroll
+      for (int j = 0; j < 8; ++j) {
+        a0[j] += lds[0][(rl * C8 + cb) * 8 + j];
+        a1[j] += lds[1][(rl * C8 + cb) * 8 + j];
+      }
+    }
+    float *p0 = partial + (long)blockIdx.x * 2 * C + cb * 8;
+    float *p1 = p0 + C;
+#pragma unroll
+    for (int j = 0; j < 8; ++j) {
+      p0[j] = a0[j];
+      p1[j] = a1[j];
+    }
+  }
+}
+
+template <int WHAT, int SPLITS>
+__global__ void bn_reduce_stats_k(const float4v *__restrict__ slabs,
+                                  int splits_rt, long len4,
+                                  ushort8 *__restrict__ out,
+                                  const ushort8 *__restrict__ x,
+                                  const ushort8 *__restrict__ y,
+                                  const uint8_t *__restrict__ mask,
+                                  const float *__restrict__ mean,
+                                  const float *__restrict__ invstd,
+                                  float *__restrict__ partial,
+                                  long M, int C8, int relu) {
+  int cb = threadIdx.x % C8;
+  int row_lane = threadIdx.x / C8;
+  int rows_per_block = blockDim.x / C8;
+  float a0[8] = {0}, a1[8] = {0};
+  float mn[8], is[8];
+  if (WHAT == 1 && row_lane < rows_per_block) {
+#pragma unroll
+    for (int j = 0; j < 8; ++j) {
+      mn[j] = mean[cb * 8 + j];
+      is[j] = invstd[cb * 8 + j];
+    }
+  }
+  if (row_lane < rows_per_block) {
+    long stride = (long)gridDim.x * rows_per_block;
+    for (long row = (long)blockIdx.x * rows_per_block + row_lane; row < M;
+         row += 2 * stride) {
+      long r2 = row + stride;
+      bool has2 = r2 < M;
+      long off = row * C8 + cb, off2 = r2 * C8 + cb;
+      float4v s0 = splitk_sum4<SPLITS>(slabs, splits_rt, len4, off * 2);
+      float4v s1 = splitk_sum4<SPLITS>(slabs, splits_rt, len4, off * 2 + 1);
+      float4v t0 = {0.f, 0.f, 0.f, 0.f}, t1 = {0.f, 0.f, 0.f, 0.f};
+      if (has2) {
+        t0 = splitk_sum4<SPLITS>(slabs, splits_rt, len4, off2 * 2);
+        t1 = splitk_sum4<SPLITS>(slabs, splits_rt, len4, off2 * 2 + 1);
+      }
+      ushort8 vo, vo2 = ushort8{0, 0, 0, 0, 0, 0, 0, 0};
+#pragma unroll
+      for (int j = 0; j < 4; ++j) {
+        vo[j] = f2bf(s0[j]);
+        vo[4 + j] = f2bf(s1[j]);
+      }
+      out[off] = vo;
+      if (has2) {
+#pragma unroll
+        for (int j = 0; j < 4; ++j) {
+          vo2[j] = f2bf(t0[j]);
+          vo2[4 + j] = f2bf(t1[j]);
+        }
+        out[off2] = vo2;
+      }
+      float fo[8], fo2[8];
+      bf8_to_f8(vo, fo);
+      bf8_to_f8(vo2, fo2);
+      if (WHAT == 0) {
+        bn_acc_fwd(a0, a1, fo, fo2);
+      } else {
+        float fx[8], fx2[8];
+        ushort8 vx = x[off];
+        ushort8 vx2 = has2 ? x[off2] : ushort8{0, 0, 0, 0, 0, 0, 0, 0};
+        bf8_to_f8(vx, fx);
+        bf8_to_f8(vx2, fx2);
+        bn_acc_bwd(a0, a1, fx, fx2, fo, fo2, y, mask, off, off2, has2, relu,
+                   mn, is);
+      }
+    }
+  }
+  bn_block_store(a0, a1, partial, C8, cb, row_lane, rows_per_block);
 }
 
 DEV_INLINE void lane8_sums(const float *__restrict__ partial, int grid, int C,
@@ -476,3 +618,75 @@
   HIP_KERNEL_CHECK();
   return hipSuccess;
 }
+
+extern "C" int bn_stats_grid(long M, int C) {
+  int grid, rpb;
+  bn_geom(M, C / 8, grid, rpb);
+  return grid;
+}
+
+#define BN_RS_DISPATCH(WHAT, ...)                                              \
+  do {                                                                         \
+    switch (splits) {                                                          \
+    case 2: bn_reduce_stats_k<WHAT, 2><<<grid, 256, 0, s>>>(__VA_ARGS__); break; \
+    case 3: bn_reduce_stats_k<WHAT, 3><<<grid, 256, 0, s>>>(__VA_ARGS__); break; \
+    case 4: bn_reduce_stats_k<WHAT, 4><<<grid, 256, 0, s>>>(__VA_ARGS__); break; \
+    case 5: bn_reduce_stats_k<WHAT, 5><<<grid, 256, 0, s>>>(__VA_ARGS__); break; \
+    case 6: bn_reduce_stats_k<WHAT, 6><<<grid, 256, 0, s>>>(__VA_ARGS__); break; \
+    case 8: bn_reduce_stats_k<WHAT, 8><<<grid, 256, 0, s>>>(__VA_ARGS__); break; \
+    case 16: bn_reduce_stats_k<WHAT, 16><<<grid, 256, 0, s>>>(__VA_ARGS__); break; \
+    default: bn_reduce_stats_k<WHAT, 0><<<grid, 256, 0, s>>>(__VA_ARGS__); break; \
+    }                                                                          \
+  } while (0)
+
+extern "C" hipError_t bn_reduce_stats_fwd_launch(const float *slabs,
+                                                 int splits, void *y,
+                                                 float *partial, long M, int C,
+                                                 hipStream_t s) {
+  int C8 = C / 8;
+  if (C8 < 1 || C8 > 256 || C % 8 != 0 || splits < 2)
+    return hipErrorInvalidValue;
+  int grid, rpb;
+  bn_geom(M, C8, grid, rpb);
+  long len4 = M * C / 4;
+  BN_RS_DISPATCH(0, (const float4v *)slabs, splits, len4, (ushort8 *)y,
+                 nullptr, nullptr, nullptr, nullptr, nullptr, partial, M, C8,
+                 0);
+  return hipGetLastError();
+}
+
+extern "C" hipError_t bn_reduce_stats_bwd_launch(
+    const float *slabs, int splits, void *dy, const void *x, const void *y,
+    const uint8_t *relu_mask, const float *mean, const float *invstd, int relu,
+    float *partial, long M, int C, hipStream_t s) {
+  int C8 = C / 8;
+  if (C8 < 1 || C8 > 256 || C % 8 != 0 || splits < 2)
+    return hipErrorInvalidValue;
+  int grid, rpb;
+  bn_geom(M, C8, grid, rpb);
+  long len4 = M * C / 4;
+  BN_RS_DISPATCH(1, (const float4v *)slabs, splits, len4, (ushort8 *)dy,
+                 (const ushort8 *)x, (const ushort8 *)y, relu_mask, mean,
+                 invstd, partial, M, C8, relu);
+  return hipGetLastError();
+}
+#undef BN_RS_DISPATCH
+
+extern "C" hipError_t bn_bwd_pre_launch(
+    const float *pre_partial, int pre_grid, const void *dy, const void *x,
+    const void *y, const uint8_t *relu_mask, const float *gamma,
+    const float *mean, const float *invstd, int relu, void *dx, float *dgamma,
+    float *dbeta, float *k1, float *k2, float *k3, long M, int C,
+    hipStream_t s) {
+  int C8 = C / 8;
+  if (C8 < 1 || C8 > 256) return hipErrorInvalidValue;
+  bn_finalize_bwd_bands_k<<<C, 256, 0, s>>>(pre_partial, pre_grid, C, gamma,
+                                            invstd, 1.f / (float)M, dbeta,
+                                            dgamma, k1, k2, k3);
+  HIP_KERNEL_CHECK();
+  bn_bwd_apply_k<<<bn_apply_grid(M, C8), 256, 0, s>>>(
+      (const ushort8 *)dy, (const ushort8 *)x, (const ushort8 *)y, relu_mask,
+      mean, invstd, k1, k2, k3, (ushort8 *)dx, M, C8, relu);
+  HIP_KERNEL_CHECK();
+  return hipSuccess;
+}
diff --git a/mpi_operator_amd/ops/csrc/bindings.cpp b/mpi_operator_amd/ops/csrc/bindings.cpp
--- a/mpi_operator_amd/ops/csrc/bindings.cpp
+++ b/mpi_operator_amd/ops/csrc/bindings.cpp
@@ -136,8 +136,20 @@
                       int, int, int, int, int, int, int, int, float *,
                       hipStream_t);
 hipError_t conv_fwd_bn(const void *, const void *, void *, int, int, int,
-                       int, int, int, int, int, int, int, int, float *,
-                       hipStream_t);
+                       int, int, int, int, int, int, int, int, int, float *,
+                       float *, hipStream_t);
+int conv_fwd_bn_rows(long, int, int, int, int, int, int, int);
+int conv_dgrad_bn_rows(long, int, int, int, int, int, int);
+hipError_t conv_dgrad_bn(const void *, const void *, void *, int, int, int,
+                         int, int, int, int, int, int, int, int, float *,
+                         const void *, const void *, const uint8_t *,
+                         const float *, const float *, int, float *,
+                         hipStream_t);
+hipError_t bn_bwd_pre_launch(const float *, int, const void *, const void *,
+                             const void *, const uint8_t *, const float *,
+                             const float *, const float *, int, void *,
+                             float *, float *, float *, float *, float *, long,
+                             int, hipStream_t);
 hipError_t bn_fwd_train_pre_launch(const float *, int, const void *,
                                    const void *, const float *, const float *,
                                    float, int, void *, uint8_t *, float *,
@@ -263,7 +275,9 @@
 }
 
 static std::vector<Tensor> conv2d_fwd_bn(const Tensor &x, const Tensor &w,
-                                         int64_t stride, int64_t pad) {
+                                         int64_t stride, int64_t pad,
+                                         bool fuse_splitk,
+                                         bool fuse_epilogue) {
   check_cl_bf16(x, "x");
   check_cl_bf16(w, "w");
   const HIPDeviceGuard guard(x.device());
@@ -274,17 +288,67 @@
   long M = (long)N * HO * WO;
   int splits = conv_splits(M, Kout, R * S * C);
   auto f32 = x.options().dtype(at::kFloat);
-  if (splits > 1 || Kout % 8 != 0) {
+  long rows = Kout % 8 != 0 ? 0
+                            : conv_fwd_bn_rows(M, C, Kout, R, S, (int)stride,
+                                               (int)pad, splits);
+  if (rows == 0 || (splits > 1 ? !fuse_splitk : !fuse_epilogue)) {
     Tensor y = conv2d_fwd(x, w, stride, pad);
     return {y, at::empty({0}, f32)};
   }
+  TORCH_CHECK(w.size(1) == C, "conv channel mismatch");
+  TORCH_CHECK(C % 8 == 0, "conv requires C%8==0 (pad the stem input)");
   Tensor y = empty_cl_bf16(N, Kout, HO, WO, x);
-  long bands = (M + 63) / 64;
-  Tensor slab = at::empty({bands, 2, (long)Kout}, f32);
+  Tensor slab = at::empty({rows, 2, (long)Kout}, f32);
+  Tensor partial;
+  float *pp = nullptr;
+  if (splits > 1) {
+    partial = at::empty({(long)splits, M, (long)Kout}, f32);
+    pp = partial.data_ptr<float>();
+  }
   CHK(conv_fwd_bn(x.data_ptr(), w.data_ptr(), y.data_ptr(), N, H, W, C, Kout,
-                  R, S, (int)stride, (int)pad, HO, WO,
+                  R, S, (int)stride, (int)pad, HO, WO, splits, pp,
                   slab.data_ptr<float>(), cur_stream()));
   return {y, slab};
+}
+
+static std::vector<Tensor> conv2d_dgrad_bn(
+    const Tensor &dy, const Tensor &w, int64_t H, int64_t W, int64_t stride,
+    int64_t pad, const Tensor &bx, const Tensor &by, const Tensor &mean,
+    const Tensor &invstd, bool relu, const Tensor &mask) {
+  check_cl_bf16(dy, "dy");
+  check_cl_bf16(w, "w");
+  const HIPDeviceGuard guard(dy.device());
+  int N = dy.size(0), Kout = dy.size(1), HO = dy.size(2), WO = dy.size(3);
+  int C = w.size(1), R = w.size(2), S = w.size(3);
+  long M = (long)N * H * W;
+  auto f32 = dy.options().dtype(at::kFloat);
+  int splits = stride == 1 ? conv_splits(M, C, R * S * Kout) : 1;
+  long rows = (Kout % 8 != 0 || C % 8 != 0)
+                  ? 0
+                  : conv_dgrad_bn_rows(M, C, Kout, R, S, (int)stride, splits);
+  if (rows == 0) return {conv2d_dgrad(dy, w, H, W, stride, pad), at::empty({0}, f32)};
+  check_cl_bf16(bx, "bx");
+  TORCH_CHECK(bx.size(0) == N && bx.size(1) == C && bx.size(2) == H &&
+                  bx.size(3) == W, "bx must have the dgrad output's shape");
+  TORCH_CHECK(mean.numel() == C && invstd.numel() == C, "mean/invstd shape");
+  const uint8_t *mp = nullptr;
+  if (mask.defined() && mask.numel() > 0) {
+    TORCH_CHECK(mask.numel() == M * (C / 8), "mask shape");
+    mp = mask.data_ptr<uint8_t>();
+  }
+  if (relu && !mp) {
+    check_cl_bf16(by, "by");
+    TORCH_CHECK(by.numel() == bx.numel(), "by shape");
+  }
+  Tensor dx = empty_cl_bf16(N, C, H, W, dy);
+  Tensor partial = at::empty({(long)splits, M, (long)C}, f32);
+  Tensor slab = at::empty({rows, 2, (long)C}, f32);
+  CHK(conv_dgrad_bn(dy.data_ptr(), w.data_ptr(), dx.data_ptr(), N, (int)H,
+                    (int)W, C, Kout, R, S, (int)pad, HO, WO, splits,
+                    partial.data_ptr<float>(), bx.data_ptr(),
+                    by.defined() && by.numel() > 0 ? by.data_ptr() : nullptr, mp, mean.data_ptr<float>(), invstd.data_ptr<float>(),
+                    relu ? 1 : 0, slab.data_ptr<float>(), cur_stream()));
+  return {dx, slab};
 }
 
 static std::vector<Tensor> bn_fwd_train_pre(
@@ -295,7 +359,9 @@
   const HIPDeviceGuard guard(x.device());
   int N = x.size(0), C = x.size(1), H = x.size(2), W = x.size(3);
   long M = (long)N * H * W;
-  TORCH_CHECK(slab.numel() == ((M + 63) / 64) * 2 * (long)C, "slab shape");
+  TORCH_CHECK(slab.dim() == 3 && slab.size(0) >= 1 && slab.size(1) == 2 &&
+                  slab.size(2) == C && slab.is_contiguous() &&
+                  slab.scalar_type() == at::kFloat, "slab must be [rows][2][C] fp32");
   auto f32 = x.options().dtype(at::kFloat);
   Tensor y = empty_cl_bf16(N, C, H, W, x);
   Tensor mean = at::empty({C}, f32), invstd = at::empty({C}, f32);
@@ -317,7 +383,7 @@
     mask = at::empty({0}, x.options().dtype(at::kByte));
   }
   CHK(bn_fwd_train_pre_launch(
-      slab.data_ptr<float>(), (int)((M + 63) / 64), x.data_ptr(), resp,
+      slab.data_ptr<float>(), (int)slab.size(0), x.data_ptr(), resp,
       gamma.data_ptr<float>(), beta.data_ptr<float>(), (float)eps,
       relu ? 1 : 0, y.data_ptr(), mp, mean.data_ptr<float>(),
       invstd.data_ptr<float>(), scale.data_ptr<float>(),
@@ -399,6 +465,35 @@
                     k1.data_ptr<float>(), k2.data_ptr<float>(),
                     k3.data_ptr<float>(), partial.data_ptr<float>(), M, C,
                     cur_stream()));
+  return {dx, dgamma, dbeta};
+}
+
+static std::vector<Tensor> bn_bwd_pre(const Tensor &dy, const Tensor &slab,
+                                      const Tensor &x, const Tensor &y,
+                                      const Tensor &gamma, const Tensor &mean,
+                                      const Tensor &invstd, bool relu,
+                                      const Tensor &mask) {
+  check_cl_bf16(dy, "dy");
+  check_cl_bf16(x, "x");
+  const HIPDeviceGuard guard(x.device());
+  int N = x.size(0), C = x.size(1), H = x.size(2), W = x.size(3);
+  long M = (long)N * H * W;
+  TORCH_CHECK(slab.dim() == 3 && slab.size(0) >= 1 && slab.size(1) == 2 &&
+                  slab.size(2) == C && slab.is_contiguous() &&
+                  slab.scalar_type() == at::kFloat, "slab must be [rows][2][C] fp32");
+  auto f32 = x.options().dtype(at::kFloat);
+  Tensor dx = empty_cl_bf16(N, C, H, W, x);
+  Tensor dgamma = at::empty({C}, f32), dbeta = at::empty({C}, f32);
+  Tensor k1 = at::empty({C}, f32), k2 = at::empty({C}, f32), k3 = at::empty({C}, f32);
+  const uint8_t *mp =
+      mask.defined() && mask.numel() > 0 ? mask.data_ptr<uint8_t>() : nullptr;
+  CHK(bn_bwd_pre_launch(slab.data_ptr<float>(), (int)slab.size(0),
+                        dy.data_ptr(), x.data_ptr(), y.data_ptr(), mp,
+                        gamma.data_ptr<float>(), mean.data_ptr<float>(),
+                        invstd.data_ptr<float>(), relu ? 1 : 0, dx.data_ptr(),
+                        dgamma.data_ptr<float>(), dbeta.data_ptr<float>(),
+                        k1.data_ptr<float>(), k2.data_ptr<float>(),
+                        k3.data_ptr<float>(), M, C, cur_stream()));
   return {dx, dgamma, dbeta};
 }
 
@@ -893,7 +988,11 @@
 PYBIND11_MODULE(TORCH_EXTENSION_NAME, m) {
   m.def("conv2d_fwd", &conv2d_fwd);
   m.def("conv2d_dgrad", &conv2d_dgrad);
-  m.def("conv2d_fwd_bn", &conv2d_fwd_bn);
+  m.def("conv2d_fwd_bn", &conv2d_fwd_bn, py::arg("x"), py::arg("w"),
+        py::arg("stride"), py::arg("pad"), py::arg("fuse_splitk") = true,
+        py::arg("fuse_epilogue") = true);
+  m.def("conv2d_dgrad_bn", &conv2d_dgrad_bn);
+  m.def("bn_bwd_pre", &bn_bwd_pre);
   m.def("bn_fwd_train_pre", &bn_fwd_train_pre);
   m.def("conv2d_wgrad", &conv2d_wgrad);
   m.def("conv2d_dgrad_acc", &conv2d_dgrad_acc);
diff --git a/mpi_operator_amd/ops/csrc/common.h b/mpi_operator_amd/ops/csrc/common.h
--- a/mpi_operator_amd/ops/csrc/common.h
+++ b/mpi_operator_amd/ops/csrc/common.h
@@ -52,7 +52,37 @@
   return v;
 }
 
-#define HIP_KERNEL_CHECK()                                                    \
+template <int SPLITS>
+DEV_INLINE float4v splitk_sum4(const float4v *__restrict__ partial,
+                               int splits_rt, long len4, long i) {
+  const int splits = SPLITS ? SPLITS : splits_rt;
+  float4v a = partial[i];
+  float4v b = {0.f, 0.f, 0.f, 0.f};
+  int s = 1;
+  if (SPLITS == 0) {
+    for (; s + 8 <= splits; s += 8) {
+      float4v c0 = {0.f, 0.f, 0.f, 0.f};
+      float4v c1 = {0.f, 0.f, 0.f, 0.f};
+#pragma unroll
+      for (int j = 0; j < 8; j += 2) {
+        c0 += partial[(long)(s + j) * len4 + i];
+        c1 += partial[(long)(s + j + 1) * len4 + i];
+      }
+      a += c0;
+      b += c1;
+    }
+  }
+#pragma unroll
+  for (; s + 1 < splits; s += 2) {
+    a += partial[(long)s * len4 + i];
+    b += partial[(long)(s + 1) * len4 + i];
+  }
+  if (s < splits) b += partial[(long)s * len4 + i];
+  a += b;
+  return a;
+}
+
+#define HIP_KERNEL_CHECK()                                                   \
   do {                                                                        \
     hipError_t e = hipGetLastError();                                         \
     if (e != hipSuccess) return e;                                            \
diff --git a/mpi_operator_amd/ops/csrc/conv.hip b/mpi_operator_amd/ops/csrc/conv.hip
--- a/mpi_operator_amd/ops/csrc/conv.hip
+++ b/mpi_operator_amd/ops/csrc/conv.hip
@@ -170,14 +170,16 @@
   }
 };
 
-extern "C" hipError_t conv_fwd(const void *x, const void *w, void *y, int N,
-                               int H, int W, int C, int Kout, int R, int S,
-                               int stride, int pad, int HO, int WO, int splits,
-                               float *partial, hipStream_t strm) {
+static hipError_t conv_fwd_impl(const void *x, const void *w, void *y, int N,
+                                int H, int W, int C, int Kout, int R, int S,
+                                int stride, int pad, int HO, int WO,
+                                int splits, float *partial, bool reduce,
+                                int *splits_out, hipStream_t strm) {
   long M = (long)N * HO * WO;
   int K = R * S * C;
   int nk = (K + BK - 1) / BK;
   if (splits > nk) splits = nk > 0 ? nk : 1;
+  if (splits_out) *splits_out = splits;
   void *out = splits > 1 ? (void *)partial : y;
   bool f32 = splits > 1;
   hipError_t e;
@@ -197,34 +199,85 @@
     e = launch_mix_gemm(sa, NtStage<GemmLoader>{lb}, out, (int)M, Kout, K,
                         Kout, f32, strm, splits);
   }
-  if (e != hipSuccess || splits <= 1) return e;
+  if (e != hipSuccess || splits <= 1 || !reduce) return e;
   return splitk_reduce(partial, splits, M * Kout, y, 1, strm);
+}
+
+extern "C" hipError_t conv_fwd(const void *x, const void *w, void *y, int N,
+                               int H, int W, int C, int Kout, int R, int S,
+                               int stride, int pad, int HO, int WO, int splits,
+                               float *partial, hipStream_t strm) {
+  return conv_fwd_impl(x, w, y, N, H, W, C, Kout, R, S, stride, pad, HO, WO,
+                       splits, partial, true, nullptr, strm);
+}
+
+extern "C" int bn_stats_grid(long M, int C);
+extern "C" hipError_t bn_reduce_stats_fwd_launch(const float *, int, void *,
+                                                 float *, long, int,
+                                                 hipStream_t);
+extern "C" hipError_t bn_reduce_stats_bwd_launch(
+    const float *, int, void *, const void *, const void *, const uint8_t *,
+    const float *, const float *, int, float *, long, int, hipStream_t);
+
+static bool conv_is_plain_1x1(int R, int S, int stride, int pad) {
+  return R == 1 && S == 1 && stride == 1 && pad == 0;
+}
+
+extern "C" int conv_fwd_bn_rows(long M, int C, int Kout, int R, int S,
+                                int stride, int pad, int splits) {
+  int K = R * S * C;
+  int nk = (K + BK - 1) / BK;
+  if (splits > nk) splits = nk > 0 ? nk : 1;
+  if (splits > 1) return bn_stats_grid(M, Kout);
+  if (conv_is_plain_1x1(R, S, stride, pad) &&
+      nt_gemm_route((int)M, Kout, C, Kout, C, C, 1) == NT_256)
+    return 0;
+  return (int)((M + 63) / 64);
 }
 
 extern "C" hipError_t conv_fwd_bn(const void *x, const void *w, void *y,
                                   int N, int H, int W, int C, int Kout, int R,
                                   int S, int stride, int pad, int HO, int WO,
-                                  float *bn_slab, hipStream_t strm) {
+                                  int splits, float *partial, float *bn_slab,
+                                  hipStream_t strm) {
   long M = (long)N * HO * WO;
   int K = R * S * C;
+  int nk = (K + BK - 1) / BK;
+  if (splits > nk) splits = nk > 0 ? nk : 1;
+  if (splits > 1) {
+    int sp = splits;
+    hipError_t e = conv_fwd_impl(x, w, y, N, H, W, C, Kout, R, S, stride, pad,
+                                 HO, WO, splits, partial, false, &sp, strm);
+    if (e != hipSuccess) return e;
+    return bn_reduce_stats_fwd_launch(partial, sp, y, bn_slab, M, Kout, strm);
+  }
   BnStatsWriter wrt{(long)Kout, bn_slab, Kout};
-  if (R == 1 && S == 1 && stride == 1 && pad == 0) {
+  if (conv_is_plain_1x1(R, S, stride, pad)) {
     GemmLoader la{(const uint16_t *)x, (int)M, (long)C, C};
     GemmLoader lb{(const uint16_t *)w, Kout, (long)C, C};
-    if (M % 256 == 0 && Kout % 256 == 0 && C % 64 == 0 &&
-        (long)(M / 256) * (Kout / 256) >= 128)
+    switch (nt_gemm_route((int)M, Kout, C, Kout, C, C, 1)) {
+    case NT_PIPE256:
       return launch_pipe256_wr(la, lb, y, (int)M, Kout, C, Kout, false, wrt,
                                strm);
-    if (use_pipemix()) {
+    case NT_256:
+      return hipErrorInvalidValue;
+    case NT_PIPEMIX: {
       NtPipe<PlainNtSrc> sa{{(const uint16_t *)x, (long)C, (int)M, C}};
       NtPipe<PlainNtSrc> sb{{(const uint16_t *)w, (long)C, Kout, C}};
       return launch_pipe_mix_wr(sa, sb, y, (int)M, Kout, C, wrt, Kout, false,
                                 strm);
     }
-    GldsNt ga{la.p, la.rows, la.ld, la.kdim};
-    GldsNt gb{lb.p, lb.rows, lb.ld, lb.kdim};
-    return launch_mix_gemm_wr(ga, gb, y, (int)M, Kout, C, wrt, Kout, false,
-                              strm);
+    case NT_GLDS: {
+      GldsNt ga{la.p, la.rows, la.ld, la.kdim};
+      GldsNt gb{lb.p, lb.rows, lb.ld, lb.kdim};
+      return launch_mix_gemm_wr(ga, gb, y, (int)M, Kout, C, wrt, Kout, false,
+                                strm);
+    }
+    default:
+      return launch_mix_gemm_wr(NtStage<GemmLoader>{la},
+                                NtStage<GemmLoader>{lb}, y, (int)M, Kout, C,
+                                wrt, Kout, false, strm);
+    }
   }
   if (use_pipegather()) {
     NtPipe<ConvFwdSrc> sa{
@@ -400,17 +453,18 @@
   return hipSuccess;
 }
 
-extern "C" hipError_t conv_dgrad(const void *dy, const void *w, void *dx,
-                                 int N, int H, int W, int C, int Kout, int R,
-                                 int S, int stride, int pad, int HO, int WO,
-                                 int splits, float *partial,
-                                 hipStream_t strm) {
+static hipError_t conv_dgrad_impl(const void *dy, const void *w, void *dx,
+                                  int N, int H, int W, int C, int Kout, int R,
+                                  int S, int stride, int pad, int HO, int WO,
+                                  int splits, float *partial, bool reduce,
+                                  int *splits_out, hipStream_t strm) {
   long M = (long)N * H * W;
   int K = R * S * Kout;
   if (stride != 1)
     return conv_dgrad_s2(dy, w, dx, N, H, W, C, Kout, R, S, pad, HO, WO, strm);
   int nk = (K + BK - 1) / BK;
   if (splits > nk) splits = nk > 0 ? nk : 1;
+  if (splits_out) *splits_out = splits;
   void *out = splits > 1 ? (void *)partial : dx;
   bool f32 = splits > 1;
   hipError_t e;
@@ -438,40 +492,54 @@
     e = launch_mix_gemm(sa, TnStage<DgradWTn>{lb}, out, (int)M, C, K, C, f32,
                         strm, splits);
   }
-  if (e != hipSuccess || splits <= 1) return e;
+  if (e != hipSuccess || splits <= 1 || !reduce) return e;
   return splitk_reduce(partial, splits, M * C, dx, 1, strm);
 }
+
+extern "C" hipError_t conv_dgrad(const void *dy, const void *w, void *dx,
+                                 int N, int H, int W, int C, int Kout, int R,
+                                 int S, int stride, int pad, int HO, int WO,
+                                 int splits, float *partial,
+                                 hipStream_t strm) {
+  return conv_dgrad_impl(dy, w, dx, N, H, W, C, Kout, R, S, stride, pad, HO,
+                         WO, splits, partial, true, nullptr, strm);
+}
+
+extern "C" int conv_dgrad_bn_rows(long M, int C, int Kout, int R, int S,
+                                  int stride, int splits) {
+  int K = R * S * Kout;
+  int nk = (K + BK - 1) / BK;
+  if (splits > nk) splits = nk > 0 ? nk : 1;
+  if (stride != 1 || splits <= 1) return 0;
+  return bn_stats_grid(M, C);
+}
+
+extern "C" hipError_t conv_dgrad_bn(const void *dy, const void *w, void *dx,
+                                    int N, int H, int W, int C, int Kout,
+                                    int R, int S, int pad, int HO, int WO,
+                                    int splits, float *partial, const void *bx,
+                                    const void *by, const uint8_t *mask,
+                                    const float *mean, const float *invstd,
+                                    int relu, float *bn_slab,
+                                    hipStream_t strm) {
+  long M = (long)N * H * W;
+  int sp = splits;
+  hipError_t e = conv_dgrad_impl(dy, w, dx, N, H, W, C, Kout, R, S, 1, pad, HO,
+                                 WO, splits, partial, false, &sp, strm);
+  if (e != hipSuccess) return e;
+  if (sp <= 1) return hipErrorInvalidValue;
+  return bn_reduce_stats_bwd_launch(partial, sp, dx, bx, by, mask, mean,
+                                    invstd, relu, bn_slab, M, C, strm);
+}
+
 
 template <bool OUT_BF16, int SPLITS = 0>
 __global__ void splitk_reduce_k(const float4v *__restrict__ partial,
                                 int splits_rt, long len4,
                                 void *__restrict__ out) {
-  const int splits = SPLITS ? SPLITS : splits_rt;
   for (long i = blockIdx.x * blockDim.x + threadIdx.x; i < len4;
        i += (long)gridDim.x * blockDim.x) {
-    float4v a = partial[i];
-    float4v b = {0.f, 0.f, 0.f, 0.f};
-    int s = 1;
-    if (SPLITS == 0) {
-      for (; s + 8 <= splits; s += 8) {
-        float4v c0 = {0.f, 0.f, 0.f, 0.f};
-        float4v c1 = {0.f, 0.f, 0.f, 0.f};
-#pragma unroll
-        for (int j = 0; j < 8; j += 2) {
-          c0 += partial[(long)(s + j) * len4 + i];
-          c1 += partial[(long)(s + j + 1) * len4 + i];
-        }
-        a += c0;
-        b += c1;
-      }
-    }
-#pragma unroll
-    for (; s + 1 < splits; s += 2) {
-      a += partial[(long)s * len4 + i];
-      b += partial[(long)(s + 1) * len4 + i];
-    }
-    if (s < splits) b += partial[(long)s * len4 + i];
-    a += b;
+    float4v a = splitk_sum4<SPLITS>(partial, splits_rt, len4, i);
     if (OUT_BF16) {
       uint16_t *o = (uint16_t *)out + i * 4;
 #pragma unroll
diff --git a/mpi_operator_amd/ops/csrc/mix_gemm.h b/mpi_operator_amd/ops/csrc/mix_gemm.h
--- a/mpi_operator_amd/ops/csrc/mix_gemm.h
+++ b/mpi_operator_amd/ops/csrc/mix_gemm.h
@@ -224,18 +224,22 @@
   int C;
   mutable float s0[2][2], s1[2][2];
   mutable int tm[2], colc[2];
-  mutable int half_;
+  mutable int h_, c_, band_;
   typedef long RowCtx;
   DEV_INLINE void reset() const {
     s0[0][0] = s0[0][1] = s0[1][0] = s0[1][1] = 0.f;
     s1[0][0] = s1[0][1] = s1[1][0] = s1[1][1] = 0.f;
     tm[0] = tm[1] = -1;
     colc[0] = colc[1] = -1;
-    half_ = 0;
+    h_ = c_ = 0;
+    band_ = -1;
+  }
+  DEV_INLINE void slot(int band, int colslot) const {
+    h_ = band;
+    c_ = colslot;
   }
   DEV_INLINE RowCtx row_ctx(int row) const {
-    half_ = (row >> 6) & 1;
-    tm[half_] = row >> 6;
+    band_ = row >> 6;
     return (long)row * ldc;
   }
   DEV_INLINE void store_f32(float *p, RowCtx b, int col, float v) const {
@@ -245,10 +249,10 @@
     uint16_t r = f2bf(v);
     p[b + col] = r;
     float vr = bf2f(r);
-    int ci = (col >> 5) & 1;
-    colc[ci] = col;
-    s0[half_][ci] += vr;
-    s1[half_][ci] += vr * vr;
+    tm[h_] = band_;
+    colc[c_] = col;
+    s0[h_][c_] += vr;
+    s1[h_][c_] += vr * vr;
   }
   DEV_INLINE void flush(int lane) const {
 #pragma unroll
@@ -424,6 +428,7 @@
       for (int ni = 0; ni < 2; ++ni) {
         int col = col0 + wc * 64 + ni * 32 + (lane & 31);
         if (col >= N) continue;
+        if constexpr (WR::STATS) wrt.slot(0, ni);
         if (C_F32)
           wrt.store_f32((float *)cptr, rc, col, acc[mi][ni][r]);
         else
@@ -490,11 +495,9 @@
 #include "pipe256.h"
 #include "pipe_mix.h"
 
-template <class LA, class LB>
-static hipError_t launch_nt_gemm(const LA &la, const LB &lb, void *c, int M,
-                                 int N, int K, long ldc, bool c_f32,
-                                 hipStream_t s, int splits = 1,
-                                 const float *bias = nullptr) {
+enum NtRoute { NT_PIPE256, NT_256, NT_PIPEMIX, NT_GLDS, NT_REG };
+static inline NtRoute nt_gemm_route(int M, int N, int K, long ldc, int kdim_a,
+                                    int kdim_b, int splits) {
   static const bool use_256 = [] {
     const char *e = getenv("MPIAMD_GEMM256");
     return !(e && e[0] == '0');
@@ -504,17 +507,32 @@
     return !(e && e[0] == '0');
   }();
   if (use_256 && splits <= 1 && M % 256 == 0 && N % 256 == 0 && K % 32 == 0 &&
-      K > 0 && la.kdim == K && lb.kdim == K && ldc == N &&
-      (long)(M / 256) * (N / 256) >= 128) {
-    if (use_pipe && K % 64 == 0)
-      return launch_pipe256(la, lb, c, M, N, K, ldc, c_f32, s, bias);
-    return launch_nt256(la, lb, c, M, N, K, ldc, c_f32, s, bias);
-  }
+      K > 0 && kdim_a == K && kdim_b == K && ldc == N &&
+      (long)(M / 256) * (N / 256) >= 128)
+    return (use_pipe && K % 64 == 0) ? NT_PIPE256 : NT_256;
   static const bool use_pipent = [] {
     const char *e = getenv("MPIAMD_PIPENT");
     return !(e && e[0] == '0');
   }();
-  if (use_pipemix() && use_pipent) {
+  if (use_pipemix() && use_pipent) return NT_PIPEMIX;
+  static const bool use_glds = [] {
+    const char *e = getenv("MPIAMD_GLDS");
+    return !(e && e[0] == '0');
+  }();
+  return use_glds ? NT_GLDS : NT_REG;
+}
+
+template <class LA, class LB>
+static hipError_t launch_nt_gemm(const LA &la, const LB &lb, void *c, int M,
+                                 int N, int K, long ldc, bool c_f32,
+                                 hipStream_t s, int splits = 1,
+                                 const float *bias = nullptr) {
+  switch (nt_gemm_route(M, N, K, ldc, la.kdim, lb.kdim, splits)) {
+  case NT_PIPE256:
+    return launch_pipe256(la, lb, c, M, N, K, ldc, c_f32, s, bias);
+  case NT_256:
+    return launch_nt256(la, lb, c, M, N, K, ldc, c_f32, s, bias);
+  case NT_PIPEMIX: {
     NtPipe<PlainNtSrc> ga{{la.p, la.ld, la.rows, la.kdim}};
     NtPipe<PlainNtSrc> gb{{lb.p, lb.ld, lb.rows, lb.kdim}};
     if (bias)
@@ -523,17 +541,16 @@
     return launch_pipe_mix_wr(ga, gb, c, M, N, K, LinearWriter{ldc}, ldc,
                               c_f32, s, splits);
   }
-  static const bool use_glds = [] {
-    const char *e = getenv("MPIAMD_GLDS");
-    return !(e && e[0] == '0');
-  }();
-  if (use_glds) {
+  case NT_GLDS: {
     GldsNt ga{la.p, la.rows, la.ld, la.kdim};
     GldsNt gb{lb.p, lb.rows, lb.ld, lb.kdim};
     if (bias)
       return launch_mix_gemm_wr(ga, gb, c, M, N, K, BiasWriter{ldc, bias},
                                 ldc, c_f32, s, splits);
     return launch_mix_gemm(ga, gb, c, M, N, K, ldc, c_f32, s, splits);
+  }
+  default:
+    break;
   }
   if (bias)
     return launch_mix_gemm_wr(NtStage<LA>{la}, NtStage<LB>{lb}, c, M, N, K,
diff --git a/mpi_operator_amd/ops/csrc/pipe256.h b/mpi_operator_amd/ops/csrc/pipe256.h
--- a/mpi_operator_amd/ops/csrc/pipe256.h
+++ b/mpi_operator_amd/ops/csrc/pipe256.h
@@ -130,6 +130,7 @@
 #pragma unroll
         for (int ni = 0; ni < 2; ++ni) {
           int col = col0 + wc * 64 + ni * 32 + (lane & 31);
+          if constexpr (WR::STATS) wrt.slot(mi >> 1, ni);
           if (C_F32)
             wrt.store_f32((float *)cptr, rc, col, acc[mi][ni][r]);
           else
@@ -266,6 +267,7 @@
 #pragma unroll
         for (int ni = 0; ni < 2; ++ni) {
           int col = col0 + wc * 64 + ni * 32 + (lane & 31);
+          if constexpr (WR::STATS) wrt.slot(0, ni);
           if (C_F32)
             wrt.store_f32((float *)cptr, rc, col, acc[mh][ni][r]);
           else
diff --git a/mpi_operator_amd/ops/csrc/pipe_mix.h b/mpi_operator_amd/ops/csrc/pipe_mix.h
--- a/mpi_operator_amd/ops/csrc/pipe_mix.h
+++ b/mpi_operator_amd/ops/csrc/pipe_mix.h
@@ -469,6 +469,7 @@
       for (int ni = 0; ni < 2; ++ni) {
         int col = col0 + wc * 64 + ni * 32 + (lane & 31);
         if (col >= N) continue;
+        if constexpr (WR::STATS) wrt.slot(0, ni);
         if (C_F32)
           wrt.store_f32((float *)cptr, rc, col, acc[mi][ni][r]);
         else
@@ -514,12 +515,10 @@
                                      int M, int N, int K, const WR &wrt,
                                      long ldc, bool c_f32, hipStream_t s,
                                      int splits = 1) {
-  if constexpr (!WR::STATS) {
-    if (use_pipe8())
-      return launch_pipe_mix8_wr(typename Pipe8Of<SA>::type{sa.s},
-                                 typename Pipe8Of<SB>::type{sb.s}, c, M, N,
-                                 K, wrt, ldc, c_f32, s, splits);
-  }
+  if (use_pipe8())
+    return launch_pipe_mix8_wr(typename Pipe8Of<SA>::type{sa.s},
+                               typename Pipe8Of<SB>::type{sb.s}, c, M, N, K,
+                               wrt, ldc, c_f32, s, splits);
   const uint16_t *zeros = pm_zeros_page();
   if (!zeros) return hipErrorOutOfMemory;
   int tiles_m = (M + PM_BM - 1) / PM_BM, tiles_n = (N + PM_BM - 1) / PM_BM;
@@ -695,12 +694,14 @@
       typename WR::RowCtx rc = wrt.row_ctx(row);
       int col = col0 + wc * 32 + (lane & 31);
       if (col >= N) continue;
+      if constexpr (WR::STATS) wrt.slot(0, 0);
       if (C_F32)
         wrt.store_f32((float *)cptr, rc, col, acc[mi][r]);
       else
         wrt.store_bf16((uint16_t *)cptr, rc, col, acc[mi][r]);
     }
   }
+  if constexpr (WR::STATS) wrt.flush(lane);
 }
 #undef PM8_IMG
 
diff --git a/mpi_operator_amd/ops/fused_block.py b/mpi_operator_amd/ops/fused_block.py
--- a/mpi_operator_amd/ops/fused_block.py
+++ b/mpi_operator_amd/ops/fused_block.py
@@ -6,7 +6,10 @@
 
 import os as _os
 
-_FUSEBN = _os.environ.get("MPIAMD_FUSEBN", "0") == "1"
+_FUSEBN = _os.environ.get("MPIAMD_FUSEBN", "1") == "1"
+_FUSEBN_EPI = _FUSEBN and _os.environ.get("MPIAMD_FUSEBN_EPI", "0") == "1"
+_FUSEBN_SPLITK = _FUSEBN and _os.environ.get("MPIAMD_FUSEBN_SPLITK", "1") == "1"
+_FUSEBN_BWD = _FUSEBN and _os.environ.get("MPIAMD_FUSEBN_BWD", "1") == "1"
 
 _EMPTY = None
 
@@ -29,12 +32,13 @@
         e = _empty()
 
         def conv_bn(xin, w, st, pad, g, b, eps_, relu, rm, rv, mom, res):
-            if not _FUSEBN:
+            if not (_FUSEBN_EPI or _FUSEBN_SPLITK):
                 a = ext.conv2d_fwd(xin, w, st, pad)
                 y, m, v, mk = ext.bn_fwd_train(a, g, b, eps_, relu, rm, rv,
                                                mom, res)
                 return a, y, m, v, mk
-            a, slab = ext.conv2d_fwd_bn(xin, w, st, pad)
+            a, slab = ext.conv2d_fwd_bn(xin, w, st, pad, _FUSEBN_SPLITK,
+                                        _FUSEBN_EPI)
             if slab.numel() > 0:
                 y, m, v, mk = ext.bn_fwd_train_pre(a, slab, g, b, eps_, relu,
                                                    rm, rv, mom, res)
@@ -74,13 +78,22 @@
             ad, md, vd, wd, gd = ctx.saved_tensors[22:]
 
         dout = dout.contiguous(memory_format=torch.channels_last)
+
+        def dgrad_bn(dyo, w, st_, pad, a, y, g, m, v, mk):
+            if not _FUSEBN_BWD or st_ != 1:
+                dy = ext.conv2d_dgrad(dyo, w, y.shape[2], y.shape[3], st_, pad)
+                return ext.bn_bwd(dy, a, y, g, m, v, True, mk)
+            dy, slab = ext.conv2d_dgrad_bn(dyo, w, y.shape[2], y.shape[3],
+                                           st_, pad, a, y, m, v, True, mk)
+            if slab.numel() > 0:
+                return ext.bn_bwd_pre(dy, slab, a, y, g, m, v, True, mk)
+            return ext.bn_bwd(dy, a, y, g, m, v, True, mk)
+
         dx3, dg3, db3 = ext.bn_bwd(dout, a3, out, g3, m3, v3, True, mk3)
         dw3 = ext.conv2d_wgrad(y2, dx3, 1, 1, 1, 0)
-        dy2 = ext.conv2d_dgrad(dx3, w3, y2.shape[2], y2.shape[3], 1, 0)
-        dx2, dg2, db2 = ext.bn_bwd(dy2, a2, y2, g2, m2, v2, True, mk2)
+        dx2, dg2, db2 = dgrad_bn(dx3, w3, 1, 0, a2, y2, g2, m2, v2, mk2)
         dw2 = ext.conv2d_wgrad(y1, dx2, 3, 3, st, 1)
-        dy1 = ext.conv2d_dgrad(dx2, w2, y1.shape[2], y1.shape[3], st, 1)
-        dx1, dg1, db1 = ext.bn_bwd(dy1, a1, y1, g1, m1, v1, True, mk1)
+        dx1, dg1, db1 = dgrad_bn(dx2, w2, st, 1, a1, y1, g1, m1, v1, mk1)
         dw1 = ext.conv2d_wgrad(x, dx1, 1, 1, 1, 0)
 
         dx0 = ext.conv2d_dgrad(dx1, w1, x.shape[2], x.shape[3], 1, 0)
```

Result: faster. 3913 images/sec (median of 6 runs) (+1.4%).
